# pachterlab/kallisto

Hardware: AMD Instinct MI355X
Metric: M paired-end reads/sec quantified (human txome index) (higher is better)
Workload: dtype u64+f64

## Files before the change

__graft_entry__.py:

```python
from __future__ import annotations

import os
import subprocess
import sys

ROOT = os.path.dirname(os.path.abspath(__file__))
if ROOT not in sys.path:
    sys.path.insert(0, ROOT)


def build() -> None:
    env = dict(os.environ)
    subprocess.check_call(["make", "-C", os.path.join(ROOT, "kallisto_amd", "csrc"), f"-j{min(os.cpu_count() or 1, 8)}", "all"], env=env)
    subprocess.check_call(["make", "-C", os.path.join(ROOT, "oracle"), "oracle"], env=env)
    subprocess.check_call(["make", "-C", os.path.join(ROOT, "tests", "emu")], env=env)
    subprocess.check_call(["make", "-C", os.path.join(ROOT, "tests", "emu_ixbuild")], env=env)
    subprocess.check_call(["make", "-C", os.path.join(ROOT, "tests", "emu_aa")], env=env)
    subprocess.check_call(["make", "-C", os.path.join(ROOT, "tests", "emu_shade")], env=env)
    subprocess.check_call(["make", "-C", os.path.join(ROOT, "tests", "emu_inflate")], env=env)
    subprocess.check_call(["make", "-C", os.path.join(ROOT, "tests", "emu_readec")], env=env)
    subprocess.check_call(["make", "-C", os.path.join(ROOT, "tests", "emu_bustag")], env=env)
    if os.path.exists("/root/reference/src/main.cpp"):
        subprocess.check_call(["make", "-C", os.path.join(ROOT, "oracle"), "-j8", "ref"], env=env)
        subprocess.check_call(["make", "-C", os.path.join(ROOT, "oracle"), "ref_bound"], env=env)
    import kallisto_amd
    kallisto_amd.load_library()
    if os.path.exists(os.path.join(ROOT, "oracle", "_ref", "kallisto")):
        for extra in ([], ["--workload", "stress"], ["--genes", "46000"]):
            subprocess.check_call([sys.executable, os.path.join(ROOT, "bench.py"), "--prepare-only", *extra], env=env)


def smoke() -> None:
    import numpy as np
    import kallisto_amd as ka
    from oracle import oracle as O
    from tests import common

    meta, idx_path, r1, r2 = common.load_case("ref_test_pe")
    reads = common.interleave(r1, r2)
    index = ka.Index(idx_path)
    ctx = ka.Context(0)
    ctx.upload(index)
    words, lens, max_len = ctx.pack_reads_host(reads)
    opts = ka.QuantOpts(1, 0.0, 0.0, 0, 0)
    res = ka.quant(ctx, opts, [(words, lens, len(r1), max_len)])
    oix = O.Index(idx_path)
    buf, off, ln = O.pack_reads(reads)
    ores = O.process_reads(oix, O.Opts(1, 0.0, 0.0, 0, 0), buf, off, ln)
    assert res.ecs.multiset() == ores.multiset(), "EC counts differ from the oracle"
    assert np.array_equal(res.flens, ores.flens), "fragment length sample differs from the oracle"
    eff, _ = O.eff_lens(oix.target_lens, O.mean_frag_lens_trunc(ores.flens))
    assert np.array_equal(eff, res.eff_lens)
    alpha, _, rounds = O.em_run(ores.ec_off, ores.ec_ids, ores.counts, eff, oix.num_targets)
    common.assert_abundance_close(res.est_counts, alpha, "est_counts")
    print(f"smoke ok: {res.n_processed} pairs, {res.n_pseudoaligned} pseudoaligned, {len(res.ecs.counts)} ECs, "
          f"EM rounds {res.em_rounds} (oracle {rounds})")


if __name__ == "__main__":
    build()
    if len(sys.argv) > 1 and sys.argv[1] == "smoke":
        smoke()
```

kallisto_amd/csrc/kamd_ctx.hip:

```cpp
#include "kamd_dev.h"

namespace {
void tuning_defaults(kamd_tuning* t) {
  memset(t, 0, sizeof *t);
  t->text_verify = 1; t->items_per_wave = 1024; t->refill_min = 8; t->lds_pad = -1;
  t->em_form = 3; t->em_local_block = 1024; t->em_group_div = -1; t->em_split_len = 16; t->em_small_nnz = -1; t->em_entries_per_lane = -1; t->em_windowed = 2; t->em_graph = 1; t->em_row_lanes = 4;
  t->em_fin_blocks = 1024; t->dedup_form = 2; t->align_chunks = -1; t->em_reg_slices = 1;
  t->em_hybrid = 1; t->overflow_second_pass = 1; t->em_giant_nnz = -1; t->em_blocked = 1;
}
void tuning_merge(kamd_tuning* t, const kamd_tuning& n) {
  if (n.text_verify == 1 || n.text_verify == 2) t->text_verify = n.text_verify;
  if (n.dedup_form == 1 || n.dedup_form == 2) t->dedup_form = n.dedup_form;
  if (n.items_per_wave >= 64) t->items_per_wave = n.items_per_wave;
  if (n.refill_min >= 1 && n.refill_min <= 64) t->refill_min = n.refill_min;
  if (n.lds_pad != 0) t->lds_pad = n.lds_pad < 0 ? -1 : n.lds_pad;
  if (n.em_form >= 1 && n.em_form <= 3) t->em_form = n.em_form;
  if (n.em_local_block == 128 || n.em_local_block == 256 || n.em_local_block == 512 || n.em_local_block == 1024) t->em_local_block = n.em_local_block;
  if (n.em_split_len >= 1 && n.em_split_len <= 64) t->em_split_len = n.em_split_len;
  if (n.em_group_div >= 1 && n.em_group_div <= 1024) t->em_group_div = n.em_group_div;
  else if (n.em_group_div < 0) t->em_group_div = -1;
  if (n.em_small_nnz != 0) t->em_small_nnz = n.em_small_nnz < 0 ? -1 : std::min(n.em_small_nnz, 4096);
  if (n.em_entries_per_lane != 0) t->em_entries_per_lane = n.em_entries_per_lane < 0 ? -1 : n.em_entries_per_lane;
  if (n.em_windowed == 1 || n.em_windowed == 2) t->em_windowed = n.em_windowed;
  if (n.em_graph == 1 || n.em_graph == 2) t->em_graph = n.em_graph;
  if (n.em_row_lanes == 2 || n.em_row_lanes == 4 || n.em_row_lanes == 8) t->em_row_lanes = n.em_row_lanes;
  if (n.em_fin_blocks >= 64) t->em_fin_blocks = n.em_fin_blocks;
  if (n.align_chunks != 0) t->align_chunks = n.align_chunks < 0 ? -1 : std::min(n.align_chunks, 64);
  if (n.em_reg_slices == 1 || n.em_reg_slices == 2) t->em_reg_slices = n.em_reg_slices;
  if (n.em_hybrid == 1 || n.em_hybrid == 2) t->em_hybrid = n.em_hybrid;
  if (n.overflow_second_pass >= 1 && n.overflow_second_pass <= 3) t->overflow_second_pass = n.overflow_second_pass;
  if (n.em_blocked == 1 || n.em_blocked == 2) t->em_blocked = n.em_blocked;
  if (n.em_giant_nnz != 0) t->em_giant_nnz = n.em_giant_nnz < 0 ? -1 : std::max(n.em_giant_nnz, 8);
}
void tuning_from_env(kamd_tuning* t) {
  const char* e = getenv("KAMD_TUNE");
  if (!e || !*e) return;
  kamd_tuning n; memset(&n, 0, sizeof n);
  struct Field { const char* name; int32_t kamd_tuning::*p; bool onoff; };
  static const Field fields[] = {
    {"text_verify", &kamd_tuning::text_verify, true}, {"items_per_wave", &kamd_tuning::items_per_wave, false}, {"refill_min", &kamd_tuning::refill_min, false},
    {"lds_pad", &kamd_tuning::lds_pad, false}, {"em_form", &kamd_tuning::em_form, false}, {"em_entries_per_lane", &kamd_tuning::em_entries_per_lane, false},
    {"em_windowed", &kamd_tuning::em_windowed, true}, {"em_graph", &kamd_tuning::em_graph, true}, {"em_row_lanes", &kamd_tuning::em_row_lanes, false},
    {"em_fin_blocks", &kamd_tuning::em_fin_blocks, false}, {"em_local_block", &kamd_tuning::em_local_block, false}, {"em_group_div", &kamd_tuning::em_group_div, false},
    {"em_split_len", &kamd_tuning::em_split_len, false}, {"dedup_form", &kamd_tuning::dedup_form, false}, {"align_chunks", &kamd_tuning::align_chunks, false},
    {"em_small_nnz", &kamd_tuning::em_small_nnz, false}, {"em_reg_slices", &kamd_tuning::em_reg_slices, true}, {"em_hybrid", &kamd_tuning::em_hybrid, true},
    {"overflow_second_pass", &kamd_tuning::overflow_second_pass, false}, {"em_giant_nnz", &kamd_tuning::em_giant_nnz, false}, {"em_blocked", &kamd_tuning::em_blocked, true}};
  std::string all(e);
  for (size_t pos = 0; pos < all.size();) {
    size_t end = all.find(',', pos);
    if (end == std::string::npos) end = all.size();
    const std::string kv = all.substr(pos, end - pos);
    pos = end + 1;
    const size_t eq = kv.find('=');
    if (eq == std::string::npos) continue;
    const std::string key = kv.substr(0, eq), val = kv.substr(eq + 1);
    bool known = false;
    for (const Field& f : fields) {
      if (key != f.name) continue;
      known = true;
      int32_t v = atoi(val.c_str());
      if (key == "em_form") v = val == "streamed" ? 1 : val == "csr" ? 2 : val == "local" ? 3 : v;
      if (key == "overflow_second_pass" && v == 0) v = 2;
      n.*(f.p) = f.onoff ? (v != 0 ? 1 : 2) : v;
    }
    if (!known) fprintf(stderr, "[kallisto_amd] KAMD_TUNE: unknown field '%s' ignored\n", key.c_str());
  }
  tuning_merge(t, n);
}
}
namespace kamdi {
void apply_quant_opts(kamd_ctx* c, const kamd_quant_opts* o) {
  c->ix.no_jump = o->no_jump ? 1 : 0;
  c->ix.union_mode = o->do_union ? 1 : 0;
  c->ix.comprehensive = (o->strand != 0 && (o->no_jump || o->do_union || c->ix.n_shades)) ? 1 : 0;
}
void apply_tuning(kamd_ctx* c) {
  c->items_per_wave = c->tune.items_per_wave; c->refill_min = c->tune.refill_min;
}
int sync_state(kamd_ctx* c) {
  if (!c->state_pin) HIPC(hipHostMalloc((void**)&c->state_pin, sizeof(DevState), hipHostMallocDefault));
  HIPC(hipMemcpyAsync(c->state_pin, c->state.p, sizeof(DevState), hipMemcpyDeviceToHost, c->stream));
  HIPC(hipStreamSynchronize(c->stream));
  memcpy(&c->host_state, c->state_pin, sizeof(DevState));
  return 0;
}
int push_state(kamd_ctx* c) {
  HIPC(hipMemcpyAsync(c->state.p, &c->host_state, sizeof(DevState), hipMemcpyHostToDevice, c->stream));
  return 0;
}
}

extern "C" uint32_t kamd_abi_version(void) { return KAMD_ABI_VERSION; }
extern "C" int kamd_ctx_create(int device, void* hip_stream, kamd_ctx** out) {
  if (!out) return kamd::fail(-1, "kamd_ctx_create: null output pointer");
  *out = nullptr;
  int ndev = 0;
  if (hipGetDeviceCount(&ndev) != hipSuccess || ndev == 0)
    return kamd::fail(-102, "kamd_ctx_create: no HIP device available (this library has no CPU path)");
  if (device < 0 || device >= ndev) return kamd::fail(-1, "kamd_ctx_create: bad device ordinal");
  HIPC(hipSetDevice(device));
  kamd_ctx* c = new kamd_ctx;
  c->device = device;
  c->stream = (hipStream_t)hip_stream;
  { int v = 0; if (hipDeviceGetAttribute(&v, hipDeviceAttributeMultiprocessorCount, device) != hipSuccess || v <= 0) v = 256; c->n_cus = v; }
  if (c->state.ensure(sizeof(DevState), 0, c->stream)) { delete c; return -100; }
  memset(&c->host_state, 0, sizeof c->host_state);
  if (push_state(c)) { delete c; return -100; }
  if (hipEventCreate(&c->ev0) != hipSuccess || hipEventCreate(&c->ev1) != hipSuccess || hipEventCreate(&c->ev2) != hipSuccess || hipEventCreate(&c->ev3) != hipSuccess) { delete c; return kamd::fail(-100, "hipEventCreate failed"); }
  if (c->stats_a.ensure(sizeof(DevStatsA), 0, c->stream) || hipMemsetAsync(c->stats_a.p, 0, sizeof(DevStatsA), c->stream) != hipSuccess) { delete c; return -100; }
  tuning_defaults(&c->tune);
  tuning_from_env(&c->tune);
  apply_tuning(c);
  *out = c;
  return 0;
}

extern "C" int kamd_ctx_tune(kamd_ctx* c, const kamd_tuning* t) {
  if (!c || !t) return kamd::fail(-1, "kamd_ctx_tune: null argument");
  tuning_merge(&c->tune, *t);
  apply_tuning(c);
  return 0;
}
extern "C" int kamd_ctx_get_tuning(const kamd_ctx* c, kamd_tuning* out) {
  if (!c || !out) return kamd::fail(-1, "kamd_ctx_get_tuning: null argument");
  *out = c->tune;
  return 0;
}

extern "C" void kamd_ctx_destroy(kamd_ctx* c) {
  if (!c) return;
  (void)hipSetDevice(c->device);
  (void)hipStreamSynchronize(c->stream);
  comm_detach_all(c);
  if (c->ev0) (void)hipEventDestroy(c->ev0);
  if (c->ev1) (void)hipEventDestroy(c->ev1);
  if (c->ev2) (void)hipEventDestroy(c->ev2);
  if (c->ev3) (void)hipEventDestroy(c->ev3);
  if (c->al_stream) { (void)hipStreamSynchronize(c->al_stream); (void)hipStreamDestroy(c->al_stream); }
  if (c->al_ev_in) (void)hipEventDestroy(c->al_ev_in);
  if (c->al_ev_out) (void)hipEventDestroy(c->al_ev_out);
  for (hipEvent_t e : c->al_ev_chunk) if (e) (void)hipEventDestroy(e);
  if (c->ev_fin0) (void)hipEventDestroy(c->ev_fin0);
  if (c->ev_fin1) (void)hipEventDestroy(c->ev_fin1);
  for (hipEvent_t e : c->aa_ev) if (e) (void)hipEventDestroy(e);
  for (hipEvent_t e : c->rec_ev) if (e) (void)hipEventDestroy(e);
  for (hipEvent_t e : c->bus_ev) if (e) (void)hipEventDestroy(e);
  if (c->ev_ab0) (void)hipEventDestroy(c->ev_ab0);
  if (c->ev_ab1) (void)hipEventDestroy(c->ev_ab1);
  if (c->em_stream) (void)hipStreamDestroy(c->em_stream);
  if (c->em_side_stream) { (void)hipStreamSynchronize(c->em_side_stream); (void)hipStreamDestroy(c->em_side_stream); }
  if (c->em_ev_fork) (void)hipEventDestroy(c->em_ev_fork);
  if (c->em_ev_join) (void)hipEventDestroy(c->em_ev_join);
  if (c->em_pin) (void)hipHostFree(c->em_pin);
  if (c->state_pin) (void)hipHostFree(c->state_pin);
  c->em_clk.release();
  if (c->hy_giant_stream) { (void)hipStreamSynchronize(c->hy_giant_stream); (void)hipStreamDestroy(c->hy_giant_stream); }
  if (c->hy_ev_sell) (void)hipEventDestroy(c->hy_ev_sell);
  if (c->hy_ev_giant) (void)hipEventDestroy(c->hy_ev_giant);
  if (c->ev_mg0) (void)hipEventDestroy(c->ev_mg0);
  if (c->ev_mg1) (void)hipEventDestroy(c->ev_mg1);
  if (c->ev_ov0) (void)hipEventDestroy(c->ev_ov0);
  if (c->ev_ov1) (void)hipEventDestroy(c->ev_ov1);
  if (c->ov_stream) { (void)hipStreamSynchronize(c->ov_stream); (void)hipStreamDestroy(c->ov_stream); }
  for (hipEvent_t e : {c->ov_ev_in, c->ov_ev_done, c->ov_ev_t0, c->ov_ev_t1}) if (e) (void)hipEventDestroy(e);
  if (c->ov_pin) (void)hipHostFree(c->ov_pin);
  c->ov_state.release();
  for (DBuf* b : {&c->hy_sub, &c->hy_a, &c->hy_b, &c->hy_x, &c->hy_maps, &c->hy_gb[0], &c->hy_gb[1], &c->hy_gb[2], &c->hy_gb[3], &c->hy_gb[4], &c->hy_gb[5]}) b->release();
  if (c->fld_stream) { (void)hipStreamSynchronize(c->fld_stream); (void)hipStreamDestroy(c->fld_stream); }
  if (c->fld_ev) (void)hipEventDestroy(c->fld_ev);
  if (c->fld_ev_in) (void)hipEventDestroy(c->fld_ev_in);
  if (c->fld_host) (void)hipHostFree(c->fld_host);
  if (c->fq_host) (void)hipHostFree(c->fq_host);
  if (c->sell_cache) sell_cache_free(c->sell_cache);
  for (void* p : c->index_allocs) (void)hipFree(p);
  for (DBuf* b : {&c->dense, &c->stream_buf, &c->rec_off, &c->overflow_items, &c->overflow_scratch, &c->state, &c->rec_slot,
                  &c->retry, &c->ttable, &c->tstore, &c->stats_a, &c->list, &c->cand, &c->cand_off, &c->cand_slot, &c->ctable, &c->tup_bound, &c->tup_off, &c->tup_big, &c->raw2, &c->overflow_left, &c->stats_b, &c->clist, &c->sizes, &c->explicit_items,
                  &c->explicit_items_big, &c->exp_stream, &c->exp_off, &c->exp_scratch, &c->bs_cp, &c->bs_samp, &c->raw, &c->dense_first, &c->exp_key, &c->cand_key, &c->ec_first, &c->pm_a, &c->pm_b, &c->pm_rank, &c->eml_tmp, &c->ems_tmp, &c->ems_plan, &c->ems_maps, &c->fld_tl, &c->fld_card, &c->fld_scratch, &c->fld_items, &c->fld_cand,
                  &c->block_sums, &c->ec_off, &c->ec_ids, &c->ec_counts, &c->em_alpha, &c->em_next, &c->em_eff,
                  &c->em_state, &c->em_cn, &c->em_colcnt, &c->em_coloff, &c->em_colrow,
                  &c->em_segoff, &c->em_segt, &c->em_partial, &c->em_a0, &c->em_a1, &c->em_single, &c->em_actflag, &c->em_actpos, &c->em_active, &c->pt_label, &c->pt_flag, &c->pt_len,
                  &c->pt_rowpos, &c->pt_nnzpos, &c->pt_off, &c->pt_ids, &c->pt_counts, &c->pt_wcounts, &c->pt_hist, &c->pt_ck_alpha,
                  &c->pt_ck_a, &c->fq_tiles, &c->fq_nlpos[0], &c->fq_nlpos[1], &c->fq_recs, &c->fq_res, &c->fq_words, &c->fq_len, &c->aa_frames, &c->aa_flen, &c->aa_scratch, &c->aa_offlist, &c->aa_ctr, &c->inf_members, &c->inf_res, &c->txt_counts, &c->txt_res,
                  &c->rec_table, &c->rec_scratch, &c->rec_big_scratch, &c->rec_big_items, &c->rec_ctr, &c->bus_blk, &c->bus_ctr})
    b->release();
  delete c;
}

namespace {
__global__ void k_bm_fill(const u64* __restrict__ ec_off, const u32* __restrict__ ec_ids, const u32* __restrict__ which, u32 stride, u32* words) {
  const u32 e = which[blockIdx.x];
  u32* w = words + (u64)blockIdx.x * stride;
  for (u64 j = ec_off[e] + threadIdx.x; j < ec_off[e + 1]; j += blockDim.x) { const u32 x = ec_ids[j]; atomicOr(&w[x >> 5], 1u << (x & 31)); }
}
}
extern "C" int kamd_index_upload(kamd_ctx* c, const kamd_index* hix) {
  if (!c || !hix) return kamd::fail(-1, "kamd_index_upload: null argument");
  HIPC(hipSetDevice(c->device));
  kamd_index_view v;
  if (int rc = kamd_index_get_view(hix, &v)) return rc;
  const bool build_table = v.table == nullptr;
  HIPC(hipStreamSynchronize(c->stream));
  c->has_index = false;
  for (void* p : c->index_allocs) (void)hipFree(p);
  c->index_allocs.clear();
  DevIndex d{};
  d.k = v.k; d.n_buckets = v.n_buckets; d.n_ecs = v.n_ecs;
  d.table_layout = (int)v.table_layout; d.tag_q = v.tag_q; d.tag_dsh = v.tag_dsh; d.tag_w = v.tag_w;
  const u64 slots = (v.n_buckets + v.pad_buckets) * v.slots_per_bucket;
  if (!build_table) {
    if (int rc = upload(c, (const u64*)v.table, (size_t)(v.n_buckets + v.pad_buckets) * 8, &d.table)) return rc;
    if (int rc = upload(c, v.slot_block, slots, &d.slot_block)) return rc;
    if (int rc = upload(c, v.slot_dist, slots, &d.slot_dist)) return rc;
  }
  if (int rc = upload(c, v.uec_ec, v.n_uec, &d.uec_ec)) return rc;
  if (int rc = upload(c, (const u64*)v.ec_off, v.n_ecs + 1, &d.ec_off)) return rc;
  if (int rc = upload(c, v.ec_ids, v.ec_nnz, &d.ec_ids)) return rc;
  std::vector<uint8_t> ne(v.n_ecs + 1);
  for (u64 e = 0; e < v.n_ecs; e++) ne[e] = v.ec_off[e + 1] > v.ec_off[e];
  if (int rc = upload(c, ne.data(), v.n_ecs, &d.ec_nonempty)) return rc;
  std::vector<u32> ecn(v.n_uec + 1);
  for (u64 u = 0; u < v.n_uec; u++) ecn[u] = v.uec_ec[u] | (ne[v.uec_ec[u]] ? 0x80000000u : 0u);
  if (int rc = upload(c, ecn.data(), v.n_uec, &d.uec_ecn)) return rc;
  if (int rc = upload(c, v.onlist_bits, v.onlist_words, &d.onlist_bits)) return rc;
  d.n_shades = v.n_shades;
  if (v.n_shades) {
    if (int rc = upload(c, (const u64*)v.core_off, v.n_ecs + 1, &d.core_off)) return rc;
    if (int rc = upload(c, v.core_ids, (size_t)v.core_nnz, &d.core_ids)) return rc;
    if (int rc = upload(c, (const u64*)v.shade_off, v.n_ecs + 1, &d.shade_off)) return rc;
    if (int rc = upload(c, v.shade_ids, (size_t)v.shade_nnz, &d.shade_ids)) return rc;
    if (int rc = upload(c, v.shade_colour, (size_t)v.n_targets, &d.shade_colour)) return rc;
  }
  {
    const uint64_t* boff = v.n_shades ? v.core_off : v.ec_off;
    const u64 n_ids = v.n_targets + v.dlist_size;
    const u32 stride = (u32)((n_ids + 31) / 32);
    std::vector<std::pair<u64, u32>> big;
    for (u64 e = 0; e < v.n_ecs; e++) { const u64 sz = boff[e + 1] - boff[e]; if (sz > BM_MIN_MEMBERS) big.emplace_back(sz, (u32)e); }
    std::sort(big.begin(), big.end(), [](const std::pair<u64, u32>& a, const std::pair<u64, u32>& b) { return a.first > b.first || (a.first == b.first && a.second < b.second); });
    const size_t fit = stride ? BM_MAX_BYTES / ((size_t)stride * 4) : 0;
    if (big.size() > fit) big.resize(fit);
    d.bm_stride = stride; d.bm_min = big.empty() ? 0xFFFFFFFFu : BM_MIN_MEMBERS;
    d.ec_bm_slot = nullptr; d.bm_words = nullptr;
    if (!big.empty()) {
      std::vector<u32> slot(v.n_ecs, BM_NONE), which(big.size());
      for (size_t s = 0; s < big.size(); s++) { slot[big[s].second] = (u32)s; which[s] = big[s].second; }
      const u32* d_which = nullptr; const u32* d_words = nullptr;
      if (int rc = upload(c, slot.data(), slot.size(), &d.ec_bm_slot)) return rc;
      if (int rc = upload(c, which.data(), which.size(), &d_which)) return rc;
      {
        void* p = nullptr;
        HIPC(hipMalloc(&p, big.size() * (size_t)stride * 4));
        c->index_allocs.push_back(p);
        HIPC(hipMemsetAsync(p, 0, big.size() * (size_t)stride * 4, c->stream));
        d_words = (const u32*)p;
      }
      hipLaunchKernelGGL(k_bm_fill, dim3((unsigned)big.size()), dim3(256), 0, c->stream, v.n_shades ? d.core_off : d.ec_off, v.n_shades ? d.core_ids : d.ec_ids, d_which, stride, const_cast<u32*>(d_words));
      HIPC(hipGetLastError());
      d.bm_words = d_words;
      HIPC(hipStreamSynchronize(c->stream));
    }
    c->n_set_bitmaps = (u32)big.size();
  }
  if (int rc = upload(c, (const u64*)v.unitig_blk_off, v.n_unitigs + 1, &d.unitig_blk_off)) return rc;
  if (int rc = upload(c, v.unitig_len, v.n_unitigs, &d.unitig_len)) return rc;
  if (int rc = upload(c, v.blk_unitig, v.n_blocks, &d.blk_unitig)) return rc;
  if (int rc = upload(c, v.blk_lb, v.n_blocks, &d.blk_lb)) return rc;
  if (int rc = upload(c, v.blk_ub, v.n_blocks, &d.blk_ub)) return rc;
  if (int rc = upload(c, v.blk_ec, v.n_blocks, &d.blk_ec)) return rc;
  if (int rc = upload(c, (const u64*)v.blk_pos_off, v.n_blocks + 1, &d.blk_pos_off)) return rc;
  if (int rc = upload(c, v.blk_posw, (size_t)v.blk_pos_off[v.n_blocks], &d.blk_posw)) return rc;
  if (int rc = upload(c, v.blk_sense, (size_t)v.blk_pos_off[v.n_blocks], &d.blk_sense)) return rc;
  if (int rc = upload(c, v.target_lens, v.n_targets + v.dlist_size, &d.target_lens)) return rc;
  d.dtable = nullptr; d.n_dbuckets = v.n_dbuckets; d.dummy_slot = v.dummy_slot; d.dummy_uec = v.dummy_uec; d.dummy_strand = v.dummy_strand;
  if (v.n_dbuckets) if (int rc = upload(c, (const u64*)v.dtable, (size_t)(v.n_dbuckets + v.dpad_buckets) * 8, &d.dtable)) return rc;
  if (int rc = upload(c, v.utext, (size_t)v.utext_words, &d.utext)) return rc;
  HIPC(hipStreamSynchronize(c->stream));
  kamd_table_info ti; memset(&ti, 0, sizeof ti);
  if (build_table) { if (int rc = index_build_device(c, hix, v, &d, &ti)) return rc; }
  else {
    ti.n_buckets = v.n_buckets; ti.pad_buckets = v.pad_buckets; ti.table_layout = v.table_layout; ti.slots_per_bucket = v.slots_per_bucket;
    ti.tag_q = v.tag_q; ti.tag_dsh = v.tag_dsh; ti.tag_w = v.tag_w; ti.n_dbuckets = v.n_dbuckets; ti.dpad_buckets = v.dpad_buckets;
    ti.dummy_slot = v.dummy_slot; ti.dummy_uec = v.dummy_uec; ti.dummy_strand = v.dummy_strand;
  }
  c->tinfo = ti;
  c->aa_ready = false; memset(&c->aa_stats, 0, sizeof c->aa_stats);
  c->ix = d; c->has_index = true; c->n_ecs = v.n_ecs; c->n_targets = v.n_targets;
  if (int rc = c->dense.ensure(std::max<u64>(v.n_ecs, 1) * sizeof(u32), 0, c->stream)) return rc;
  HIPC(hipMemsetAsync(c->dense.p, 0, std::max<u64>(v.n_ecs, 1) * sizeof(u32), c->stream));
  if (int rc = c->dense_first.ensure(std::max<u64>(v.n_ecs, 1) * sizeof(u64), 0, c->stream)) return rc;
  HIPC(hipMemsetAsync(c->dense_first.p, 0xFF, std::max<u64>(v.n_ecs, 1) * sizeof(u64), c->stream));
  memset(&c->host_state, 0, sizeof c->host_state);
  c->finalized = false; c->exp_words_done = 0; c->recs_total = 0; c->multi_before = 0; c->last_absorb_ms = 0.f; c->overflow_total = 0; c->overflow_ms = 0.f;
  if (int rc = tuples_clear(c)) return rc;
  HIPC(hipMemsetAsync(c->stats_a.p, 0, sizeof(DevStatsA), c->stream));
  return push_state(c);
}

extern "C" int kamd_ec_reset(kamd_ctx* c) {
  if (!c || !c->has_index) return kamd::fail(-1, "kamd_ec_reset: no context / index");
  HIPC(hipSetDevice(c->device));
  HIPC(hipMemsetAsync(c->dense.p, 0, std::max<u64>(c->n_ecs, 1) * sizeof(u32), c->stream));
  HIPC(hipMemsetAsync(c->dense_first.p, 0xFF, std::max<u64>(c->n_ecs, 1) * sizeof(u64), c->stream));
  memset(&c->host_state, 0, sizeof c->host_state);
  c->finalized = false; c->exp_words_done = 0; c->recs_total = 0; c->multi_before = 0; c->last_absorb_ms = 0.f; c->overflow_total = 0; c->overflow_ms = 0.f; c->overflow_second_total = 0;
  if (c->ov_side_pending) { (void)hipStreamSynchronize(c->ov_stream); c->ov_side_pending = false; }
  if (int rc = tuples_clear(c)) return rc;
// ... 428 lines not shown
```

kallisto_amd/csrc/kamd_dev.h:

```cpp
#pragma once

#include <hip/hip_runtime.h>

#include <dlfcn.h>

#include <algorithm>
#include <cstring>
#include <string>
#include <chrono>
#include <thread>
#include <vector>

#include "../../include/kallisto_amd.h"
#include "kamd_core.h"
#include "kamd_fq_core.h"
#include "kamd_host.h"
#include "kamd_em_local.h"
#include "kamd_em_sell.h"

#define HIPC(x)                                                                                   \
  do {                                                                                            \
    hipError_t e_ = (x);                                                                          \
    if (e_ != hipSuccess) return kamd::fail(-100, std::string(#x) + ": " + hipGetErrorString(e_)); \
  } while (0)
// ... 93 lines not shown
constexpr u32 BM_NONE = 0xFFFFFFFFu;
constexpr u32 BM_MIN_MEMBERS = 128;
constexpr size_t BM_MAX_BYTES = 256u << 20;
__device__ __forceinline__ bool bitmap_has(const DevIndex& ix, u32 slot, u32 x) { return (ix.bm_words[(u64)slot * ix.bm_stride + (x >> 5)] >> (x & 31)) & 1u; }
__device__ __forceinline__ bool set_has(const DevIndex& ix, u32 e, u64 off, u32 sz, u32 x) {
  if (sz > ix.bm_min) { const u32 s = ix.ec_bm_slot[e]; if (s != BM_NONE) return bitmap_has(ix, s, x); }
  return set_contains(ix.ec_ids + off, sz, x);
}
__host__ __device__ inline kamd::ShadeTables shade_tables(const DevIndex& ix) {
  return kamd::ShadeTables{(const uint64_t*)ix.core_off, ix.core_ids, (const uint64_t*)ix.shade_off, ix.shade_ids, ix.shade_colour};
}
__host__ __device__ inline DevIndex core_view(DevIndex ix) {
  if (ix.n_shades) { ix.ec_off = ix.core_off; ix.ec_ids = ix.core_ids; ix.n_shades = 0; }
  return ix;
}
template <class F>
__device__ __forceinline__ void for_each_member(const DevIndex& ix, const kamd::EcList& ecs, u32* cur, F&& f) {
  if (ix.n_shades) {
    kamd::for_each_in_shaded_set(shade_tables(ix), ecs, ix.union_mode != 0, cur, [&](u32 x) { if (onlisted(ix.onlist_bits, x)) f(x); });
    return;
  }
  const kamd::SetTables st{(const uint64_t*)ix.ec_off, ix.ec_ids};
  kamd::for_each_in_set(st, ecs, ix.union_mode != 0, cur, [&](u32 x) { if (onlisted(ix.onlist_bits, x)) f(x); });
}
__device__ __forceinline__ kamd::PosTables pos_tables(const DevIndex& ix) {
  return kamd::PosTables{(const uint64_t*)ix.unitig_blk_off, ix.unitig_len, ix.blk_unitig, ix.blk_lb, ix.blk_ub, ix.blk_ec,
                         (const uint64_t*)ix.blk_pos_off, ix.blk_posw, ix.blk_sense, (const uint64_t*)ix.ec_off, ix.ec_ids,
                         ix.target_lens, ix.k};
}
__device__ __forceinline__ kamd::FirstHit first_hit(const DevIndex& ix, const kamd::MateInfo& m) {
  kamd::FirstHit h; h.valid = m.n_hits > 0;
  h.block = h.valid ? ix.slot_block[m.first_slot] : 0u; h.dist = h.valid ? ix.slot_dist[m.first_slot] : 0u;
  h.strand = m.first_strand; h.pos = m.first_pos;
  return h;
}
__device__ __forceinline__ kamd::FilterCfg item_filter_cfg(const FilterDev& fd, bool paired, const kamd::MateInfo& m0,
                                                           const kamd::MateInfo& m1) {
  kamd::FilterCfg cfg;
  cfg.fraglen = !fd.single_overhang && fd.has_mean_fl && (!paired || m0.n_hits == 0 || m1.n_hits == 0);
  cfg.fl = fd.fl; cfg.strand = fd.strand;
  cfg.comprehensive = fd.comprehensive != 0 && fd.strand != 0;
  return cfg;
}
__device__ __forceinline__ bool needs_hit_list(const FilterDev& fd, const kamd::MateInfo& m1) {
  return fd.comprehensive != 0 && fd.strand != 0 && m1.n_hits == 0;
}
__device__ __noinline__ u32 class_size_bound(const DevIndex& ix, const kamd::EcList& ecs) {
  if (ix.n_shades) return (u32)kamd::shaded_size_bound(shade_tables(ix), ecs.e, ecs.n, ix.union_mode != 0);
  const kamd::SetTables st{(const uint64_t*)ix.ec_off, ix.ec_ids};
  return (u32)kamd::set_size_bound(st, ecs.e, ecs.n, ix.union_mode != 0);
}
__device__ __forceinline__ int filter_outcome(const DevIndex& ix, const FilterDev& fd, bool paired, const kamd::MateInfo& m0,
                                              const kamd::MateInfo& m1, const kamd::EcList& ecs, u32* kept, u32* cur) {
  const kamd::FilterCfg cfg = item_filter_cfg(fd, paired, m0, m1);
  if (!cfg.fraglen && !cfg.strand) return 0;
  if (needs_hit_list(fd, m1)) {
    *kept = class_size_bound(ix, ecs);
    return 2;
  }
  const kamd::PosTables pt = pos_tables(ix);
  const kamd::FirstHit h0 = first_hit(ix, m0), h1 = first_hit(ix, m1);
  u32 total = 0, keep = 0;
  for_each_member(ix, ecs, cur, [&](u32 tr) { ++total; keep += kamd::keep_transcript(pt, cfg, h0, h1, tr) ? 1u : 0u; });
  *kept = keep;
  return keep == total ? 0 : (keep == 0 ? 1 : 2);
}
struct DBuf {
  void* p = nullptr; size_t cap = 0;
  int ensure(size_t bytes, size_t keep, hipStream_t s) {
    if (bytes <= cap) return 0;
    size_t ncap = std::max(bytes, 2 * cap);
    void* np = nullptr;
    HIPC(hipMalloc(&np, ncap));
    if (keep && p) HIPC(hipMemcpyAsync(np, p, keep, hipMemcpyDeviceToDevice, s));
    if (p) { HIPC(hipStreamSynchronize(s)); HIPC(hipFree(p)); }
    p = np; cap = ncap;
    return 0;
  }
  void release() { if (p) (void)hipFree(p); p = nullptr; cap = 0; }
  template <class T> T* as() { return reinterpret_cast<T*>(p); }
};

inline unsigned grid_for(u64 n, int block) { return (unsigned)((n + block - 1) / block); }

struct SellCache;
void sell_cache_free(SellCache*);
}
using namespace kamdi;
namespace {
__global__ void k_copy_words(const u32* __restrict__ src, u64 n, u32* dst) {
  u64 i = (u64)blockIdx.x * blockDim.x + threadIdx.x;
  if (i < n) dst[i] = src[i];
}
__global__ void k_copy_offsets(const u64* __restrict__ src, u64 n, u64 base, u64* dst) {
  u64 i = (u64)blockIdx.x * blockDim.x + threadIdx.x;
  if (i < n) dst[i] = src[i] + base;
}
}

struct kamd_ctx {
  int device = 0;
  hipStream_t stream = nullptr;
  bool has_index = false;
  DevIndex ix{};
  std::vector<void*> index_allocs;
  u64 n_ecs = 0, n_targets = 0;
  u32 n_set_bitmaps = 0;
  kamd_table_info tinfo{};
  DBuf dense, stream_buf, rec_off, overflow_items, overflow_scratch, state, rec_slot, retry, ttable, list;
  DBuf cand, cand_off, cand_slot, ctable, clist, sizes, block_sums, tup_bound, tup_off, tup_big;
  DBuf raw2, overflow_left, stats_b;
  u64 overflow_second_total = 0;
  DBuf ov_state; DevState* ov_pin = nullptr; hipStream_t ov_stream = nullptr; hipEvent_t ov_ev_in = nullptr, ov_ev_done = nullptr, ov_ev_t0 = nullptr, ov_ev_t1 = nullptr;
  bool ov_side_pending = false;
  u64 last_fin_big = 0;
  DBuf explicit_items, explicit_items_big, exp_stream, exp_off, exp_scratch, bs_cp, bs_samp, raw, dense_first, exp_key, cand_key, ec_first;
  DBuf ec_off, ec_ids, ec_counts;
  DBuf em_alpha, em_next, em_eff, em_state, em_cn, em_colcnt, em_coloff, em_colrow, em_segoff, em_segt, em_partial, em_a0, em_a1, em_single, em_actflag, em_actpos, em_active;
  DBuf pm_a, pm_b, pm_rank;
  DBuf eml_tmp, ems_tmp, ems_plan, ems_maps;
  SellCache* sell_cache = nullptr;
  u64 ec_generation = 0;
  int last_em_plan_cached = 0;
  DBuf fq_tiles, fq_nlpos[2], fq_recs, fq_res, fq_words, fq_len;
  void* fq_host = nullptr;
  u64 fq_batch_reads = 0; int32_t fq_batch_max_len = 0, fq_batch_files = 0;
  DBuf fld_tl, fld_card, fld_scratch, fld_items, fld_cand;
  void* fld_host = nullptr; u64 fld_host_cap = 0;
  hipStream_t fld_stream = nullptr; hipEvent_t fld_ev = nullptr, fld_ev_in = nullptr;
  struct { const uint32_t* w = nullptr; const uint16_t* l = nullptr; u64 n = 0; int32_t max_len = 0, strand = 0, so = 0; bool valid = false; } fld_pending;
  struct { const uint32_t* w = nullptr; const uint16_t* l = nullptr; u64 n = 0; int32_t max_len = 0, strand = 0, so = 0, comp = 0; bool valid = false; } fld_deferred;
  DBuf pt_label, pt_flag, pt_len, pt_rowpos, pt_nnzpos, pt_off, pt_ids, pt_counts, pt_wcounts, pt_hist, pt_ck_alpha, pt_ck_a;
  DevState host_state{};
  DevState* state_pin = nullptr;
  u64 tcap = 0, ccap = 0;
  DBuf tstore;
  bool ttable_clean = false;
  u64 recs_total = 0;
  u64 multi_before = 0;
  u64 n_distinct_tuples = 0;
  float last_absorb_ms = 0.f; hipEvent_t ev_ab0 = nullptr, ev_ab1 = nullptr;
  kamd_ec_result result{};
  bool finalized = false;
  u64 exp_words_done = 0;
  hipEvent_t ev0 = nullptr, ev1 = nullptr;
  float last_align_ms = 0.f, last_em_ms = 0.f, last_classify_ms = 0.f;
  hipEvent_t ev2 = nullptr, ev3 = nullptr, ev_fin0 = nullptr, ev_fin1 = nullptr;
  DBuf stats_a;
  hipStream_t al_stream = nullptr; hipEvent_t al_ev_in = nullptr, al_ev_out = nullptr; std::vector<hipEvent_t> al_ev_chunk;
  float last_finalize_ms = 0.f; u64 last_fin_records = 0, last_fin_stream_words = 0, last_fin_cand_words = 0;
  hipStream_t em_stream = nullptr;
  hipStream_t em_side_stream = nullptr; hipEvent_t em_ev_fork = nullptr, em_ev_join = nullptr;
  void* em_pin = nullptr; size_t em_pin_bytes = 0;
  DBuf em_clk;
  DBuf hy_sub, hy_a, hy_b, hy_x, hy_maps;
  DBuf hy_gb[6];
  hipStream_t hy_giant_stream = nullptr;
  hipEvent_t hy_ev_sell = nullptr, hy_ev_giant = nullptr;
  uint64_t last_em_max_comp_nnz = 0, last_em_giant_nnz = 0, last_em_giant_rows = 0, last_em_giant_tr = 0;
  uint32_t last_em_giant_chunks = 0; uint64_t last_em_giant_pieces = 0; int last_em_graph_fallback = 0; float last_em_plan_ms = 0.f;
  float last_merge_ms = 0.f, em_coll_ms = 0.f; uint32_t em_coll_n = 0; hipEvent_t ev_mg0 = nullptr, ev_mg1 = nullptr;
  const uint32_t* labels_override = nullptr;
  bool em_prefer_hybrid = false;
  uint64_t overflow_total = 0; float overflow_ms = 0.f; hipEvent_t ev_ov0 = nullptr, ev_ov1 = nullptr;
  int items_per_wave = 1024, refill_min = 8;
  kamd_tuning tune{};
  bool track_order = false;
  bool had_overflow_items = false;
  int n_cus = 0, last_em_k = 0; unsigned last_em_grid = 0, last_em_lds = 0;
  uint64_t last_em_iters = 0, last_em_nnz = 0, last_em_nnz_multi = 0, last_em_nseg = 0, last_em_necs = 0;
  DBuf aa_frames, aa_flen, aa_scratch, aa_offlist, aa_ctr;
  bool aa_ready = false;
  kamd_aa_stats aa_stats{};
  hipEvent_t aa_ev[3] = {nullptr, nullptr, nullptr};
  DBuf inf_members, inf_res, txt_counts, txt_res;
  DBuf rec_table, rec_scratch, rec_big_scratch, rec_big_items, rec_ctr;
  u64 rec_table_gen = 0, rec_table_cap = 0, rec_chunk = 0, rec_second = 0;
  int rec_small_cap = 0;
  hipEvent_t rec_ev[3] = {nullptr, nullptr, nullptr};
  float rec_table_ms = 0.f, rec_items_ms = 0.f;
  DBuf bus_blk, bus_ctr;
  hipEvent_t bus_ev[2] = {nullptr, nullptr};
  std::vector<struct kamd_comm*> comms;
};

namespace kamdi {
int sync_state(kamd_ctx* c);
int push_state(kamd_ctx* c);
void apply_quant_opts(kamd_ctx* c, const kamd_quant_opts* o);
void apply_tuning(kamd_ctx* c);
void comm_detach_all(kamd_ctx* c);
int index_build_device(kamd_ctx* c, const kamd_index* hix, const kamd_index_view& v, DevIndex* d, kamd_table_info* info);
int exclusive_scan(kamd_ctx* c, const u32* sizes, u64 n, u64* out, u64* d_total);
int tuples_clear(kamd_ctx* c);
int absorb_tuples(kamd_ctx* c, const u32* batch, const u64* rec_off, u64 n, u64 batch_words, u64 key_base, u64 n_tuple_bound,
                  const u64* first_idx = nullptr, u32 fixed_stride = 0, u64 item0 = 0);
template <class T>
int upload(kamd_ctx* c, const T* host, size_t n, const T** dev) {
  void* p = nullptr;
  size_t bytes = std::max<size_t>(n, 1) * sizeof(T);
  HIPC(hipMalloc(&p, bytes));
  c->index_allocs.push_back(p);
  if (n) HIPC(hipMemcpyAsync(p, host, n * sizeof(T), hipMemcpyHostToDevice, c->stream));
  *dev = reinterpret_cast<const T*>(p);
  return 0;
}
}
```

kallisto_amd/csrc/kamd_em.hip:

```cpp
#include "kamd_dev.h"

namespace {

struct EmState {
  int iter;
  int chcount;
  int final_round;
  int done;
  int rounds;
  int force_final;
  int pad[2];
};
struct EmNow { int it, fin, done, rounds; };
__host__ __device__ inline EmNow em_next_round(const EmState& prev, int n_iter, int min_rounds, bool spec) {
  EmNow n; n.it = prev.iter; n.fin = prev.final_round; n.done = prev.done; n.rounds = prev.rounds;
  if (n.done) return n;
  if (prev.final_round) { n.done = 1; n.rounds = prev.iter; return n; }
  const bool stopEM = !spec && prev.chcount == 0 && prev.iter > min_rounds;
  n.it = prev.iter + 1;
  n.fin = (stopEM || prev.force_final) ? 1 : 0;
  if (n.it >= n_iter) { n.done = 1; n.rounds = n_iter; }
  return n;
}
__device__ __forceinline__ double em_clamped(const double* alpha, const double* a, u32 t, int clamp) {
// ... 763 lines not shown
    case 8: pm_launch_round<8>(P, s, parity); break;
    case 12: pm_launch_round<12>(P, s, parity); break;
    case 16: pm_launch_round<16>(P, s, parity); break;
    case 20: pm_launch_round<20>(P, s, parity); break;
    case 24: pm_launch_round<24>(P, s, parity); break;
    case 28: pm_launch_round<28>(P, s, parity); break;
    default: pm_launch_round<32>(P, s, parity); break;
  }
}

int em_streamed_setup(kamd_ctx* c, const u64* ec_off, const u32* ec_ids, const u32* counts, const u32* wcounts, u64 n_ecs, u64 T,
                      const u32* col_cnt, u32* col_fill, PmPlan* P, DBuf* arena_a = nullptr, DBuf* arena_b = nullptr) {
  if (n_ecs == 0) return 1;
  DBuf& ar_a = arena_a ? *arena_a : c->pm_a;
  DBuf& ar_b = arena_b ? *arena_b : c->pm_b;
  if (c->n_cus == 0) {
    int v = 0;
    HIPC(hipDeviceGetAttribute(&v, hipDeviceAttributeMultiprocessorCount, c->device));
    c->n_cus = v > 0 ? v : 256;
  }
  Carver s1;
  const size_t o_hist = s1.take((T + 1) * 4), o_fill = s1.take((T + 1) * 4), o_mflag = s1.take(T * 4);
  const size_t o_start = s1.take((T + 2) * 8), o_rpos = s1.take((n_ecs + 1) * 8), o_mpos = s1.take((T + 1) * 8);
  const size_t o_len = s1.take((n_ecs + 1) * 4), o_roff = s1.take((n_ecs + 2) * 8);
  if (int rc = ar_a.ensure(s1.off, 0, c->stream)) return rc;
  char* b1 = (char*)ar_a.p;
  u32* hist = (u32*)(b1 + o_hist); u32* mflag = (u32*)(b1 + o_mflag);
  u64* start = (u64*)(b1 + o_start); u64* rpos = (u64*)(b1 + o_rpos); u64* mpos = (u64*)(b1 + o_mpos);
  u32* len_sorted = (u32*)(b1 + o_len); u64* roff = (u64*)(b1 + o_roff);
  (void)o_fill;
  HIPC(hipMemsetAsync(hist, 0, (o_mflag - o_hist), c->stream));
  hipLaunchKernelGGL(k_pm_flags, dim3(grid_for(std::max(n_ecs, T), BLOCK)), dim3(BLOCK), 0, c->stream, ec_off, ec_ids, n_ecs, col_cnt, T, hist,
                     mflag);
  if (int rc = exclusive_scan(c, hist, T, start, start + T)) return rc;
  if (int rc = exclusive_scan(c, mflag, T, mpos, mpos + T)) return rc;
  u64 R = 0, NZ = 0, M = 0;
  HIPC(hipMemcpyAsync(&R, start + T, 8, hipMemcpyDeviceToHost, c->stream));
  HIPC(hipMemcpyAsync(&M, mpos + T, 8, hipMemcpyDeviceToHost, c->stream));
  HIPC(hipMemcpyAsync(&NZ, c->em_coloff.as<u64>() + T, 8, hipMemcpyDeviceToHost, c->stream));
  HIPC(hipStreamSynchronize(c->stream));
  if (NZ == 0 || R == 0 || M == 0 || R >= 0x7FFFFFF0ULL || M >= 0x7FFFFFF0ULL || NZ >= (1ULL << 40)) return 1;
  {
    if (n_ecs >= 0xFFFFFFF0ULL) return 1;
    const u32 n_tiles = (u32)((n_ecs + PM_RANK_TILE - 1) / PM_RANK_TILE);
    const u64 n_cells = (u64)PM_RANK_BUCKETS * n_tiles;
    Carver rv;
    const size_t o_key = rv.take(n_ecs * 8), o_oa = rv.take(n_ecs * 4), o_ob = rv.take(n_ecs * 4), o_h = rv.take(n_cells * 4), o_f = rv.take((n_cells + 2) * 8);
    if (int rc = c->pm_rank.ensure(rv.off, 0, c->stream)) return rc;
    char* rb = (char*)c->pm_rank.p;
    u64* key = (u64*)(rb + o_key); u32* ord[2] = {(u32*)(rb + o_oa), (u32*)(rb + o_ob)}; u32* rhist = (u32*)(rb + o_h); u64* rfirst = (u64*)(rb + o_f);
    hipLaunchKernelGGL(k_pm_rowkey, dim3(grid_for(n_ecs * 8, BLOCK)), dim3(BLOCK), 0, c->stream, ec_off, ec_ids, n_ecs, T, key);
    const u32* in = nullptr;
    for (int pass = 0; pass < PM_RANK_PASSES; pass++) {
      u32* out = ord[pass & 1];
      hipLaunchKernelGGL(k_pm_radix_hist, dim3(n_tiles), dim3(64), 0, c->stream, (const u64*)key, in, n_ecs, pass, n_tiles, rhist);
      if (int rc = exclusive_scan(c, rhist, n_cells, rfirst, rfirst + n_cells)) return rc;
      hipLaunchKernelGGL(k_pm_radix_place, dim3(n_tiles), dim3(64), 0, c->stream, (const u64*)key, in, n_ecs, pass, n_tiles, (const u64*)rfirst, out);
      in = out;
    }
    hipLaunchKernelGGL(k_pm_rank_emit, dim3(grid_for(R, BLOCK)), dim3(BLOCK), 0, c->stream, ec_off, in, R, rpos, len_sorted);
    HIPC(hipGetLastError());
  }
  if (int rc = exclusive_scan(c, len_sorted, R, roff, roff + R)) return rc;
  int K = PM_KS[sizeof(PM_KS) / sizeof(PM_KS[0]) - 1];
  bool k_forced = false;
  if (c->tune.em_entries_per_lane > 0) { for (int k : PM_KS) if (k == c->tune.em_entries_per_lane) { K = k; k_forced = true; } }
  if (!k_forced) for (int k : PM_KS) if ((NZ + 64ULL * k - 1) / (64ULL * k) <= (u64)c->n_cus * 12) { K = k; break; }
  const u32 chunk = 64u * (u32)K;
  const u64 n_chunks64 = (NZ + chunk - 1) / chunk;
  if (n_chunks64 >= 0x7FFFFFF0ULL) return 1;
  const u32 n_chunks = (u32)n_chunks64;
  const u64 nzpad = (u64)n_chunks * chunk;
  Carver s2;
  const size_t front = 64 * PM_HEAD * 4;
  const size_t o_rs = s2.take(front + nzpad * 4), o_cs = s2.take(front + nzpad * 4);
  size_t o_meta[2][5];
  size_t o_lane[2];
  for (int s = 0; s < 2; s++) {
    for (int j = 0; j < 3; j++) o_meta[s][j] = s2.take((size_t)n_chunks * 4);
    for (int j = 3; j < 5; j++) o_meta[s][j] = s2.take((size_t)n_chunks * 8);
    o_lane[s] = s2.take((size_t)n_chunks * 64 * 4);
  }
  const size_t o_cw = s2.take(R * 8), o_coff = s2.take((M + 1) * 8), o_g = s2.take((R + 1) * 8);
  size_t o_vec[6];
  for (int j = 0; j < 6; j++) o_vec[j] = s2.take((M + 1) * 8);
  const size_t o_single = s2.take(M * 8), o_eff = s2.take(M * 8), o_nfix = s2.take(64);
  if (int rc = ar_b.ensure(s2.off, 0, c->stream)) return rc;
  char* b2 = (char*)ar_b.p;
  u32* rs = (u32*)(b2 + o_rs + front); u32* cs = (u32*)(b2 + o_cs + front);
  HIPC(hipMemsetAsync(b2 + o_rs, 0, front, c->stream));
  HIPC(hipMemsetAsync(b2 + o_cs, 0, front, c->stream));
  u64* cw = (u64*)(b2 + o_cw); u64* coff = (u64*)(b2 + o_coff);
  double* g = (double*)(b2 + o_g);
  double* vec[6]; for (int j = 0; j < 6; j++) vec[j] = (double*)(b2 + o_vec[j]);
  double* single_m = (double*)(b2 + o_single); double* eff_m = (double*)(b2 + o_eff);
  HIPC(hipMemsetAsync(b2 + o_nfix, 0, 64, c->stream));
  HIPC(hipMemsetAsync(g + R, 0, 8, c->stream));
  const u64* col_off = c->em_coloff.as<u64>();
  hipLaunchKernelGGL(k_pm_rows, dim3(grid_for(n_ecs * 8, BLOCK)), dim3(BLOCK), 0, c->stream, ec_off, ec_ids, counts, wcounts, n_ecs, rpos, roff,
                     mpos, rs, cw);
  hipLaunchKernelGGL(k_pm_cols, dim3(grid_for(n_ecs * 8, BLOCK)), dim3(BLOCK), 0, c->stream, ec_off, ec_ids, n_ecs, rpos, col_off, col_fill, cs);
  if (nzpad > NZ) {
    hipLaunchKernelGGL(k_pm_fill, dim3(grid_for(nzpad - NZ, BLOCK)), dim3(BLOCK), 0, c->stream, rs, NZ, nzpad, (u32)M);
    hipLaunchKernelGGL(k_pm_fill, dim3(grid_for(nzpad - NZ, BLOCK)), dim3(BLOCK), 0, c->stream, cs, NZ, nzpad, (u32)R);
  }
  hipLaunchKernelGGL(k_pm_minit, dim3(grid_for(T, BLOCK)), dim3(BLOCK), 0, c->stream, T, mflag, mpos, col_off, c->em_single.as<double>(),
                     c->em_eff.as<double>(), M, coff, single_m, eff_m, vec[0], vec[1], vec[2], vec[3], vec[4], vec[5]);
  PmSide sides[2];
  for (int s = 0; s < 2; s++) {
    PmSide& d = sides[s];
    d.stream = s == 0 ? rs : cs;
    u32* sb = (u32*)(b2 + o_meta[s][0]); u32* hd = (u32*)(b2 + o_meta[s][1]); u32* ff = (u32*)(b2 + o_meta[s][2]);
    d.seg_base = sb; d.head = hd; d.fix_first = ff;
    d.lp = (double*)(b2 + o_meta[s][3]); d.rp = (double*)(b2 + o_meta[s][4]);
    d.n_chunks = n_chunks;
    u32* lw = (u32*)(b2 + o_lane[s]);
    d.lane_word = lw;
    hipLaunchKernelGGL(k_pm_lanes, dim3(grid_for(n_chunks, PM_BLOCK / 64)), dim3(PM_BLOCK), 0, c->stream, d.stream, chunk / 64, n_chunks, lw);
    hipLaunchKernelGGL(k_pm_chunks, dim3(grid_for(n_chunks, BLOCK)), dim3(BLOCK), 0, c->stream, s == 0 ? roff : coff, s == 0 ? R : M, NZ, chunk,
                       n_chunks, sb, hd, ff, (u32*)(b2 + o_nfix) + s, (u32*)(b2 + o_nfix) + 2, getenv("KAMD_EM_NO_LONG_HEADS") ? 1 : 0);
  }
  HIPC(hipGetLastError());
  PmArgs& A = P->args;
  A.rows = sides[0]; A.cols = sides[1];
  A.cw = cw; A.g = g;
  A.alpha0 = vec[0]; A.alpha1 = vec[1]; A.a0 = vec[2]; A.a1 = vec[3]; A.ac0 = vec[4]; A.ac1 = vec[5];
  A.single = single_m; A.eff = eff_m;
  A.R = (u32)R; A.M = (u32)M;
  A.st = (EmState*)c->em_state.p;
  u32 plan_words[3] = {0, 0, 0};
  HIPC(hipMemcpyAsync(plan_words, b2 + o_nfix, sizeof plan_words, hipMemcpyDeviceToHost, c->stream));
  HIPC(hipStreamSynchronize(c->stream));
  P->n_fix[0] = plan_words[0]; P->n_fix[1] = plan_words[1];
  P->windowed = plan_words[2] > (u32)PM_LDS_SLOTS;
  if (c->tune.em_windowed == 1) P->windowed = true;
  P->k = K; P->n_chunks = n_chunks; P->mflag = mflag; P->mpos = mpos; P->rpos = rpos;
  P->roff = roff; P->coff = coff; P->rs = rs; P->cs = cs; P->nzpad = nzpad;
  c->last_em_nnz_multi = NZ; c->last_em_nseg = n_chunks; c->last_em_necs = n_ecs; c->last_em_k = K;
  c->last_em_grid = grid_for(n_chunks, PM_BLOCK / 64);
  return 0;
}

struct EmLocalDev {
  const u32* row_base; const u32* tr_base; const u64* nz_base;
  const u32* row_ptr; const u32* col_ptr; const uint16_t* row_tr; const uint16_t* col_row;
  const u64* cw; const double* single; const double* eff;
  const u32* tr_id = nullptr;
};
constexpr int EML_MAX_ROUNDS = 64;
struct EmSellDev {
  const u32* row_base; const u32* tr_base; const u32* rslice_base; const u32* cslice_base; const u64* rell_base; const u64* cell_base;
  const u32* rdesc; const u32* cdesc; const uint16_t* rell; const uint16_t* cell;
  const u64* cw; const double* single; const double* eff;
};
constexpr int EMS_MAX_BLOCK = 1024;
template <int EXP>
__device__ __forceinline__ double ems_slice_sum(const u64* e, u32 width, const double* src, u32 n_src) {
  const u32 cf = (u32)lane_id() % n_src;
  u32 sink = 0;
  auto val_at = [&](u32 ix) -> double {
    if constexpr (EXP == 1) { sink += ix; return src[cf]; }
    else if constexpr (EXP == 3) return __hiloint2double(0x3ff00000, (int)ix);
    else return src[ix];
  };
  double S = 0.0;
  u32 j = 0;
  for (; j + 8 <= width; j += 8) {
    const u64 w0 = e[(size_t)(j >> 2) * 64], w1 = e[(size_t)((j >> 2) + 1) * 64];
    const u32 a0 = (u32)w0, a1 = (u32)(w0 >> 32), b0 = (u32)w1, b1 = (u32)(w1 >> 32);
    const double v0 = val_at(a0 & 0xFFFFu), v1 = val_at(a0 >> 16), v2 = val_at(a1 & 0xFFFFu), v3 = val_at(a1 >> 16);
    const double v4 = val_at(b0 & 0xFFFFu), v5 = val_at(b0 >> 16), v6 = val_at(b1 & 0xFFFFu), v7 = val_at(b1 >> 16);
    S += v0; S += v1; S += v2; S += v3; S += v4; S += v5; S += v6; S += v7;
  }
  if (j < width) {
    const u32 rem = width - j;
    const u64 w0 = e[(size_t)(j >> 2) * 64];
    const u64 w1 = rem > 4 ? e[(size_t)((j >> 2) + 1) * 64] : 0ULL;
    const u32 a0 = (u32)w0, a1 = (u32)(w0 >> 32), b0 = (u32)w1, b1 = (u32)(w1 >> 32);
    const double v0 = val_at(a0 & 0xFFFFu);
    const double v1 = rem > 1 ? val_at(a0 >> 16) : 0.0;
    const double v2 = rem > 2 ? val_at(a1 & 0xFFFFu) : 0.0;
    const double v3 = rem > 3 ? val_at(a1 >> 16) : 0.0;
    S += v0;
    if (rem > 1) S += v1;
    if (rem > 2) S += v2;
    if (rem > 3) S += v3;
    if (rem > 4) {
      const double v4 = val_at(b0 & 0xFFFFu);
      const double v5 = rem > 5 ? val_at(b0 >> 16) : 0.0;
      const double v6 = rem > 6 ? val_at(b1 & 0xFFFFu) : 0.0;
      S += v4;
      if (rem > 5) S += v5;
      if (rem > 6) S += v6;
    }
  }
  if constexpr (EXP != 0) { if (sink == 0xFFFFFFFFu) S += 1.0; }
  return S;
}
constexpr int EMS_CLK_ROUND = 8, EMS_CLK_WORDS = 16;
template <bool WAVE_TEAM, int EXP = 0>
__device__ __forceinline__ void ems_group_rounds(const EmSellDev& P, u32 g, unsigned char* smem, u32 tid, u32 nthr, const double* alpha, const double* a,
                                                 double* alpha_out, double* a_out, int n_rounds, int clamp, int* s_hist, long long* clk = nullptr) {
  namespace L = kamd_em_sell;
  const int lane = lane_id();
  const u32 wv = WAVE_TEAM ? 0u : (u32)__builtin_amdgcn_readfirstlane((int)(tid >> 6)), NW = WAVE_TEAM ? 1u : nthr >> 6;
  const u32 r0 = P.row_base[g], nR = P.row_base[g + 1] - r0, t0 = P.tr_base[g], nT = P.tr_base[g + 1] - t0;
  const u32 rs0 = P.rslice_base[g], nrs = P.rslice_base[g + 1] - rs0, cs0 = P.cslice_base[g], ncs = P.cslice_base[g + 1] - cs0;
  const u64 re0 = P.rell_base[g], ce0 = P.cell_base[g];
  const u32 nru = (u32)(P.rell_base[g + 1] - re0), ncu = (u32)(P.cell_base[g + 1] - ce0);
  auto team_sync = [] {
    if (WAVE_TEAM || EXP == 5) __builtin_amdgcn_fence(__ATOMIC_SEQ_CST, "wavefront");
    else __syncthreads();
  };
  double* s_al0 = reinterpret_cast<double*>(smem);
  double* s_a0 = s_al0 + (nT + 1); double* s_al1 = s_a0 + (nT + 1); double* s_a1 = s_al1 + (nT + 1);
  double* s_single = s_a1 + (nT + 1); double* s_eff = s_single + nT; double* s_g = s_eff + nT;
  u64* s_cw = reinterpret_cast<u64*>(s_g + (nR + 1));
  u32* s_rdesc = reinterpret_cast<u32*>(s_cw + nR); u32* s_cdesc = s_rdesc + 2 * nrs;
  uint16_t* s_rell = reinterpret_cast<uint16_t*>(s_cdesc + 2 * ncs); uint16_t* s_cell = s_rell + ((nru + 1) & ~1u);
  for (u32 i = tid; i < nT; i += nthr) {
    double al = alpha[t0 + i], av = a[t0 + i];
    if (clamp && al < 1e-7 / 10.0) { al = 0.0; av = 0.0; }
    s_al0[i] = al; s_a0[i] = av; s_single[i] = P.single[t0 + i]; s_eff[i] = P.eff[t0 + i];
  }
  for (u32 i = tid; i < nR; i += nthr) s_cw[i] = P.cw[r0 + i];
  for (u32 i = tid; i < 2 * nrs; i += nthr) s_rdesc[i] = P.rdesc[2 * (u64)rs0 + i];
  for (u32 i = tid; i < 2 * ncs; i += nthr) s_cdesc[i] = P.cdesc[2 * (u64)cs0 + i];
  for (u32 i = tid; i < nru; i += nthr) { const uint16_t v = P.rell[re0 + i]; s_rell[i] = v == (uint16_t)L::SELL_PAD ? (uint16_t)nT : v; }
  for (u32 i = tid; i < ncu; i += nthr) { const uint16_t v = P.cell[ce0 + i]; s_cell[i] = v == (uint16_t)L::SELL_PAD ? (uint16_t)nR : v; }
  if (tid == 0) { s_al0[nT] = s_a0[nT] = s_al1[nT] = s_a1[nT] = 0.0; s_g[nR] = 0.0; }
  team_sync();
  double* al = s_al0; double* av = s_a0; double* aln = s_al1; double* avn = s_a1;
  for (int r = 0; r < n_rounds; r++) {
    const bool tick = clk && r == EMS_CLK_ROUND && lane == 0;
    long long w0 = 0;
    if (tick) { clk[0] = clock64(); w0 = wall_clock64(); }
    for (u32 s = wv; s < nrs; s += NW) {
      const u32 d0 = s_rdesc[2 * s], d1 = s_rdesc[2 * s + 1];
      const bool meta = (d0 & L::DESC_META) != 0;
      const u32 off = d0 & ~L::DESC_META, width = d1 & 0xFFFFu;
      const bool tk = tick && s == wv;
      if (tk) clk[12] = clock64();
      double S = ems_slice_sum<EXP>(reinterpret_cast<const u64*>(s_rell + off + (meta ? 2 * L::SELL_META_WORDS : 0u)) + lane, width, av, nT);
      if (tk) { clk[13] = clock64(); clk[14] = (long long)(width | (meta ? 0x10000u : 0u)); }
      u32 seg = (d1 >> 16) + (u32)lane; bool fin = seg < nR;
      if (meta) {
        const u32 w = reinterpret_cast<const u32*>(s_rell + off)[lane];
        S = pm_scan_seg(S, (int)((w >> 16) & 0x7Fu), lane);
        seg = w & 0xFFFFu; fin = (w & L::META_ACTIVE) && (w & L::META_LAST);
      }
      if (fin) {
        const u64 cwv = s_cw[seg];
        const u32 cnt = (u32)cwv, wc = (u32)(cwv >> 32);
        if constexpr (EXP == 4) s_g[seg] = (double)cnt * S;
        else s_g[seg] = (cnt == 0 || (double)wc * S < 4.9406564584124654e-324) ? 0.0 : (double)cnt / S;
      }
      if (tk) clk[15] = clock64();
    }
    if (tick) clk[1] = clock64();
    team_sync();
    if (tick) clk[2] = clock64();
    int ch = 0;
    for (u32 s = wv; s < ncs; s += NW) {
      const u32 d0 = s_cdesc[2 * s], d1 = s_cdesc[2 * s + 1];
      const bool meta = (d0 & L::DESC_META) != 0;
      const u32 off = d0 & ~L::DESC_META, width = d1 & 0xFFFFu;
      const bool tk = tick && s == wv;
      if (tk) clk[8] = clock64();
      double acc = ems_slice_sum<EXP>(reinterpret_cast<const u64*>(s_cell + off + (meta ? 2 * L::SELL_META_WORDS : 0u)) + lane, width, s_g, nR);
      if (tk) { clk[9] = clock64(); clk[10] = (long long)(width | (meta ? 0x10000u : 0u)); }
      u32 seg = (d1 >> 16) + (u32)lane; bool fin = seg < nT;
      if (meta) {
        const u32 w = reinterpret_cast<const u32*>(s_cell + off)[lane];
        acc = pm_scan_seg(acc, (int)((w >> 16) & 0x7Fu), lane);
        seg = w & 0xFFFFu; fin = (w & L::META_ACTIVE) && (w & L::META_LAST);
      }
      bool chg = false;
      if (fin) {
        const double at = av[seg], cur = al[seg];
        const double nx = s_single[seg] + at * acc;
        const double dd = fabs(nx - cur);
        bool moved = dd > 1.0000001e-2 * nx;
        if (dd > 0.9999999e-2 * nx && !moved) moved = dd / nx > 1e-2;
        chg = nx > 1e-2 && moved;
        aln[seg] = nx;
        if constexpr (EXP == 4) avn[seg] = nx * s_eff[seg];
        else avn[seg] = nx / s_eff[seg];
      }
      ch += __popcll(__ballot(chg));
      if (tk) clk[11] = clock64();
    }
    if (ch && lane == 0) atomicAdd(&s_hist[r], ch);
    if (tick) clk[3] = clock64();
    team_sync();
    if (tick) { clk[4] = clock64(); clk[5] = (long long)(nrs | (ncs << 16)); clk[6] = (long long)(nru | ((u64)ncu << 32)); clk[7] = wall_clock64() - w0; }
    double* t1 = al; al = aln; aln = t1;
    double* t2 = av; av = avn; avn = t2;
  }
  for (u32 i = tid; i < nT; i += nthr) { alpha_out[t0 + i] = al[i]; a_out[t0 + i] = av[i]; }
}
template <int NB>
__device__ __forceinline__ void ems_reg_gather(const u64* w, const unsigned char* lds0, double* v) {
#pragma unroll
  for (int q = 0; q < NB; q++) {
    u32 lo = (u32)w[q], hi = (u32)(w[q] >> 32);
    asm volatile("" : "+v"(lo), "+v"(hi));
    v[4 * q] = *reinterpret_cast<const double*>(lds0 + (lo & 0xFFFFu)); v[4 * q + 1] = *reinterpret_cast<const double*>(lds0 + (lo >> 16));
    v[4 * q + 2] = *reinterpret_cast<const double*>(lds0 + (hi & 0xFFFFu)); v[4 * q + 3] = *reinterpret_cast<const double*>(lds0 + (hi >> 16));
  }
}
template <int NQ, bool TREE>
__device__ __forceinline__ double ems_reg_sum(const u64* w, const unsigned char* lds0, double S = 0.0) {
  if constexpr (!TREE) {
    constexpr int NB = NQ < 2 ? NQ : 2;
    double v[4 * NB];
    ems_reg_gather<NB>(w, lds0, v);
#pragma unroll
    for (int i = 0; i < 4 * NB; i++) S += v[i];
    if constexpr (NQ > 2) return ems_reg_sum<NQ - 2, false>(w + 2, lds0, S);
    else return S;
  } else {
    constexpr int NB = NQ < 4 ? NQ : 4;
    double v[4 * NB];
    ems_reg_gather<NB>(w, lds0, v);
#pragma unroll
    for (int st = 1; st < 4 * NB; st *= 2)
#pragma unroll
      for (int i = 0; i + st < 4 * NB; i += 2 * st) v[i] += v[i + st];
    if constexpr (NQ > 4) return ems_reg_sum<NQ - 4, true>(w + 4, lds0, S + v[0]);
    else return S + v[0];
  }
}
template <int W, bool TREE, int NQ = 1>
__device__ __forceinline__ double ems_reg_slice_sum(const u64* w, u32 nq, const unsigned char* lds0) {
  if constexpr (NQ >= W) return ems_reg_sum<W, TREE>(w, lds0);
  else { if (nq <= (u32)NQ) return ems_reg_sum<NQ, TREE>(w, lds0); return ems_reg_slice_sum<W, TREE, NQ + 1>(w, nq, lds0); }
}
__device__ __forceinline__ u32 pm_scan_seg_steps(int reach, int lane) {
  const int r = lane & 15;
  u32 m = 0;
  if (__ballot(reach >= 1 && r >= 1)) m |= 1u;
  if (__ballot(reach >= 2 && r >= 2)) m |= 2u;
  if (__ballot(reach >= 4 && r >= 4)) m |= 4u;
  if (__ballot(reach >= 8 && r >= 8)) m |= 8u;
  if (__ballot((lane & 16) && reach > r)) m |= 16u;
  if (__ballot(lane >= 32 && reach > lane - 32)) m |= 32u;
  return m;
}
__device__ __forceinline__ double pm_scan_seg_masked(double y, int reach, int lane, u32 steps) {
  const int r = lane & 15;
  if (steps & 1u) { const double t = pm_dpp<0x111, 0xF>(y); if (reach >= 1 && r >= 1) y += t; }
  if (steps & 2u) { const double t = pm_dpp<0x112, 0xF>(y); if (reach >= 2 && r >= 2) y += t; }
  if (steps & 4u) { const double t = pm_dpp<0x114, 0xF>(y); if (reach >= 4 && r >= 4) y += t; }
  if (steps & 8u) { const double t = pm_dpp<0x118, 0xF>(y); if (reach >= 8 && r >= 8) y += t; }
  if (steps & 16u) { const double t = pm_dpp<0x142, 0xA>(y); if ((lane & 16) && reach > r) y += t; }
  if (steps & 32u) { const double t = pm_dpp<0x143, 0xC>(y); if (lane >= 32 && reach > lane - 32) y += t; }
  return y;
}
__device__ __forceinline__ double ems_slice_sum_narrow(const u64* e, u32 width, const double* src) {
  double S = 0.0;
  for (u32 j = 0; j < width; j += 4) {
    const u64 w = e[(size_t)(j >> 2) * 64];
    const u32 lo = (u32)w, hi = (u32)(w >> 32);
    const double v0 = src[lo & 0xFFFFu], v1 = src[lo >> 16], v2 = src[hi & 0xFFFFu], v3 = src[hi >> 16];
    S += v0; S += v1; S += v2; S += v3;
  }
  return S;
}
template <int W, int NS>
__device__ __forceinline__ void ems_group_rounds_reg(const EmSellDev& P, u32 g, unsigned char* smem, u32 tid, u32 nthr, const double* alpha, const double* a,
                                                     double* alpha_out, double* a_out, int n_rounds, int clamp, int* s_hist, long long* clk = nullptr) {
  namespace L = kamd_em_sell;
  constexpr bool TREE = W >= 8 || (W == 4 && NS == 2);
  const int lane = lane_id();
  const u32 wv = (u32)__builtin_amdgcn_readfirstlane((int)(tid >> 6)), NW = nthr >> 6;
  const u32 r0 = P.row_base[g], nR = P.row_base[g + 1] - r0, t0 = P.tr_base[g], nT = P.tr_base[g + 1] - t0;
  const u32 rs0 = P.rslice_base[g], nrs = P.rslice_base[g + 1] - rs0, cs0 = P.cslice_base[g], ncs = P.cslice_base[g + 1] - cs0;
  const u64 re0 = P.rell_base[g], ce0 = P.cell_base[g];
  const u32 nru = (u32)(P.rell_base[g + 1] - re0), ncu = (u32)(P.cell_base[g + 1] - ce0);
  double* s_a0 = reinterpret_cast<double*>(smem);
  double* s_g = s_a0 + (nT + 1);
  double* s_al0 = s_g + (nR + 1);
  double* s_single = s_al0 + (nT + 1); double* s_eff = s_single + nT;
  u64* s_cw = reinterpret_cast<u64*>(s_eff + nT);
  u32* s_rdesc = reinterpret_cast<u32*>(s_cw + nR); u32* s_cdesc = s_rdesc + 2 * nrs;
  uint16_t* s_rell = reinterpret_cast<uint16_t*>(s_cdesc + 2 * ncs); uint16_t* s_cell = s_rell + ((nru + 1) & ~1u);
  const u32 a_off = 0u, g_off = (nT + 1) * 8u;
  const bool near = g_off + (nR + 1) * 8u <= 0x10000u;
  for (u32 i = tid; i < nT; i += nthr) {
    double al = alpha[t0 + i], av = a[t0 + i];
    if (clamp && al < 1e-7 / 10.0) { al = 0.0; av = 0.0; }
    s_al0[i] = al; s_a0[i] = av; s_single[i] = P.single[t0 + i]; s_eff[i] = P.eff[t0 + i];
  }
  for (u32 i = tid; i < nR; i += nthr) s_cw[i] = P.cw[r0 + i];
  for (u32 i = tid; i < 2 * nrs; i += nthr) s_rdesc[i] = P.rdesc[2 * (u64)rs0 + i];
  for (u32 i = tid; i < 2 * ncs; i += nthr) s_cdesc[i] = P.cdesc[2 * (u64)cs0 + i];
  for (u32 i = tid; i < nru; i += nthr) { const uint16_t v = P.rell[re0 + i]; s_rell[i] = v == (uint16_t)L::SELL_PAD ? (uint16_t)nT : v; }
  for (u32 i = tid; i < ncu; i += nthr) { const uint16_t v = P.cell[ce0 + i]; s_cell[i] = v == (uint16_t)L::SELL_PAD ? (uint16_t)nR : v; }
  if (tid == 0) { s_al0[nT] = s_a0[nT] = 0.0; s_g[nR] = 0.0; }
  __syncthreads();
  struct Own { u64 w[W]; u32 nq, seg, steps; int reach; bool has, meta, fin; };
  auto take = [&](const u32* desc, const uint16_t* ell, u32 s, u32 n_slices, u32 n_segs, u32 zero, u32 base_off) {
    Own o;
    o.has = near && s < n_slices; o.nq = 1; o.seg = 0; o.reach = 0; o.meta = false; o.fin = false; o.steps = 0;
    if (o.has && (((desc[2 * s + 1] & 0xFFFFu) + 3u) >> 2) > (u32)W) o.has = false;
    const u64 padw = (u64)(base_off + zero * 8u) * 0x0001000100010001ULL;
#pragma unroll
    for (int q = 0; q < W; q++) o.w[q] = padw;
    if (o.has) {
      const u32 d0 = desc[2 * s], d1 = desc[2 * s + 1];
      o.meta = (d0 & L::DESC_META) != 0;
      const u32 off = d0 & ~L::DESC_META, width = d1 & 0xFFFFu;
      o.nq = (u32)__builtin_amdgcn_readfirstlane((int)((width + 3u) >> 2));
      const u64* e = reinterpret_cast<const u64*>(ell + off + (o.meta ? 2 * L::SELL_META_WORDS : 0u)) + lane;
#pragma unroll
      for (int q = 0; q < W; q++) if ((u32)q < o.nq) {
        const u64 ix4 = e[(size_t)q * 64];
        o.w[q] = ((ix4 & 0x1FFF1FFF1FFF1FFFULL) << 3) + (u64)base_off * 0x0001000100010001ULL;
      }
      o.seg = (d1 >> 16) + (u32)lane; o.fin = o.seg < n_segs;
      if (o.meta) {
        const u32 w = reinterpret_cast<const u32*>(ell + off)[lane];
        o.reach = (int)((w >> 16) & 0x7Fu); o.seg = w & 0xFFFFu; o.fin = (w & L::META_ACTIVE) && (w & L::META_LAST);
        o.steps = pm_scan_seg_steps(o.reach, lane);
      }
      if (!o.fin) o.seg = 0;
    }
    return o;
  };
  Own ro[NS], co[NS];
  u32 r_cnt[NS], r_wc[NS];
  double c_single[NS], c_eff[NS], c_at[NS], c_cur[NS];
  u32 r_next = wv, c_next = wv;
#pragma unroll
  for (int k = 0; k < NS; k++) {
    ro[k] = take(s_rdesc, s_rell, wv + (u32)k * NW, nrs, nR, nT, a_off);
    co[k] = take(s_cdesc, s_cell, wv + (u32)k * NW, ncs, nT, nR, g_off);
    if (ro[k].has && r_next == wv + (u32)k * NW) r_next += NW; else ro[k].has = false;
    if (co[k].has && c_next == wv + (u32)k * NW) c_next += NW; else co[k].has = false;
    r_cnt[k] = 0; r_wc[k] = 0; c_single[k] = 0.0; c_eff[k] = 1.0; c_at[k] = 0.0; c_cur[k] = 0.0;
    if (ro[k].has && ro[k].fin) { const u64 cwv = s_cw[ro[k].seg]; r_cnt[k] = (u32)cwv; r_wc[k] = (u32)(cwv >> 32); }
    if (co[k].has && co[k].fin) { c_single[k] = s_single[co[k].seg]; c_eff[k] = s_eff[co[k].seg]; c_at[k] = s_a0[co[k].seg]; c_cur[k] = s_al0[co[k].seg]; }
  }
  double* const al = s_al0; double* const av = s_a0;
  const unsigned char* const lds0 = smem;
  for (int r = 0; r < n_rounds; r++) {
    const bool tick = clk && r == EMS_CLK_ROUND && lane == 0;
    long long w0 = 0;
    if (tick) { clk[0] = clock64(); w0 = wall_clock64(); }
#pragma unroll
    for (int k = 0; k < NS; k++) {
      if (ro[k].has) {
        const bool tk = tick && k == 0;
        if (tk) clk[12] = clock64();
        double S = ems_reg_slice_sum<W, TREE>(ro[k].w, ro[k].nq, lds0);
        if (tk) { clk[13] = clock64(); clk[14] = (long long)((ro[k].nq * 4u) | (ro[k].meta ? 0x10000u : 0u)); }
        if (ro[k].meta) S = pm_scan_seg_masked(S, ro[k].reach, lane, ro[k].steps);
        if (ro[k].fin) s_g[ro[k].seg] = (r_cnt[k] == 0 || (double)r_wc[k] * S < 4.9406564584124654e-324) ? 0.0 : (double)r_cnt[k] / S;
        if (tk) clk[15] = clock64();
      }
    }
    for (u32 s = r_next; s < nrs; s += NW) {
      const u32 d0 = s_rdesc[2 * s], d1 = s_rdesc[2 * s + 1];
      const bool meta = (d0 & L::DESC_META) != 0;
      const u32 off = d0 & ~L::DESC_META, width = d1 & 0xFFFFu;
      double S = ems_slice_sum_narrow(reinterpret_cast<const u64*>(s_rell + off + (meta ? 2 * L::SELL_META_WORDS : 0u)) + lane, width, av);
      u32 seg = (d1 >> 16) + (u32)lane; bool fin = seg < nR;
      if (meta) {
        const u32 w = reinterpret_cast<const u32*>(s_rell + off)[lane];
        S = pm_scan_seg(S, (int)((w >> 16) & 0x7Fu), lane);
        seg = w & 0xFFFFu; fin = (w & L::META_ACTIVE) && (w & L::META_LAST);
      }
      if (fin) {
        const u64 cwv = s_cw[seg];
        const u32 cnt = (u32)cwv, wc = (u32)(cwv >> 32);
        s_g[seg] = (cnt == 0 || (double)wc * S < 4.9406564584124654e-324) ? 0.0 : (double)cnt / S;
      }
    }
    if (tick) clk[1] = clock64();
    __syncthreads();
    if (tick) clk[2] = clock64();
    int ch = 0;
    auto finish_col = [&](u32 seg, double at, double cur, double single, double eff, double acc, double& nx_out, double& a_out_v) {
      const double nx = single + at * acc;
      const double dd = fabs(nx - cur);
      bool moved = dd > 1.0000001e-2 * nx;
      if (dd > 0.9999999e-2 * nx && !moved) moved = dd / nx > 1e-2;
      nx_out = nx; a_out_v = nx / eff;
      al[seg] = nx; av[seg] = a_out_v;
      return nx > 1e-2 && moved;
    };
#pragma unroll
    for (int k = 0; k < NS; k++) {
      if (co[k].has) {
        const bool tk = tick && k == 0;
        if (tk) clk[8] = clock64();
        double acc = ems_reg_slice_sum<W, TREE>(co[k].w, co[k].nq, lds0);
        if (tk) { clk[9] = clock64(); clk[10] = (long long)((co[k].nq * 4u) | (co[k].meta ? 0x10000u : 0u)); }
        if (co[k].meta) acc = pm_scan_seg_masked(acc, co[k].reach, lane, co[k].steps);
        bool chg = false;
        if (co[k].fin) chg = finish_col(co[k].seg, c_at[k], c_cur[k], c_single[k], c_eff[k], acc, c_cur[k], c_at[k]);
        ch += __popcll(__ballot(chg));
        if (tk) clk[11] = clock64();
      }
    }
    for (u32 s = c_next; s < ncs; s += NW) {
      const u32 d0 = s_cdesc[2 * s], d1 = s_cdesc[2 * s + 1];
      const bool meta = (d0 & L::DESC_META) != 0;
      const u32 off = d0 & ~L::DESC_META, width = d1 & 0xFFFFu;
      double acc = ems_slice_sum_narrow(reinterpret_cast<const u64*>(s_cell + off + (meta ? 2 * L::SELL_META_WORDS : 0u)) + lane, width, s_g);
      u32 seg = (d1 >> 16) + (u32)lane; bool fin = seg < nT;
      if (meta) {
        const u32 w = reinterpret_cast<const u32*>(s_cell + off)[lane];
        acc = pm_scan_seg(acc, (int)((w >> 16) & 0x7Fu), lane);
        seg = w & 0xFFFFu; fin = (w & L::META_ACTIVE) && (w & L::META_LAST);
      }
      bool chg = false;
      if (fin) { double nx, an; chg = finish_col(seg, av[seg], al[seg], s_single[seg], s_eff[seg], acc, nx, an); }
      ch += __popcll(__ballot(chg));
    }
    if (ch && lane == 0) atomicAdd(&s_hist[r], ch);
    if (tick) clk[3] = clock64();
    __syncthreads();
    if (tick) { clk[4] = clock64(); clk[5] = (long long)(nrs | (ncs << 16)); clk[6] = (long long)(nru | ((u64)ncu << 32)); clk[7] = wall_clock64() - w0; }
  }
  for (u32 i = tid; i < nT; i += nthr) { alpha_out[t0 + i] = al[i]; a_out[t0 + i] = av[i]; }
}
struct EmsPrev { const int* hist; int n; int base; int min_rounds; int* host_hist; int* host_seq; int seq; };
__device__ __forceinline__ bool ems_prev_stopped(const EmsPrev& v, int* s_flag) {
  if (!v.hist) return false;
  if (threadIdx.x < 64) {
    const int i = (int)threadIdx.x;
    const int h = i < v.n ? v.hist[i] : 1;
    const bool stop = i < v.n && h == 0 && v.base + i > v.min_rounds;
    const u64 m = __ballot(stop);
    if (blockIdx.x == 0 && v.host_hist) {
      if (i < v.n) v.host_hist[i] = h;
      __threadfence_system();
      if (i == 0) __hip_atomic_store(v.host_seq, v.seq, __ATOMIC_RELEASE, __HIP_MEMORY_SCOPE_SYSTEM);
    }
    if (i == 0) *s_flag = m != 0;
  }
  __syncthreads();
  return *s_flag != 0;
}
template <bool CLK, int EXP = 0, int W = 0, int NS = 1>
__global__ __launch_bounds__(EMS_MAX_BLOCK) __attribute__((amdgpu_waves_per_eu((W >= 8 || (W == 4 && NS == 2)) ? 4 : 8))) void k_em_sell(EmSellDev P, u32 g_first, const double* alpha, const double* a, double* alpha_out, double* a_out,
                                                           int n_rounds, int clamp, int* hist, EmsPrev prev, long long* clk) {
  extern __shared__ __attribute__((aligned(16))) unsigned char ems_smem[];
  __shared__ int s_hist[EML_MAX_ROUNDS];
  __shared__ int s_stop;
  if (ems_prev_stopped(prev, &s_stop)) return;
  if (threadIdx.x < EML_MAX_ROUNDS) s_hist[threadIdx.x] = 0;
  __syncthreads();
  long long* my_clk = CLK ? clk + ((size_t)blockIdx.x * (EMS_MAX_BLOCK / 64) + (threadIdx.x >> 6)) * EMS_CLK_WORDS : nullptr;
  if constexpr (W > 0) ems_group_rounds_reg<W, NS>(P, g_first + blockIdx.x, ems_smem, threadIdx.x, blockDim.x, alpha, a, alpha_out, a_out, n_rounds, clamp, s_hist, my_clk);
  else ems_group_rounds<false, EXP>(P, g_first + blockIdx.x, ems_smem, threadIdx.x, blockDim.x, alpha, a, alpha_out, a_out, n_rounds, clamp, s_hist, my_clk);
  __syncthreads();
  if (hist && (int)threadIdx.x < n_rounds && s_hist[threadIdx.x]) atomicAdd(&hist[threadIdx.x], s_hist[threadIdx.x]);
}
constexpr int EMS_WAVE_TEAMS = 4;
__global__ __launch_bounds__(64 * EMS_WAVE_TEAMS) void k_em_sell_wave(EmSellDev P, u32 n_small, u32 team_bytes, const double* alpha, const double* a,
                                                                        double* alpha_out, double* a_out, int n_rounds, int clamp, int* hist, EmsPrev prev) {
  extern __shared__ __attribute__((aligned(16))) unsigned char ems_smem[];
  __shared__ int s_hist[EML_MAX_ROUNDS];
  __shared__ int s_stop;
  if (ems_prev_stopped(prev, &s_stop)) return;
  if (threadIdx.x < EML_MAX_ROUNDS) s_hist[threadIdx.x] = 0;
  __syncthreads();
  const u32 team = (u32)__builtin_amdgcn_readfirstlane((int)(threadIdx.x >> 6));
  const u32 g = blockIdx.x * EMS_WAVE_TEAMS + team;
  if (g < n_small) ems_group_rounds<true>(P, g, ems_smem + (size_t)team * team_bytes, (u32)lane_id(), 64u, alpha, a, alpha_out, a_out, n_rounds, clamp, s_hist);
  __syncthreads();
  if (hist && (int)threadIdx.x < n_rounds && s_hist[threadIdx.x]) atomicAdd(&hist[threadIdx.x], s_hist[threadIdx.x]);
}
struct SellBuild {
  const u32* row_base; const u32* tr_base; const u32* row_ptr; const u32* col_ptr; const uint16_t* row_tr; const uint16_t* col_row; const u64* nz_base;
  const u64* cw; const double* single; const double* eff; const u32* tr_id; u32 n_groups; u32 R; u32 M; u32 cap;
  u32* rlen; u32* clen; u32* rnew; u32* cnew; u32* rlane; u32* clane; u32* rvl; u32* cvl; u32* gsz;
  const u32* rslice_base; const u32* cslice_base; const u64* rell_base; const u64* cell_base;
  u32* rdesc; u32* cdesc; uint16_t* rell; uint16_t* cell; u64* cw_new; double* single_new; double* eff_new; u32* tr_id_new;
};
__device__ __forceinline__ u32 sell_group_of(const u32* base, u32 n_groups, u32 i) {
  u32 lo = 0, hi = n_groups;
  while (hi - lo > 1) { const u32 mid = (lo + hi) / 2; if (base[mid] <= i) lo = mid; else hi = mid; }
  return lo;
}
__global__ void k_sell_lens(SellBuild B) {
  const u32 i = blockIdx.x * blockDim.x + threadIdx.x;
  if (i < B.R) { const u32 g = sell_group_of(B.row_base, B.n_groups, i); B.rlen[i] = B.row_ptr[(u64)i + g + 1] - B.row_ptr[(u64)i + g]; }
  if (i < B.M) { const u32 g = sell_group_of(B.tr_base, B.n_groups, i); B.clen[i] = B.col_ptr[(u64)i + g + 1] - B.col_ptr[(u64)i + g]; }
}
constexpr int SELL_BUILD_WAVES = 4;
struct SellWaveScratch { u32 hist[kamd_em_sell::SELL_LANES + 1], start[kamd_em_sell::SELL_LANES + 1], cur[kamd_em_sell::SELL_LANES + 1]; };
template <class Sink>
__device__ kamd_em_sell::LayoutSize sell_layout_wave(const u32* __restrict__ len, u32 n, u32 cap, Sink& sink, SellWaveScratch& S) {
  namespace L = kamd_em_sell;
  const int lane = lane_id();
  for (u32 b = lane; b <= L::SELL_LANES; b += 64) { S.hist[b] = 0; S.cur[b] = 0; }
  __builtin_amdgcn_wave_barrier();
  u32 n_split = 0, pos = 0;
  u32 off = 0;
  u32 width = 0;
  u32 mw = 0;
  u32 closed = 0;
  for (u32 c0 = 0; c0 < n; c0 += 64) {
    const u32 i = c0 + lane;
    const u32 l = i < n ? len[i] : 0;
    if (i < n && l <= cap) atomicAdd(&S.hist[l], 1u);
    u64 m = __ballot(i < n && l > cap);
    while (m) {
      const int b = __ffsll((unsigned long long)m) - 1;
      m &= m - 1;
      const u32 lb = (u32)__shfl((int)l, b, 64);
      const u32 nv = L::seg_lanes(lb, cap), vl = L::seg_vlen(lb, cap);
      if ((pos % L::SELL_LANES) + nv > L::SELL_LANES) {
        sink.meta(off, lane, mw);
        if (lane == 0) sink.slice(closed, off | L::DESC_META, width);
        off += 2 * L::SELL_META_WORDS + L::quad_width(width) * L::SELL_LANES; ++closed; width = 0; mw = 0;
        pos = (pos / L::SELL_LANES + 1) * L::SELL_LANES;
      }
      if (Sink::wants_segments && lane == b) sink.seg(c0 + b, n_split, pos, nv, vl);
      const u32 rel = pos % L::SELL_LANES;
      if ((u32)lane >= rel && (u32)lane < rel + nv) {
        const u32 v = (u32)lane - rel;
        mw = n_split | (v << 16) | (v + 1 == nv ? L::META_LAST : 0u) | L::META_ACTIVE;
      }
      width = vl > width ? vl : width;
      pos += nv; ++n_split;
      if (pos % L::SELL_LANES == 0) {
        sink.meta(off, lane, mw);
        if (lane == 0) sink.slice(closed, off | L::DESC_META, width);
        off += 2 * L::SELL_META_WORDS + L::quad_width(width) * L::SELL_LANES; ++closed; width = 0; mw = 0;
      }
    }
  }
  __builtin_amdgcn_wave_barrier();
  const u32 split_lanes = pos;
  if (lane == 0) { u32 c = split_lanes; for (u32 b = L::SELL_LANES; b >= 1; b--) { S.start[b] = c; c += S.hist[b]; } S.start[0] = c; }
  __builtin_amdgcn_wave_barrier();
  const u32 total_lanes = S.start[0];
  if (Sink::wants_segments) {
    for (u32 c0 = 0; c0 < n; c0 += 64) {
      const u32 i = c0 + lane;
      const u32 l = i < n ? len[i] : 0u;
      const bool act = i < n && l <= cap;
      u64 same = __ballot(act);
#pragma unroll
      for (int b = 0; b < 7; b++) { const u64 bal = __ballot((l >> b) & 1u); same &= ((l >> b) & 1u) ? bal : ~bal; }
      const u32 below = (u32)__popcll(same & ((1ULL << lane) - 1ULL)), cls = (u32)__popcll(same);
      u32 base = 0;
      if (act) base = S.cur[l];
      __builtin_amdgcn_wave_barrier();
      if (act) {
        const u32 p = S.start[l] + base + below;
        sink.seg(i, n_split + (p - split_lanes), p, 1u, l);
        if (below + 1 == cls) S.cur[l] = base + cls;
      }
      __builtin_amdgcn_wave_barrier();
    }
  }
  auto len_at = [&](u32 p) -> u32 {
    u32 b = L::SELL_LANES;
    while (b > 1 && !(p >= S.start[b] && p < S.start[b] + S.hist[b])) --b;
    return b;
  };
  const u32 n_slices = (total_lanes + L::SELL_LANES - 1) / L::SELL_LANES;
  if (split_lanes % L::SELL_LANES) {
    const u32 lo = closed * L::SELL_LANES, p = lo + (u32)lane;
    if (split_lanes < total_lanes) { const u32 b = len_at(split_lanes); width = b > width ? b : width; }
    if (p >= split_lanes && p < total_lanes) mw = (n_split + (p - split_lanes)) | L::META_LAST | L::META_ACTIVE;
    sink.meta(off, lane, mw);
    if (lane == 0) sink.slice(closed, off | L::DESC_META, width);
    off += 2 * L::SELL_META_WORDS + L::quad_width(width) * L::SELL_LANES; ++closed;
  }
  for (u32 s0 = closed; s0 < n_slices; s0 += 64) {
    const u32 si = s0 + (u32)lane;
    u32 w = 0;
    if (si < n_slices) w = len_at(si * L::SELL_LANES);
    const u32 mine = L::quad_width(w) * L::SELL_LANES;
    const u32 incl = wave_incl_scan(mine);
    if (si < n_slices) sink.slice(si, off + (incl - mine), w | ((n_split + (si * L::SELL_LANES - split_lanes)) << 16));
    off += (u32)__shfl((int)incl, 63, 64);
  }
  return L::LayoutSize{n_slices, off};
}
__global__ __launch_bounds__(64 * SELL_BUILD_WAVES) void k_sell_sizes(SellBuild B) {
  __shared__ SellWaveScratch scr[SELL_BUILD_WAVES];
  const u32 w = (blockIdx.x * blockDim.x + threadIdx.x) / 64, g = w >> 1;
  if (g >= B.n_groups) return;
  kamd_em_sell::NullSink ns;
  const kamd_em_sell::LayoutSize z = (w & 1) ? sell_layout_wave(B.clen + B.tr_base[g], B.tr_base[g + 1] - B.tr_base[g], B.cap, ns, scr[threadIdx.x / 64])
                                             : sell_layout_wave(B.rlen + B.row_base[g], B.row_base[g + 1] - B.row_base[g], B.cap, ns, scr[threadIdx.x / 64]);
  if (lane_id() == 0) { B.gsz[4 * g + 2 * (w & 1)] = z.n_slices; B.gsz[4 * g + 2 * (w & 1) + 1] = z.n_u16; }
}
struct SellDevSink {
  static const bool wants_segments = true;
  u32* new_id; u32* lane; u32* vlen; u32* desc; uint16_t* ell; u32 seg0; u32 desc0; u64 ell0;
  __device__ void seg(u32 old, u32 id, u32 ln, u32, u32 vl) const { new_id[seg0 + old] = id; lane[seg0 + old] = ln; vlen[seg0 + old] = vl; }
  __device__ void slice(u32 i, u32 d0, u32 d1) const { desc[2 * (u64)(desc0 + i)] = d0; desc[2 * (u64)(desc0 + i) + 1] = d1; }
  __device__ void meta(u32 off, u32 l, u32 w) const { ell[ell0 + off + 2 * l] = (uint16_t)w; ell[ell0 + off + 2 * l + 1] = (uint16_t)(w >> 16); }
};
__global__ __launch_bounds__(64 * SELL_BUILD_WAVES) void k_sell_layout(SellBuild B) {
  __shared__ SellWaveScratch scr[SELL_BUILD_WAVES];
  const u32 w = (blockIdx.x * blockDim.x + threadIdx.x) / 64, g = w >> 1;
  if (g >= B.n_groups) return;
  if (w & 1) {
    SellDevSink sc{B.cnew, B.clane, B.cvl, B.cdesc, B.cell, B.tr_base[g], B.cslice_base[g], B.cell_base[g]};
    sell_layout_wave(B.clen + B.tr_base[g], B.tr_base[g + 1] - B.tr_base[g], B.cap, sc, scr[threadIdx.x / 64]);
  } else {
    SellDevSink sr{B.rnew, B.rlane, B.rvl, B.rdesc, B.rell, B.row_base[g], B.rslice_base[g], B.rell_base[g]};
    sell_layout_wave(B.rlen + B.row_base[g], B.row_base[g + 1] - B.row_base[g], B.cap, sr, scr[threadIdx.x / 64]);
  }
}
__global__ void k_sell_entries(SellBuild B) {
  const u32 i = blockIdx.x * blockDim.x + threadIdx.x;
  if (i < B.R) {
    const u32 g = sell_group_of(B.row_base, B.n_groups, i), r0 = B.row_base[g], t0 = B.tr_base[g];
    B.cw_new[r0 + B.rnew[i]] = B.cw[i];
    const u32* rd = B.rdesc + 2 * (u64)B.rslice_base[g];
    const uint16_t* src = B.row_tr + B.nz_base[g];
    const u32 b = B.row_ptr[(u64)i + g], e = B.row_ptr[(u64)i + g + 1];
    const u32 ln = B.rlane[i], vl = B.rvl[i];
    for (u32 j = b, q = 0; j < e; j++, q++)
      B.rell[B.rell_base[g] + kamd_em_sell::entry_pos(rd, ln, vl, q)] = (uint16_t)B.cnew[t0 + src[j]];
// ... 106 lines not shown
  for (int d = 1; d < 64; d <<= 1) { const u32 t = __shfl_up(incl, d, 64); if (lane_id() >= d) incl += t; }
  const u32 w = tid >> 6;
  if (lane_id() == 63) s_w[w] = incl;
  __syncthreads();
  u32 woff = 0;
  for (u32 j = 0; j < w; j++) woff += s_w[j];
  u32 acc = woff + incl - run;
  for (u32 i = b0; i < b1; i++) { const u32 x = a[i]; a[i] = acc; acc += x; }
  if (tid == nthr - 1) a[n] = woff + incl;
  __syncthreads();
}
__global__ __launch_bounds__(BLOCK) void k_eml_rank_tr(kamd_em_local::BuildArgs A) {
  extern __shared__ __attribute__((aligned(16))) unsigned char gb_smem[];
  u32* s_t = reinterpret_cast<u32*>(gb_smem);
  const u32 g = blockIdx.x, lo = A.tr_base[g], n = A.tr_base[g + 1] - lo;
  for (u32 i = threadIdx.x; i < n; i += blockDim.x) s_t[i] = A.tmp_tr_id[lo + i];
  __syncthreads();
  for (u32 i = threadIdx.x; i < n; i += blockDim.x) {
    const u32 t = s_t[i];
    u32 rank = 0;
    u32 j = 0;
    for (; j + 8 <= n; j += 8) {
      u32 k[8];
#pragma unroll
      for (int q = 0; q < 8; q++) k[q] = s_t[j + q];
#pragma unroll
      for (int q = 0; q < 8; q++) rank += k[q] < t ? 1u : 0u;
    }
    for (; j < n; j++) rank += s_t[j] < t ? 1u : 0u;
    A.local_of[t] = rank;
    const u64 m = (u64)lo + rank;
    A.tr_id[m] = t; A.single[m] = A.single_all[t]; A.eff_m[m] = A.eff[t];
  }
}
constexpr int EML_RANK_BLOCK = 1024;
__global__ __launch_bounds__(EML_RANK_BLOCK) void k_eml_rank_rows(kamd_em_local::BuildArgs A) {
  extern __shared__ __attribute__((aligned(16))) unsigned char gb_smem[];
  const u32 g = blockIdx.x, lo = A.row_base[g], n = A.row_base[g + 1] - lo;
  u64* s_k = reinterpret_cast<u64*>(gb_smem);
  u32* s_e = reinterpret_cast<u32*>(s_k + n);
  for (u32 i = threadIdx.x; i < n; i += blockDim.x) { s_k[i] = A.row_key[lo + i]; s_e[i] = A.row_e[lo + i]; }
  __syncthreads();
  for (u32 i = threadIdx.x; i < n; i += blockDim.x) {
    const u64 key = s_k[i];
    const u32 e = s_e[i];
    u32 rank = 0;
    u32 j = 0;
    for (; j + 8 <= n; j += 8) {
      u64 k[8];
#pragma unroll
      for (int q = 0; q < 8; q++) k[q] = s_k[j + q];
      bool tie = false;
#pragma unroll
      for (int q = 0; q < 8; q++) { rank += k[q] < key ? 1u : 0u; tie = tie || k[q] == key; }
      if (tie) {
#pragma unroll
        for (int q = 0; q < 8; q++) rank += (k[q] == key && s_e[j + q] < e) ? 1u : 0u;
      }
    }
    for (; j < n; j++) { const u64 kj = s_k[j]; rank += (kj < key || (kj == key && s_e[j] < e)) ? 1u : 0u; }
    const u32 rn = lo + rank;
    A.row_new[e] = rn;
    A.row_e_final[rn] = e;
    A.len_new[rn] = (u32)(A.ec_off[(u64)e + 1] - A.ec_off[e]);
    A.cw[rn] = (u64)A.counts[e] | ((u64)(A.wcounts ? A.wcounts[e] : A.counts[e]) << 32);
  }
}
__global__ __launch_bounds__(BLOCK) void k_eml_group_build(kamd_em_local::BuildArgs A) {
  extern __shared__ __attribute__((aligned(16))) unsigned char gb_smem[];
  __shared__ u32 s_w[BLOCK / 64];
  const u32 g = blockIdx.x, tid = threadIdx.x, nthr = blockDim.x;
  const u32 r0 = A.row_base[g], nR = A.row_base[g + 1] - r0, t0 = A.tr_base[g], nT = A.tr_base[g + 1] - t0;
  const u64 z0 = A.nz_base[g];
  const u32 nnz = (u32)(A.nz_base[g + 1] - z0);
  u32* s_roff = reinterpret_cast<u32*>(gb_smem);
  u32* s_coff = s_roff + (nR + 1);
  u32* s_cur = s_coff + (nT + 1);
  uint16_t* s_erow = reinterpret_cast<uint16_t*>(s_cur + nT);
  uint16_t* s_ecol = s_erow + ((nnz + 1) & ~1u);
  for (u32 r = tid; r < nR; r += nthr) s_roff[r] = A.len_new[r0 + r];
  for (u32 l = tid; l <= nT; l += nthr) s_coff[l] = 0;
  for (u32 l = tid; l < nT; l += nthr) s_cur[l] = 0;
  __syncthreads();
  eml_block_excl_scan(s_roff, nR, s_w);
  for (u32 r = tid; r <= nR; r += nthr) A.row_ptr[(u64)r0 + r + g] = s_roff[r];
  for (u32 r = tid; r < nR; r += nthr) {
    const u32 e = A.row_e_final[r0 + r];
    const u64 a = A.ec_off[e];
    const u32 len = s_roff[r + 1] - s_roff[r], at = s_roff[r];
    for (u32 j = 0; j < len; j++) {
      const u32 l = A.local_of[A.ec_ids[a + j]];
      A.row_tr[z0 + at + j] = (uint16_t)l;
      atomicAdd(&s_coff[l], 1u);
    }
  }
  __syncthreads();
  eml_block_excl_scan(s_coff, nT, s_w);
  for (u32 l = tid; l <= nT; l += nthr) A.col_ptr[(u64)t0 + l + g] = s_coff[l];
  for (u32 r = tid; r < nR; r += nthr) {
    const u32 len = s_roff[r + 1] - s_roff[r], at = s_roff[r];
    for (u32 j = 0; j < len; j++) {
      const u32 l = A.row_tr[z0 + at + j];
      const u32 p = s_coff[l] + atomicAdd(&s_cur[l], 1u);
      s_erow[p] = (uint16_t)r; s_ecol[p] = (uint16_t)l;
    }
  }
  __syncthreads();
  for (u32 p = tid; p < nnz; p += nthr) {
    const u32 l = s_ecol[p], v = s_erow[p];
    const u32 lo = s_coff[l], hi = s_coff[l + 1];
    u32 rank = 0;
    u32 q = lo;
    for (; q + 8 <= hi; q += 8) {
      u32 k[8];
#pragma unroll
      for (int i = 0; i < 8; i++) k[i] = s_erow[q + i];
#pragma unroll
      for (int i = 0; i < 8; i++) rank += k[i] < v ? 1u : 0u;
    }
    for (; q < hi; q++) rank += s_erow[q] < v ? 1u : 0u;
    A.col_row[z0 + lo + rank] = (uint16_t)v;
  }
}
struct CompStats { u32 max_nnz, max_rows, max_tr, pad; };
__global__ void k_comp_stats(const u32* __restrict__ c_nnz, const u32* __restrict__ c_rows, const u32* __restrict__ c_tr, u64 T, u32* stats) {
  u32 v0 = 0, v1 = 0, v2 = 0;
  for (u64 r = (u64)blockIdx.x * blockDim.x + threadIdx.x; r < T; r += (u64)gridDim.x * blockDim.x) {
    v0 = max(v0, c_nnz[r]);
    if (c_rows) v1 = max(v1, c_rows[r]);
    if (c_tr) v2 = max(v2, c_tr[r]);
  }
  __shared__ u32 red[3][BLOCK / 64];
#pragma unroll
  for (int d = 32; d > 0; d >>= 1) { v0 = max(v0, (u32)__shfl_down(v0, d, 64)); v1 = max(v1, (u32)__shfl_down(v1, d, 64)); v2 = max(v2, (u32)__shfl_down(v2, d, 64)); }
  const int w = threadIdx.x >> 6;
  if (lane_id() == 0) { red[0][w] = v0; red[1][w] = v1; red[2][w] = v2; }
  __syncthreads();
  if (threadIdx.x == 0) {
    for (int i = 1; i < (int)(blockDim.x >> 6); i++) { v0 = max(v0, red[0][i]); v1 = max(v1, red[1][i]); v2 = max(v2, red[2][i]); }
    if (v0 > __atomic_load_n(&stats[0], __ATOMIC_RELAXED)) atomicMax(&stats[0], v0);
    if (v1 > __atomic_load_n(&stats[1], __ATOMIC_RELAXED)) atomicMax(&stats[1], v1);
    if (v2 > __atomic_load_n(&stats[2], __ATOMIC_RELAXED)) atomicMax(&stats[2], v2);
  }
}
constexpr unsigned COMP_STATS_BLOCKS = 256;
int cc_labels(kamd_ctx* c, const u64* d_ec_off, const u32* d_ec_ids, u64 n_ecs, u64 T) {
  if (int rc = c->pt_label.ensure((T + 1) * sizeof(u32), 0, c->stream)) return rc;
  hipLaunchKernelGGL(k_cc_init, dim3(grid_for(T, BLOCK)), dim3(BLOCK), 0, c->stream, c->pt_label.as<u32>(), T);
  if (n_ecs) hipLaunchKernelGGL(k_cc_union, dim3(grid_for(n_ecs, BLOCK)), dim3(BLOCK), 0, c->stream, d_ec_off, d_ec_ids, n_ecs, c->pt_label.as<u32>());
  hipLaunchKernelGGL(k_cc_flatten, dim3(grid_for(T, BLOCK)), dim3(BLOCK), 0, c->stream, c->pt_label.as<u32>(), T);
  HIPC(hipGetLastError());
  return 0;
}
int em_local_setup_device(kamd_ctx* c, const u64* d_ec_off, const u32* d_ec_ids, const u32* d_counts, const u32* d_wcounts, u64 n_ecs, u64 nnz,
                          const double* eff_lens, u64 T, u64 budget, u64 target, kamd_em_local::Plan* P, EmLocalDev* dev,
                          kamd_em_local::BuildArgs* args_out = nullptr, u32 small_limit = 0, u64 target_small = 0, bool host_maps = true,
                          CompStats* comp_out = nullptr) {
  namespace L = kamd_em_local;
  if (nnz >= (1ULL << 32) || T >= 0xFFFFFFF0ULL || n_ecs >= 0xFFFFFFF0ULL) return 1;
  if (int rc = c->pt_label.ensure((T + 1) * sizeof(u32), 0, c->stream)) return rc;
  if (int rc = c->pt_hist.ensure(64, 0, c->stream)) return rc;
  if (!c->labels_override) if (int rc = cc_labels(c, d_ec_off, d_ec_ids, n_ecs, T)) return rc;
  Carver t1;
  const size_t o_inm = t1.take(T + 8), o_sall = t1.take(T * 8 + 8), o_cn = t1.take(T * 4 + 8), o_cr = t1.take(T * 4 + 8), o_ct = t1.take(T * 4 + 8);
  const size_t o_cum = t1.take((T + 2) * 8), o_loc = t1.take(T * 4 + 8), o_eff = t1.take(T * 8 + 8), o_rnew = t1.take(n_ecs * 4 + 8);
  const size_t o_cs = t1.take(small_limit ? T * 4 + 8 : 8), o_cb = t1.take(small_limit ? T * 4 + 8 : 8), o_cumb = t1.take(small_limit ? (T + 2) * 8 : 8);
  const u64 ng_max = nnz / std::max<u64>(1, target) + 2 + (small_limit ? nnz / std::max<u64>(1, target_small) + 2 : 0);
  const size_t o_gr = t1.take(ng_max * 4 + 8), o_gt = t1.take(ng_max * 4 + 8), o_gn = t1.take(ng_max * 4 + 8), o_rf = t1.take(ng_max * 4 + 8),
               o_tf = t1.take(ng_max * 4 + 8);
  if (int rc = c->eml_tmp.ensure(t1.off, 0, c->stream)) return rc;
  char* tb = (char*)c->eml_tmp.p;
  HIPC(hipMemsetAsync(tb, 0, o_cum, c->stream));
  HIPC(hipMemcpyAsync(tb + o_eff, eff_lens, T * 8, hipMemcpyHostToDevice, c->stream));
  L::BuildArgs A{};
  A.ec_off = (const uint64_t*)d_ec_off; A.ec_ids = d_ec_ids; A.counts = d_counts; A.wcounts = d_wcounts; A.n_ecs = n_ecs;
  A.eff = (const double*)(tb + o_eff); A.T = T; A.label = c->labels_override ? c->labels_override : c->pt_label.as<u32>(); A.target_nnz = std::max<u64>(1, target);
  A.in_multi = (uint8_t*)(tb + o_inm); A.single_all = (double*)(tb + o_sall); A.c_nnz = (u32*)(tb + o_cn); A.c_rows = (u32*)(tb + o_cr);
  A.c_tr = (u32*)(tb + o_ct); A.cum_nnz = (const uint64_t*)(tb + o_cum); A.local_of = (u32*)(tb + o_loc); A.row_new = (u32*)(tb + o_rnew);
  hipLaunchKernelGGL(k_eml_step<0>, dim3(grid_for(n_ecs, BLOCK)), dim3(BLOCK), 0, c->stream, A, n_ecs);
  hipLaunchKernelGGL(k_eml_step<1>, dim3(grid_for(T, BLOCK)), dim3(BLOCK), 0, c->stream, A, T);
  CompStats cst{};
  HIPC(hipMemsetAsync(c->pt_hist.p, 0, sizeof(CompStats), c->stream));
  hipLaunchKernelGGL(k_comp_stats, dim3(std::min<unsigned>(grid_for(T, BLOCK), COMP_STATS_BLOCKS)), dim3(BLOCK), 0, c->stream, A.c_nnz, A.c_rows, A.c_tr, T, (u32*)c->pt_hist.p);
  HIPC(hipMemcpyAsync(&cst, c->pt_hist.p, sizeof(CompStats), hipMemcpyDeviceToHost, c->stream));
  u64 NZ = 0;
  u32 ng = 0;
  P->n_small = 0;
  if (small_limit) {
    A.small_limit = small_limit; A.c_small = (u32*)(tb + o_cs); A.c_big = (u32*)(tb + o_cb);
    hipLaunchKernelGGL(k_eml_step<9>, dim3(grid_for(T, BLOCK)), dim3(BLOCK), 0, c->stream, A, T);
    if (int rc = exclusive_scan(c, A.c_small, T, (u64*)(tb + o_cum), (u64*)(tb + o_cum) + T)) return rc;
    if (int rc = exclusive_scan(c, A.c_big, T, (u64*)(tb + o_cumb), (u64*)(tb + o_cumb) + T)) return rc;
    u64 nz2[2] = {0, 0};
    HIPC(hipMemcpyAsync(&nz2[0], (u64*)(tb + o_cum) + T, 8, hipMemcpyDeviceToHost, c->stream));
    HIPC(hipMemcpyAsync(&nz2[1], (u64*)(tb + o_cumb) + T, 8, hipMemcpyDeviceToHost, c->stream));
    HIPC(hipStreamSynchronize(c->stream));
    NZ = nz2[0] + nz2[1];
    if (comp_out) *comp_out = cst;
    if (NZ == 0) return 1;
    A.target_big = A.target_nnz; A.target_nnz = std::max<u64>(1, target_small); A.cum_big = (const uint64_t*)(tb + o_cumb);
    A.ng_small = nz2[0] ? (u32)((nz2[0] - 1) / A.target_nnz + 1) : 0u;
    ng = A.ng_small + (nz2[1] ? (u32)((nz2[1] - 1) / A.target_big + 1) : 0u);
    P->n_small = A.ng_small;
  } else {
    if (int rc = exclusive_scan(c, A.c_nnz, T, (u64*)(tb + o_cum), (u64*)(tb + o_cum) + T)) return rc;
    HIPC(hipMemcpyAsync(&NZ, (u64*)(tb + o_cum) + T, 8, hipMemcpyDeviceToHost, c->stream));
    HIPC(hipStreamSynchronize(c->stream));
    if (comp_out) *comp_out = cst;
    if (NZ == 0) return 1;
    ng = (u32)((NZ - 1) / A.target_nnz + 1);
  }
  if (comp_out) *comp_out = cst;
  if ((u64)ng > ng_max) return kamd::fail(-105, "kamd_em_run: component-local EM: more groups than entries allow");
  A.n_groups = ng;
  HIPC(hipMemsetAsync(tb + o_gr, 0, t1.off - o_gr, c->stream));
  A.g_rows = (u32*)(tb + o_gr); A.g_tr = (u32*)(tb + o_gt); A.g_nnz = (u32*)(tb + o_gn); A.row_fill = (u32*)(tb + o_rf); A.tr_fill = (u32*)(tb + o_tf);
  hipLaunchKernelGGL(k_eml_step<2>, dim3(grid_for(T, BLOCK)), dim3(BLOCK), 0, c->stream, A, T);
  std::vector<u32> g_rows(ng), g_tr(ng), g_nnz(ng);
  HIPC(hipMemcpyAsync(g_rows.data(), A.g_rows, ng * 4, hipMemcpyDeviceToHost, c->stream));
  HIPC(hipMemcpyAsync(g_tr.data(), A.g_tr, ng * 4, hipMemcpyDeviceToHost, c->stream));
  HIPC(hipMemcpyAsync(g_nnz.data(), A.g_nnz, ng * 4, hipMemcpyDeviceToHost, c->stream));
  HIPC(hipStreamSynchronize(c->stream));
  P->n_groups = ng; P->T = T; P->max_group_bytes = 0;
  P->row_base.assign(ng + 1, 0); P->tr_base.assign(ng + 1, 0); P->nz_base.assign(ng + 1, 0);
  for (u32 g = 0; g < ng; g++) {
    const u64 gb = L::group_bytes(g_nnz[g], g_rows[g], g_tr[g]);
    if (g_rows[g] > 65535 || g_tr[g] > 65535 || gb > budget) return 1;
    P->max_group_bytes = std::max<uint64_t>(P->max_group_bytes, gb);
    P->row_base[g + 1] = P->row_base[g] + g_rows[g]; P->tr_base[g + 1] = P->tr_base[g] + g_tr[g]; P->nz_base[g + 1] = P->nz_base[g] + g_nnz[g];
  }
  const u64 R = P->row_base[ng], M = P->tr_base[ng];
  if (P->nz_base[ng] != NZ) return kamd::fail(-105, "kamd_em_run: component-local EM: group sizes do not add up");
  Carver pv;
  const size_t p_rb = pv.take((ng + 1) * 4), p_tb = pv.take((ng + 1) * 4), p_zb = pv.take((ng + 1) * 8);
  const size_t p_rp = pv.take((R + ng) * 4 + 8), p_cp = pv.take((M + ng) * 4 + 8), p_rt = pv.take(NZ * 2 + 8), p_cr = pv.take(NZ * 2 + 8);
  const size_t p_cw = pv.take(R * 8 + 8), p_sg = pv.take(M * 8 + 8), p_ef = pv.take(M * 8 + 8), p_id = pv.take(M * 4 + 8);
  const size_t p_len = pv.take(R * 4 + 8), p_rabs = pv.take((R + 2) * 8), p_cc = pv.take(M * 4 + 8), p_cf = pv.take(M * 4 + 8), p_cabs = pv.take((M + 2) * 8);
  const size_t p_tt = pv.take(M * 4 + 8), p_rk = pv.take(R * 8 + 8), p_crt = pv.take(NZ * 2 + 8), p_ec = pv.take(NZ * 4 + 8), p_re = pv.take(R * 4 + 8), p_ref = pv.take(R * 4 + 8);
  if (int rc = c->pm_a.ensure(pv.off, 0, c->stream)) return rc;
  char* pb = (char*)c->pm_a.p;
  HIPC(hipMemcpyAsync(pb + p_rb, P->row_base.data(), (ng + 1) * 4, hipMemcpyHostToDevice, c->stream));
  HIPC(hipMemcpyAsync(pb + p_tb, P->tr_base.data(), (ng + 1) * 4, hipMemcpyHostToDevice, c->stream));
  HIPC(hipMemcpyAsync(pb + p_zb, P->nz_base.data(), (ng + 1) * 8, hipMemcpyHostToDevice, c->stream));
  HIPC(hipMemsetAsync(pb + p_cc, 0, p_cabs - p_cc, c->stream));
  A.row_base = (const u32*)(pb + p_rb); A.tr_base = (const u32*)(pb + p_tb); A.nz_base = (const uint64_t*)(pb + p_zb);
  A.row_ptr = (u32*)(pb + p_rp); A.col_ptr = (u32*)(pb + p_cp); A.row_tr = (uint16_t*)(pb + p_rt); A.col_row = (uint16_t*)(pb + p_cr);
  A.cw = (uint64_t*)(pb + p_cw); A.single = (double*)(pb + p_sg); A.eff_m = (double*)(pb + p_ef); A.tr_id = (u32*)(pb + p_id);
  A.len_new = (u32*)(pb + p_len); A.row_abs = (const uint64_t*)(pb + p_rabs); A.col_cnt = (u32*)(pb + p_cc); A.col_fill = (u32*)(pb + p_cf);
  A.col_abs = (const uint64_t*)(pb + p_cabs);
  A.tmp_tr_id = (u32*)(pb + p_tt); A.row_key = (uint64_t*)(pb + p_rk); A.col_row_tmp = (uint16_t*)(pb + p_crt); A.ent_col = (u32*)(pb + p_ec); A.row_e = (u32*)(pb + p_re); A.row_e_final = (u32*)(pb + p_ref);
  size_t rk_lds = 0;
  for (u32 g = 0; g < ng; g++) rk_lds = std::max(rk_lds, std::max((size_t)g_tr[g] * 4, (size_t)g_rows[g] * 12) + 16);
  const bool lds_rank = rk_lds <= 150 * 1024;
  hipLaunchKernelGGL(k_eml_step<3>, dim3(grid_for(T, BLOCK)), dim3(BLOCK), 0, c->stream, A, T);
  if (lds_rank) {
    HIPC(hipFuncSetAttribute((const void*)k_eml_rank_tr, hipFuncAttributeMaxDynamicSharedMemorySize, (int)rk_lds));
    HIPC(hipFuncSetAttribute((const void*)k_eml_rank_rows, hipFuncAttributeMaxDynamicSharedMemorySize, (int)rk_lds));
    hipLaunchKernelGGL(k_eml_rank_tr, dim3(ng), dim3(BLOCK), rk_lds, c->stream, A);
  } else hipLaunchKernelGGL(k_eml_step<10>, dim3(grid_for(M, BLOCK)), dim3(BLOCK), 0, c->stream, A, M);
  if (A.n_groups <= (u32)RG_BINS) hipLaunchKernelGGL(k_eml_rows_g, dim3(grid_for(n_ecs, RG_BLOCK * RG_PER)), dim3(RG_BLOCK), 0, c->stream, A);
  else hipLaunchKernelGGL(k_eml_step<4>, dim3(grid_for(n_ecs, BLOCK)), dim3(BLOCK), 0, c->stream, A, n_ecs);
  if (lds_rank) hipLaunchKernelGGL(k_eml_rank_rows, dim3(ng), dim3(EML_RANK_BLOCK), rk_lds, c->stream, A);
  else hipLaunchKernelGGL(k_eml_step<11>, dim3(grid_for(R, BLOCK)), dim3(BLOCK), 0, c->stream, A, R);
  size_t gb_lds = 0;
  for (u32 g = 0; g < ng; g++)
    gb_lds = std::max(gb_lds, ((size_t)g_rows[g] + 1 + 2 * (size_t)g_tr[g] + 1) * 4 + (((size_t)g_nnz[g] + 1) & ~(size_t)1) * 4 + 16);
  if (gb_lds <= 150 * 1024) {
    HIPC(hipFuncSetAttribute((const void*)k_eml_group_build, hipFuncAttributeMaxDynamicSharedMemorySize, (int)gb_lds));
    hipLaunchKernelGGL(k_eml_group_build, dim3(ng), dim3(BLOCK), gb_lds, c->stream, A);
  } else {
    if (int rc = exclusive_scan(c, A.len_new, R, (u64*)(pb + p_rabs), (u64*)(pb + p_rabs) + R)) return rc;
    hipLaunchKernelGGL(k_eml_step<5>, dim3(grid_for(n_ecs, BLOCK)), dim3(BLOCK), 0, c->stream, A, n_ecs);
    if (int rc = exclusive_scan(c, A.col_cnt, M, (u64*)(pb + p_cabs), (u64*)(pb + p_cabs) + M)) return rc;
    hipLaunchKernelGGL(k_eml_step<6>, dim3(grid_for(M, BLOCK)), dim3(BLOCK), 0, c->stream, A, M);
    hipLaunchKernelGGL(k_eml_step<7>, dim3(grid_for(ng, BLOCK)), dim3(BLOCK), 0, c->stream, A, (u64)ng);
    hipLaunchKernelGGL(k_eml_step<8>, dim3(grid_for(n_ecs, BLOCK)), dim3(BLOCK), 0, c->stream, A, n_ecs);
    hipLaunchKernelGGL(k_eml_step<12>, dim3(grid_for(NZ, BLOCK)), dim3(BLOCK), 0, c->stream, A, NZ);
  }
  HIPC(hipGetLastError());
  if (host_maps) {
    P->tr_id.resize(M); P->single_all.resize(T);
    if (M) HIPC(hipMemcpyAsync(P->tr_id.data(), A.tr_id, M * 4, hipMemcpyDeviceToHost, c->stream));
    HIPC(hipMemcpyAsync(P->single_all.data(), A.single_all, T * 8, hipMemcpyDeviceToHost, c->stream));
    HIPC(hipStreamSynchronize(c->stream));
  }
  *dev = EmLocalDev{(const u32*)(pb + p_rb), (const u32*)(pb + p_tb), (const u64*)(pb + p_zb), (const u32*)(pb + p_rp), (const u32*)(pb + p_cp),
                    (const uint16_t*)(pb + p_rt), (const uint16_t*)(pb + p_cr), (const u64*)(pb + p_cw), (const double*)(pb + p_sg),
                    (const double*)(pb + p_ef), (const u32*)(pb + p_id)};
  if (args_out) *args_out = A;
  return 0;
}
constexpr u32 SELL_NONE = 0xFFFFFFFFu;
__global__ void k_sell_maps(kamd_em_local::BuildArgs A, SellBuild B, u32* row_final, u32* mslot) {
  const u64 i = (u64)blockIdx.x * blockDim.x + threadIdx.x;
  if (i < A.n_ecs) {
    const u64 a = A.ec_off[i], b = A.ec_off[i + 1];
    u32 rf = SELL_NONE;
    if (b - a >= 2) {
      const u32 rn = A.row_new[i];
      const u32 g = sell_group_of(B.row_base, B.n_groups, rn);
      rf = B.row_base[g] + B.rnew[rn];
    }
    row_final[i] = rf;
  }
  if (i < A.T) {
    u32 ms = SELL_NONE;
    if (A.in_multi[i]) {
      const u32 g = kamd_em_local::eml_group_of(A, A.label[i]);
      const u32 old_m = B.tr_base[g] + A.local_of[i];
      ms = B.tr_base[g] + B.cnew[old_m];
    }
    mslot[i] = ms;
  }
}
__global__ void k_sell_refresh(const u64* __restrict__ ec_off, const u32* __restrict__ ec_ids, const u32* __restrict__ counts,
                               const u32* __restrict__ wcounts, u64 n_ecs, const double* __restrict__ eff, u64 T,
                               const u32* __restrict__ row_final, const u32* __restrict__ mslot, u64* cw, double* single_m,
                               double* eff_m, double* single_all) {
  const u64 i = (u64)blockIdx.x * blockDim.x + threadIdx.x;
  if (i < n_ecs) {
    const u64 a = ec_off[i], b = ec_off[i + 1];
    if (b - a == 1) {
      const u32 t = ec_ids[a];
      single_all[t] = (double)counts[i];
      if (mslot[t] != SELL_NONE) single_m[mslot[t]] = (double)counts[i];
    } else if (b - a >= 2) cw[row_final[i]] = (u64)counts[i] | ((u64)wcounts[i] << 32);
  }
  if (i < T && mslot[i] != SELL_NONE) eff_m[mslot[i]] = eff[i];
}

struct GiDesc { int* hist; int stopped; int pad; };
__global__ void k_gi_set_desc(GiDesc* d, EmsPrev prev, int* hist) {
  const int i = (int)threadIdx.x;
  bool stop = false;
  if (prev.hist && i < 64) { const int h = i < prev.n ? prev.hist[i] : 1; stop = i < prev.n && h == 0 && prev.base + i > prev.min_rounds; }
  const u64 m = __ballot(stop);
  if (i == 0) { d->hist = hist; d->stopped = m != 0 ? 1 : 0; d->pad = 0; }
}
__device__ __forceinline__ bool gi_stopped(const GiDesc* d, int*) { return d->stopped != 0; }
struct GiColEmit {
  const double* alpha_cur; const double* a_cur; const double* single; const double* eff; double* alpha_nx; double* a_nx; int* ch; int clamp;
  struct Ctx { double al, at, sg, ef; };
  __device__ __forceinline__ Ctx load(u32 m) const { return Ctx{alpha_cur[m], a_cur[m], single[m], eff[m]}; }
  __device__ __forceinline__ void finish(u32 m, const Ctx& x, double acc) const {
    const double al = (clamp && x.al < 1e-7 / 10.0) ? 0.0 : x.al;
    const double nx = x.sg + x.at * acc;
    if (nx > 1e-2 && (fabs(nx - al) / nx) > 1e-2) ++*ch;
    alpha_nx[m] = nx;
    a_nx[m] = nx / x.ef;
  }
};
__device__ __forceinline__ void gi_count_changes(int ch, int* lds_ch, int* slot) {
  if (threadIdx.x == 0) *lds_ch = 0;
  __syncthreads();
  if (__ballot(ch != 0)) {
    int wsum = ch;
#pragma unroll
    for (int d = 32; d > 0; d >>= 1) wsum += __shfl_down(wsum, d, 64);
    if (lane_id() == 0) atomicAdd(lds_ch, wsum);
  }
  __syncthreads();
  if (threadIdx.x == 0 && *lds_ch && slot) atomicAdd(slot, *lds_ch);
}
template <int K, int PRE, bool WIN>
__global__ __launch_bounds__(PM_BLOCK) void k_gi_rows(PmArgs A, const double* a_src, const GiDesc* desc) {
  __shared__ double lds_sums[(PM_BLOCK / 64) * PM_LDS_SLOTS];
  __shared__ int s_stop;
  const u32 c = __builtin_amdgcn_readfirstlane(blockIdx.x * (PM_BLOCK / 64) + (threadIdx.x >> 6));
  PmWave<K> w;
  if (c < A.rows.n_chunks) pm_wave_load<K>(A.rows, c, w);
  if (gi_stopped(desc, &s_stop)) return;
  if (c >= A.rows.n_chunks) return;
  const PmRowEmit em{A.cw, A.g};
  pm_wave_pass<K, PRE, WIN>(A.rows, c, w, PmSrcGlobal{a_src}, lds_sums + (threadIdx.x >> 6) * PM_LDS_SLOTS, em);
}
// ... 753 lines not shown
                             const double* __restrict__ before, u64 T, int have_final, double* out_alpha, double* out_abz) {
  const u64 t = (u64)blockIdx.x * blockDim.x + threadIdx.x;
  if (t >= T) return;
  const u32 ms = mslot[t];
  const double sa = single_all[t];
  out_alpha[t] = ms != 0xFFFFFFFFu ? fin[ms] : sa;
  out_abz[t] = have_final ? (ms != 0xFFFFFFFFu ? before[ms] : sa) : 0.0;
}
__global__ void k_em_publish(EmsPrev prev) {
  __shared__ int s_stop;
  (void)ems_prev_stopped(prev, &s_stop);
}
int em_sell_drive_async(kamd_ctx* c, EmSellGpu& B, const SellCache& K, u64 T, int n_iter, int min_rounds, double* alpha_out, double* abz_out, int* rounds_out) {
  const int CH = EML_MAX_ROUNDS;
  if (n_iter <= 0) {
    hipLaunchKernelGGL(k_em_scatter, dim3(grid_for(T, BLOCK)), dim3(BLOCK), 0, c->stream, K.mslot, K.single_all, B.d_alpha, B.d_alpha, T, 0, B.d_out, B.d_out + T);
    if (B.gi) hipLaunchKernelGGL(k_gi_scatter, dim3(grid_for(T, BLOCK)), dim3(BLOCK), 0, c->stream, T, B.gi->plan.mflag, B.gi->plan.mpos, B.gi->G_al[0], B.gi->G_al[0], 0,
                                 B.d_out, B.d_out + T);
    HIPC(hipGetLastError());
    std::vector<double> tmp(2 * T);
    HIPC(hipMemcpyAsync(tmp.data(), B.d_out, 2 * T * 8, hipMemcpyDeviceToHost, c->stream));
    HIPC(hipStreamSynchronize(c->stream));
    memcpy(alpha_out, tmp.data(), T * 8);
    if (abz_out) memcpy(abz_out, tmp.data() + T, T * 8);
    *rounds_out = 0;
    return 0;
  }
  const int n_chunks = std::max(1, (n_iter + CH - 1) / CH);
  const size_t hist_ints = (size_t)(n_chunks + 1) * CH;
  const size_t need = hist_ints * 4 + 256 + 2 * T * 8 + 256;
  if (c->em_pin_bytes < need) {
    if (c->em_pin) { HIPC(hipStreamSynchronize(c->stream)); HIPC(hipHostFree(c->em_pin)); c->em_pin = nullptr; c->em_pin_bytes = 0; }
    HIPC(hipHostMalloc(&c->em_pin, need, hipHostMallocMapped));
    c->em_pin_bytes = need;
  }
  int* h_hist = (int*)c->em_pin;
  int* h_seq = h_hist + hist_ints;
  double* h_out = (double*)((char*)c->em_pin + hist_ints * 4 + 256);
  void* dp = nullptr;
  HIPC(hipHostGetDevicePointer(&dp, c->em_pin, 0));
  int* d_hh = (int*)dp; int* d_seq = d_hh + hist_ints;
  __atomic_store_n(h_seq, 0, __ATOMIC_RELEASE);
  HIPC(hipMemsetAsync(B.d_hist, 0, (size_t)n_chunks * CH * sizeof(int), c->stream));
  double* al[2] = {B.d_alpha, B.d_ck_alpha};
  double* av[2] = {B.d_a, B.d_ck_a};
  auto prev_of = [&](int k) {
    if (k == 0) return EmsPrev{};
    const int pb = (k - 1) * CH;
    return EmsPrev{B.d_hist + (size_t)(k - 1) * CH, std::min(CH, n_iter - pb), pb, min_rounds, d_hh + (size_t)(k - 1) * CH, d_seq, k};
  };
  const char* clk_path = getenv("KAMD_EM_CLK");
  long long* d_clk = nullptr; size_t clk_words = 0;
  if (clk_path && *clk_path && B.P.n_groups > B.P.n_small) {
    clk_words = (size_t)(B.P.n_groups - B.P.n_small) * (EMS_MAX_BLOCK / 64) * EMS_CLK_WORDS;
    if (int rc = c->em_clk.ensure(clk_words * 8, 0, c->stream)) return rc;
    d_clk = c->em_clk.as<long long>();
    HIPC(hipMemsetAsync(d_clk, 0, clk_words * 8, c->stream));
  }
  int launched = 0, decided = 0, stop = -1;
  bool published_last = false;
  for (;;) {
    while (launched < n_chunks && launched < decided + 2) {
      const int k = launched, base = k * CH, n = std::min(CH, n_iter - base);
      if (int rc = B.launch(n, 0, al[k & 1], av[k & 1], al[(k + 1) & 1], av[(k + 1) & 1], B.d_hist + (size_t)k * CH, prev_of(k), k == 0 ? d_clk : nullptr))
        return kamd::fail(rc, "kamd_em_run: the component-local EM failed to launch");
      ++launched;
    }
    if (launched == n_chunks && decided == n_chunks - 1 && !published_last) {
      hipLaunchKernelGGL(k_em_publish, dim3(1), dim3(64), 0, c->stream, prev_of(n_chunks));
      HIPC(hipGetLastError());
      published_last = true;
    }
    {
      const auto t0 = std::chrono::steady_clock::now();
      for (u64 spin = 1;; spin++) {
        if (__atomic_load_n(h_seq, __ATOMIC_ACQUIRE) >= decided + 1) break;
        if ((spin & 4095) == 0) {
          const hipError_t q = hipStreamQuery(c->stream);
          if (q == hipSuccess) {
            if (__atomic_load_n(h_seq, __ATOMIC_ACQUIRE) >= decided + 1) break;
            return kamd::fail(-104, "kamd_em_run: the change counts of a chunk never arrived");
          }
          if (q != hipErrorNotReady) return kamd::fail(-104, std::string("kamd_em_run: ") + hipGetErrorString(q));
          if (std::chrono::steady_clock::now() - t0 > std::chrono::seconds(120)) return kamd::fail(-104, "kamd_em_run: timed out waiting for a chunk of rounds");
        }
        __builtin_ia32_pause();
      }
    }
    const int base = decided * CH, n = std::min(CH, n_iter - base);
    const int* hh = h_hist + (size_t)decided * CH;
    for (int i = 0; i < n; i++) if (hh[i] == 0 && base + i > min_rounds) { stop = base + i; break; }
    if (stop >= 0) break;
    if (++decided == n_chunks) break;
  }
  const double* fin; const double* before;
  int rounds;
  const bool have_final = stop >= 0;
  if (have_final) {
    const int s = decided, base = s * CH;
    if (int rc = B.launch(stop - base + 1, 0, al[s & 1], av[s & 1], al[(s + 1) & 1], av[(s + 1) & 1], nullptr, EmsPrev{})) return kamd::fail(rc, "kamd_em_run: replay failed to launch");
    if (int rc = B.launch(1, 1, al[(s + 1) & 1], av[(s + 1) & 1], al[s & 1], av[s & 1], nullptr, EmsPrev{})) return kamd::fail(rc, "kamd_em_run: final round failed to launch");
    before = al[(s + 1) & 1]; fin = al[s & 1];
    rounds = stop + 1;
  } else {
    fin = al[n_chunks & 1]; before = fin;
    rounds = n_iter;
  }
  hipLaunchKernelGGL(k_em_scatter, dim3(grid_for(T, BLOCK)), dim3(BLOCK), 0, c->stream, K.mslot, K.single_all, fin, before, T, have_final ? 1 : 0, B.d_out, B.d_out + T);
  if (B.gi) hipLaunchKernelGGL(k_gi_scatter, dim3(grid_for(T, BLOCK)), dim3(BLOCK), 0, c->stream, T, B.gi->plan.mflag, B.gi->plan.mpos, B.gi->G_al[B.gi_par(fin)],
                               B.gi->G_al[B.gi_par(before)], have_final ? 1 : 0, B.d_out, B.d_out + T);
  HIPC(hipGetLastError());
  HIPC(hipMemcpyAsync(h_out, B.d_out, 2 * T * 8, hipMemcpyDeviceToHost, c->stream));
  HIPC(hipStreamSynchronize(c->stream));
  memcpy(alpha_out, h_out, T * 8);
  if (abz_out) memcpy(abz_out, h_out + T, T * 8);
  if (d_clk) {
    std::vector<long long> hc(clk_words);
    HIPC(hipMemcpy(hc.data(), d_clk, clk_words * 8, hipMemcpyDeviceToHost));
    if (FILE* f = fopen(clk_path, "wb")) {
      const long long hdr[4] = {(long long)(B.P.n_groups - B.P.n_small), EMS_MAX_BLOCK / 64, EMS_CLK_WORDS, B.block};
      fwrite(hdr, 8, 4, f); fwrite(hc.data(), 8, clk_words, f); fclose(f);
    }
  }
  *rounds_out = rounds;
  return 0;
}
int em_sell_setup_device(kamd_ctx* c, const u64* d_ec_off, const u32* d_ec_ids, const u32* d_counts, const u32* d_wcounts, u64 n_ecs, u64 nnz,
                         const double* eff_lens, u64 T, u64 lds_budget, u64 target, kamd_em_sell::Plan* P, EmSellDev* dev, SellCache* cache,
                         u32 small_limit = 0, u64 target_small = 0, u64 small_budget = 0, bool host_maps = true, CompStats* comp_out = nullptr) {
  namespace S = kamd_em_sell;
  kamd_em_local::Plan C;
  EmLocalDev cd{};
  kamd_em_local::BuildArgs A{};
  if (int rc = em_local_setup_device(c, d_ec_off, d_ec_ids, d_counts, d_wcounts, n_ecs, nnz, eff_lens, T, ~0ULL, target, &C, &cd, &A, small_limit, target_small, host_maps, comp_out)) return rc;
  const u32 ng = C.n_groups;
  const u64 R = C.row_base[ng], M = C.tr_base[ng];
  if (R >= 0xFFFFFFF0ULL || M >= 0xFFFFFFF0ULL) return 1;
  for (u32 g = 0; g < ng; g++)
    if (C.row_base[g + 1] - C.row_base[g] >= S::SELL_PAD || C.tr_base[g + 1] - C.tr_base[g] >= S::SELL_PAD) return 1;
  Carver tv;
  const size_t o_rlen = tv.take(R * 4 + 8), o_clen = tv.take(M * 4 + 8), o_rnew = tv.take(R * 4 + 8), o_cnew = tv.take(M * 4 + 8);
  const size_t o_rlane = tv.take(R * 4 + 8), o_clane = tv.take(M * 4 + 8), o_rvl = tv.take(R * 4 + 8), o_cvl = tv.take(M * 4 + 8), o_gsz = tv.take((size_t)ng * 16 + 16);
  if (int rc = c->ems_tmp.ensure(tv.off, 0, c->stream)) return rc;
  char* tb = (char*)c->ems_tmp.p;
  SellBuild B{};
  B.row_base = cd.row_base; B.tr_base = cd.tr_base; B.row_ptr = cd.row_ptr; B.col_ptr = cd.col_ptr; B.row_tr = cd.row_tr; B.col_row = cd.col_row;
  B.nz_base = cd.nz_base; B.cw = cd.cw; B.single = cd.single; B.eff = cd.eff; B.tr_id = cd.tr_id; B.n_groups = ng; B.R = (u32)R; B.M = (u32)M;
  B.cap = (u32)std::min(64, std::max(1, c->tune.em_split_len));
  B.rlen = (u32*)(tb + o_rlen); B.clen = (u32*)(tb + o_clen); B.rnew = (u32*)(tb + o_rnew); B.cnew = (u32*)(tb + o_cnew);
  B.rlane = (u32*)(tb + o_rlane); B.clane = (u32*)(tb + o_clane); B.rvl = (u32*)(tb + o_rvl); B.cvl = (u32*)(tb + o_cvl); B.gsz = (u32*)(tb + o_gsz);
  const u64 nseg = std::max(R, M);
  hipLaunchKernelGGL(k_sell_lens, dim3(grid_for(nseg, BLOCK)), dim3(BLOCK), 0, c->stream, B);
  hipLaunchKernelGGL(k_sell_sizes, dim3(grid_for(2 * (u64)ng, SELL_BUILD_WAVES)), dim3(64 * SELL_BUILD_WAVES), 0, c->stream, B);
  std::vector<u32> gsz((size_t)ng * 4);
  HIPC(hipMemcpyAsync(gsz.data(), B.gsz, (size_t)ng * 16, hipMemcpyDeviceToHost, c->stream));
  HIPC(hipStreamSynchronize(c->stream));
  P->n_groups = ng; P->n_small = C.n_small; P->T = T; P->row_base = C.row_base; P->tr_base = C.tr_base; P->single_all = C.single_all;
  P->rslice_base.assign(ng + 1, 0); P->cslice_base.assign(ng + 1, 0); P->rell_base.assign(ng + 1, 0); P->cell_base.assign(ng + 1, 0);
  P->max_group_bytes = 0; P->max_small_bytes = 0;
  for (u32 g = 0; g < ng; g++) {
    const u64 gb = S::group_bytes(C.row_base[g + 1] - C.row_base[g], C.tr_base[g + 1] - C.tr_base[g], gsz[4 * g], gsz[4 * g + 2], gsz[4 * g + 1], gsz[4 * g + 3]);
    if (g < P->n_small) {
      if (gb > small_budget) return 2;
      P->max_small_bytes = std::max<uint64_t>(P->max_small_bytes, gb);
    } else {
      if (gb > lds_budget) return 1;
      P->max_group_bytes = std::max<uint64_t>(P->max_group_bytes, gb);
    }
    P->rslice_base[g + 1] = P->rslice_base[g] + gsz[4 * g]; P->rell_base[g + 1] = P->rell_base[g] + gsz[4 * g + 1];
    P->cslice_base[g + 1] = P->cslice_base[g] + gsz[4 * g + 2]; P->cell_base[g + 1] = P->cell_base[g] + gsz[4 * g + 3];
  }
  const u64 nrs = P->rslice_base[ng], ncs = P->cslice_base[ng], nru = P->rell_base[ng], ncu = P->cell_base[ng];
  Carver pv;
  const size_t p_rsb = pv.take((ng + 1) * 4), p_csb = pv.take((ng + 1) * 4), p_reb = pv.take((ng + 1) * 8), p_ceb = pv.take((ng + 1) * 8);
  const size_t p_rd = pv.take(nrs * 8 + 8), p_cdesc = pv.take(ncs * 8 + 8), p_re = pv.take(nru * 2 + 8), p_ce = pv.take(ncu * 2 + 8);
  const size_t p_cw = pv.take(R * 8 + 8), p_sg = pv.take(M * 8 + 8), p_ef = pv.take(M * 8 + 8), p_id = pv.take(M * 4 + 8);
  if (int rc = c->ems_plan.ensure(pv.off, 0, c->stream)) return rc;
  char* pb = (char*)c->ems_plan.p;
  HIPC(hipMemcpyAsync(pb + p_rsb, P->rslice_base.data(), (ng + 1) * 4, hipMemcpyHostToDevice, c->stream));
  HIPC(hipMemcpyAsync(pb + p_csb, P->cslice_base.data(), (ng + 1) * 4, hipMemcpyHostToDevice, c->stream));
  HIPC(hipMemcpyAsync(pb + p_reb, P->rell_base.data(), (ng + 1) * 8, hipMemcpyHostToDevice, c->stream));
  HIPC(hipMemcpyAsync(pb + p_ceb, P->cell_base.data(), (ng + 1) * 8, hipMemcpyHostToDevice, c->stream));
  HIPC(hipMemsetAsync(pb + p_re, 0xFF, nru * 2, c->stream));
  HIPC(hipMemsetAsync(pb + p_ce, 0xFF, ncu * 2, c->stream));
  B.rslice_base = (const u32*)(pb + p_rsb); B.cslice_base = (const u32*)(pb + p_csb); B.rell_base = (const u64*)(pb + p_reb); B.cell_base = (const u64*)(pb + p_ceb);
  B.rdesc = (u32*)(pb + p_rd); B.cdesc = (u32*)(pb + p_cdesc); B.rell = (uint16_t*)(pb + p_re); B.cell = (uint16_t*)(pb + p_ce);
  B.cw_new = (u64*)(pb + p_cw); B.single_new = (double*)(pb + p_sg); B.eff_new = (double*)(pb + p_ef); B.tr_id_new = (u32*)(pb + p_id);
  hipLaunchKernelGGL(k_sell_layout, dim3(grid_for(2 * (u64)ng, SELL_BUILD_WAVES)), dim3(64 * SELL_BUILD_WAVES), 0, c->stream, B);
  hipLaunchKernelGGL(k_sell_entries, dim3(grid_for(nseg, BLOCK)), dim3(BLOCK), 0, c->stream, B);
  HIPC(hipGetLastError());
  if (host_maps) {
    P->tr_id.resize(M);
    if (M) HIPC(hipMemcpyAsync(P->tr_id.data(), B.tr_id_new, M * 4, hipMemcpyDeviceToHost, c->stream));
  }
  Carver bv;
  const size_t b_rb = bv.take((ng + 1) * 4), b_tb = bv.take((ng + 1) * 4), b_rf = bv.take(n_ecs * 4 + 8), b_ms = bv.take(T * 4 + 8), b_sa = bv.take(T * 8 + 8),
               b_ef = bv.take(T * 8 + 8);
  if (int rc = c->ems_maps.ensure(bv.off, 0, c->stream)) return rc;
  char* mb = (char*)c->ems_maps.p;
  HIPC(hipMemcpyAsync(mb + b_rb, cd.row_base, (ng + 1) * 4, hipMemcpyDeviceToDevice, c->stream));
  HIPC(hipMemcpyAsync(mb + b_tb, cd.tr_base, (ng + 1) * 4, hipMemcpyDeviceToDevice, c->stream));
  hipLaunchKernelGGL(k_sell_maps, dim3(grid_for(std::max<u64>(n_ecs, T), BLOCK)), dim3(BLOCK), 0, c->stream, A, B, (u32*)(mb + b_rf), (u32*)(mb + b_ms));
  HIPC(hipMemcpyAsync(mb + b_sa, A.single_all, T * 8, hipMemcpyDeviceToDevice, c->stream));
  HIPC(hipGetLastError());
  HIPC(hipStreamSynchronize(c->stream));
  *dev = EmSellDev{(const u32*)(mb + b_rb), (const u32*)(mb + b_tb), B.rslice_base, B.cslice_base, B.rell_base, B.cell_base, B.rdesc, B.cdesc, B.rell, B.cell,
                   B.cw_new, B.single_new, B.eff_new};
  if (cache) { cache->row_final = (u32*)(mb + b_rf); cache->mslot = (u32*)(mb + b_ms); cache->single_all = (double*)(mb + b_sa); cache->d_eff = (double*)(mb + b_ef); }
  return 0;
}
}
namespace kamdi { void sell_cache_free(SellCache* k) { delete k; } }
namespace {
__global__ void k_hy_comp_nnz(const u64* __restrict__ ec_off, const u32* __restrict__ ec_ids, u64 n_ecs, const u32* __restrict__ label, u32* c_nnz) {
  const u64 e = (u64)blockIdx.x * blockDim.x + threadIdx.x;
  u32 root = 0xFFFFFFFFu, len = 0;
  if (e < n_ecs) {
    const u64 a = ec_off[e], b = ec_off[e + 1];
    if (b - a >= 2) { root = label[ec_ids[a]]; len = (u32)(b - a); }
  }
  const bool act = len != 0;
  const u64 am = __ballot(act);
  if (!am) return;
  const int leader = __ffsll((long long)am) - 1;
  const u32 lroot = (u32)__shfl((int)root, leader, 64);
  const bool with_leader = act && root == lroot;
  u32 v = with_leader ? len : 0u;
#pragma unroll
  for (int d = 32; d > 0; d >>= 1) v += (u32)__shfl_down((int)v, d, 64);
  if (lane_id() == 0 && v) atomicAdd(&c_nnz[lroot], v);
  if (act && !with_leader) atomicAdd(&c_nnz[root], len);
}
__global__ void k_hy_sizes(const u64* __restrict__ ec_off, const u32* __restrict__ ec_ids, u64 n_ecs, const u32* __restrict__ label,
                           const u32* __restrict__ c_nnz, u32 lim, u32* flag_s, u32* len_s, u32* flag_g, u32* len_g) {
  const u64 e = (u64)blockIdx.x * blockDim.x + threadIdx.x;
  if (e >= n_ecs) return;
  const u64 a = ec_off[e], b = ec_off[e + 1];
  const bool any = b > a;
  const bool giant = any && c_nnz[label[ec_ids[a]]] > lim;
  flag_s[e] = any && !giant ? 1u : 0u; len_s[e] = any && !giant ? (u32)(b - a) : 0u;
  flag_g[e] = giant ? 1u : 0u; len_g[e] = giant ? (u32)(b - a) : 0u;
}
__global__ void k_hy_single(const u64* __restrict__ ec_off, const u32* __restrict__ ec_ids, const u32* __restrict__ counts, u64 n_ecs, double* single_all) {
  const u64 e = (u64)blockIdx.x * blockDim.x + threadIdx.x;
  if (e >= n_ecs) return;
  const u64 a = ec_off[e];
  if (ec_off[e + 1] - a == 1) single_all[ec_ids[a]] = (double)counts[e];
}
int hy_streams(kamd_ctx* c) {
  if (!c->hy_giant_stream) {
    HIPC(hipStreamCreateWithFlags(&c->hy_giant_stream, hipStreamNonBlocking));
    HIPC(hipEventCreateWithFlags(&c->hy_ev_giant, hipEventDisableTiming));
    HIPC(hipEventCreateWithFlags(&c->hy_ev_sell, hipEventDisableTiming));
  }
  return 0;
}
int em_sell_plan_search(kamd_ctx* c, const u64* d_ec_off, const u32* d_ec_ids, const u32* d_counts, const u32* d_wcounts, u64 n_ecs, u64 nnz,
                        const double* eff_lens, u64 T, u64 lds_budget, int n_cus, bool multi, SellCache& K, CompStats* cst) {
  u32 small = c->tune.em_small_nnz > 0 ? (u32)c->tune.em_small_nnz : 0u;
  const bool auto_div = c->tune.em_group_div < 0;
  const u64 ncu = (u64)std::max(1, n_cus);
  const u64 div0 = auto_div ? std::max<u64>(1, (nnz + ncu * 10000 - 1) / (ncu * 10000)) : (u64)c->tune.em_group_div;
  int prc = 1, tries = 0;
  for (u64 div = div0; div <= 1024 && prc >= 1; ) {
    const u64 target = std::max<u64>(1024, (nnz + ncu * div - 1) / (ncu * div));
    prc = em_sell_setup_device(c, d_ec_off, d_ec_ids, d_counts, d_wcounts, n_ecs, nnz, eff_lens, T, lds_budget, target, &K.P, &K.dev, &K, small, small,
                               24 * 1024, multi, cst);
    if (prc == 2) { small = 0; continue; }
    if (prc <= 0 || target == 1024) break;
    if (cst && ((u64)cst->max_nnz * 4 + (u64)cst->max_rows * 16 > lds_budget || cst->max_rows > 65000 || cst->max_tr > 65000)) break;
    if (++tries >= 5) break;
    div = auto_div && tries == 1 ? div + 1 : div * 2;
  }
  return prc == 2 ? 1 : prc;
}
int em_hybrid_setup(kamd_ctx* c, const u64* d_ec_off, const u32* d_ec_ids, const u32* d_counts, const u32* d_wcounts, u64 n_ecs, u64 nnz,
                    const double* eff_lens, u64 T, u64 lds_budget, SellCache& K, bool first_try = false, bool host_maps = false) {
  if (n_ecs == 0 || nnz >= (1ULL << 32) || T >= 0xFFFFFFF0ULL || n_ecs >= 0xFFFFFFF0ULL) return 1;
  GiantPart& G = K.G;
  G.drop_graphs();
  if (int rc = cc_labels(c, d_ec_off, d_ec_ids, n_ecs, T)) return rc;
  Carver cv;
  const size_t o_lab = cv.take(T * 4 + 8);
  const size_t o_cn = cv.take(T * 4 + 8), o_fs = cv.take(n_ecs * 4 + 8), o_ls = cv.take(n_ecs * 4 + 8), o_fg = cv.take(n_ecs * 4 + 8), o_lg = cv.take(n_ecs * 4 + 8);
  const size_t o_rs = cv.take((n_ecs + 2) * 8), o_zs = cv.take((n_ecs + 2) * 8), o_rg = cv.take((n_ecs + 2) * 8), o_zg = cv.take((n_ecs + 2) * 8);
  const size_t o_off_s = cv.take((n_ecs + 2) * 8), o_off_g = cv.take((n_ecs + 2) * 8), o_ids_s = cv.take(nnz * 4 + 8), o_ids_g = cv.take(nnz * 4 + 8);
  const size_t o_cnt_s = cv.take(n_ecs * 4 + 8), o_cnt_g = cv.take(n_ecs * 4 + 8), o_wc_s = cv.take(n_ecs * 4 + 8), o_wc_g = cv.take(n_ecs * 4 + 8);
  if (int rc = c->hy_sub.ensure(cv.off, 0, c->stream)) return rc;
  char* hb = (char*)c->hy_sub.p;
  u32* c_nnz = (u32*)(hb + o_cn);
  u32* flag_s = (u32*)(hb + o_fs); u32* len_s = (u32*)(hb + o_ls); u32* flag_g = (u32*)(hb + o_fg); u32* len_g = (u32*)(hb + o_lg);
  u64* rpos_s = (u64*)(hb + o_rs); u64* zpos_s = (u64*)(hb + o_zs); u64* rpos_g = (u64*)(hb + o_rg); u64* zpos_g = (u64*)(hb + o_zg);
  u64* off_s = (u64*)(hb + o_off_s); u64* off_g = (u64*)(hb + o_off_g); u32* ids_s = (u32*)(hb + o_ids_s); u32* ids_g = (u32*)(hb + o_ids_g);
  u32* cnt_s = (u32*)(hb + o_cnt_s); u32* cnt_g = (u32*)(hb + o_cnt_g); u32* wc_s = (u32*)(hb + o_wc_s); u32* wc_g = (u32*)(hb + o_wc_g);
  u32* label = (u32*)(hb + o_lab);
  HIPC(hipMemcpyAsync(label, c->pt_label.p, T * 4, hipMemcpyDeviceToDevice, c->stream));
  HIPC(hipMemsetAsync(c_nnz, 0, T * 4, c->stream));
  hipLaunchKernelGGL(k_hy_comp_nnz, dim3(grid_for(n_ecs, BLOCK)), dim3(BLOCK), 0, c->stream, d_ec_off, d_ec_ids, n_ecs, label, c_nnz);
  HIPC(hipGetLastError());
  {
    CompStats cs{};
    if (int rc = c->pt_hist.ensure(64, 0, c->stream)) return rc;
    HIPC(hipMemsetAsync(c->pt_hist.p, 0, sizeof(CompStats), c->stream));
    hipLaunchKernelGGL(k_comp_stats, dim3(std::min<unsigned>(grid_for(T, BLOCK), COMP_STATS_BLOCKS)), dim3(BLOCK), 0, c->stream, c_nnz, (const u32*)nullptr, (const u32*)nullptr, T, (u32*)c->pt_hist.p);
    HIPC(hipMemcpyAsync(&cs, c->pt_hist.p, sizeof(CompStats), hipMemcpyDeviceToHost, c->stream));
    HIPC(hipStreamSynchronize(c->stream));
    c->last_em_max_comp_nnz = cs.max_nnz;
    if (cs.max_nnz == 0) return 1;
  }
  u32 lim = c->tune.em_giant_nnz > 0 ? (u32)c->tune.em_giant_nnz : 6000u;
  if (c->last_em_max_comp_nnz <= lim && first_try) return 1;
  for (int attempt = 0; attempt < 4; attempt++, lim = std::max(lim / 2, 8u)) {
    hipLaunchKernelGGL(k_hy_sizes, dim3(grid_for(n_ecs, BLOCK)), dim3(BLOCK), 0, c->stream, d_ec_off, d_ec_ids, n_ecs, label, c_nnz, lim,
                       flag_s, len_s, flag_g, len_g);
    if (int rc = exclusive_scan(c, flag_s, n_ecs, rpos_s, rpos_s + n_ecs)) return rc;
    if (int rc = exclusive_scan(c, len_s, n_ecs, zpos_s, zpos_s + n_ecs)) return rc;
    if (int rc = exclusive_scan(c, flag_g, n_ecs, rpos_g, rpos_g + n_ecs)) return rc;
    if (int rc = exclusive_scan(c, len_g, n_ecs, zpos_g, zpos_g + n_ecs)) return rc;
    u64 tot[4] = {0, 0, 0, 0};
    HIPC(hipMemcpyAsync(&tot[0], rpos_s + n_ecs, 8, hipMemcpyDeviceToHost, c->stream));
    HIPC(hipMemcpyAsync(&tot[1], zpos_s + n_ecs, 8, hipMemcpyDeviceToHost, c->stream));
    HIPC(hipMemcpyAsync(&tot[2], rpos_g + n_ecs, 8, hipMemcpyDeviceToHost, c->stream));
    HIPC(hipMemcpyAsync(&tot[3], zpos_g + n_ecs, 8, hipMemcpyDeviceToHost, c->stream));
    HIPC(hipStreamSynchronize(c->stream));
    const u64 n_s = tot[0], nnz_s = tot[1], n_g = tot[2], nnz_g = tot[3];
    if (n_g == 0) continue;
    hipLaunchKernelGGL(k_part_copy, dim3(grid_for(n_ecs, BLOCK)), dim3(BLOCK), 0, c->stream, d_ec_off, d_ec_ids, d_counts, d_wcounts, n_ecs, flag_s, rpos_s, zpos_s,
                       off_s, ids_s, cnt_s, wc_s);
    hipLaunchKernelGGL(k_part_copy, dim3(grid_for(n_ecs, BLOCK)), dim3(BLOCK), 0, c->stream, d_ec_off, d_ec_ids, d_counts, d_wcounts, n_ecs, flag_g, rpos_g, zpos_g,
                       off_g, ids_g, cnt_g, wc_g);
    HIPC(hipMemcpyAsync(off_s + n_s, zpos_s + n_ecs, 8, hipMemcpyDeviceToDevice, c->stream));
    HIPC(hipMemcpyAsync(off_g + n_g, zpos_g + n_ecs, 8, hipMemcpyDeviceToDevice, c->stream));
    HIPC(hipGetLastError());
    if (int rc = hy_streams(c)) return rc;
    const int sell_cus = c->n_cus;
    CompStats cst{};
    c->labels_override = label;
    int prc = n_s ? em_sell_plan_search(c, off_s, ids_s, cnt_s, wc_s, n_s, nnz_s, eff_lens, T, lds_budget, sell_cus, host_maps, K, &cst) : 1;
    c->labels_override = nullptr;
    if (prc < 0) return prc;
    if (prc == 1 && cst.max_nnz == 0) {
      K.P = kamd_em_sell::Plan{};
      K.P.T = T; K.P.row_base.assign(1, 0); K.P.tr_base.assign(1, 0);
      K.dev = EmSellDev{};
      Carver mv;
      const size_t m_ms = mv.take(T * 4 + 8), m_sa = mv.take(T * 8 + 8);
      if (int rc = c->hy_maps.ensure(mv.off, 0, c->stream)) return rc;
      char* mb = (char*)c->hy_maps.p;
      HIPC(hipMemsetAsync(mb + m_ms, 0xFF, T * 4, c->stream));
      HIPC(hipMemsetAsync(mb + m_sa, 0, T * 8, c->stream));
      if (n_s) hipLaunchKernelGGL(k_hy_single, dim3(grid_for(n_s, BLOCK)), dim3(BLOCK), 0, c->stream, off_s, ids_s, cnt_s, n_s, (double*)(mb + m_sa));
      HIPC(hipGetLastError());
      K.mslot = (u32*)(mb + m_ms); K.single_all = (double*)(mb + m_sa); K.row_final = nullptr; K.d_eff = nullptr;
      if (host_maps) {
        K.P.single_all.resize(T);
        HIPC(hipMemcpyAsync(K.P.single_all.data(), K.single_all, T * 8, hipMemcpyDeviceToHost, c->stream));
        HIPC(hipStreamSynchronize(c->stream));
      }
      prc = 0;
    }
// ... 560 lines not shown
```

scratch/em_clk_report.py:

```python
import sys
import numpy as np

raw = np.fromfile(sys.argv[1], dtype=np.int64)
ng, nw, words, block = (int(x) for x in raw[:4])
c = raw[4:].reshape(ng, nw, words)
waves = block // 64
c = c[:, :waves]
ok = c[:, 0, 0] != 0
c = c[ok]
print(f"groups {ng} (with clocks {ok.sum()}), wavefronts per group {waves}")
rows = c[:, :, 1] - c[:, :, 0]; b1 = c[:, :, 2] - c[:, :, 1]; cols = c[:, :, 3] - c[:, :, 2]; b2 = c[:, :, 4] - c[:, :, 3]
tot = c[:, :, 4].max(1) - c[:, :, 0].min(1)
nrs = c[:, 0, 5] & 0xFFFF; ncs = (c[:, 0, 5] >> 16) & 0xFFFF
nru = c[:, 0, 6] & 0xFFFFFFFF; ncu = (c[:, 0, 6] >> 32) & 0xFFFFFFFF
wall = c[:, 0, 7]
def q(x): return f"mean {x.mean():9.1f}  p10 {np.percentile(x,10):8.0f}  p50 {np.percentile(x,50):8.0f}  p90 {np.percentile(x,90):8.0f}  max {x.max():8.0f}"
print("round, shader clocks      ", q(tot))
print("round, wall ticks (10 ns) ", q(wall))
print("rows pass, slowest wave   ", q(rows.max(1)))
print("rows pass, mean wave      ", q(rows.mean(1)))
print("barrier 1, shortest wait  ", q(b1.min(1)))
print("cols pass, slowest wave   ", q(cols.max(1)))
print("cols pass, mean wave      ", q(cols.mean(1)))
print("barrier 2, shortest wait  ", q(b2.min(1)))
print("row slices / group        ", q(nrs)); print("col slices / group        ", q(ncs))
print("row stream u16 / group    ", q(nru)); print("col stream u16 / group    ", q(ncu))
print("waves with a row slice    ", q(np.minimum(nrs, waves))); print("waves with a col slice    ", q(np.minimum(ncs, waves)))
if words >= 16:
    for name, a in (("cols", 8), ("rows", 12)):
        if name == "rows":
            st, sm, wd, fn = c[:, :, 12], c[:, :, 13], c[:, :, 14], c[:, :, 15]
        else:
            st, sm, wd, fn = c[:, :, 8], c[:, :, 9], c[:, :, 10], c[:, :, 11]
        has = st != 0
        width = (wd & 0xFFFF)[has]; meta = ((wd >> 16) & 1)[has]
        t_sum = (sm - st)[has]; t_fin = (fn - sm)[has]
        print(f"{name}: first slices {has.sum()}, with split lanes {meta.mean():.2f}")
        for lo, hi in ((1, 4), (5, 8), (9, 16), (17, 24), (25, 32), (33, 64)):
            sel = (width >= lo) & (width <= hi)
            if sel.any():
                print(f"  width {lo:2d}-{hi:2d}: n {sel.sum():6d}  sums {t_sum[sel].mean():8.1f} clk ({(t_sum[sel] / np.maximum(width[sel], 1)).mean():6.1f} / trip)  scan+finish {t_fin[sel].mean():8.1f}"
                      f"  (split {t_fin[sel & (meta == 1)].mean() if (sel & (meta == 1)).any() else 0:8.1f}, plain {t_fin[sel & (meta == 0)].mean() if (sel & (meta == 0)).any() else 0:8.1f})")
```

Baseline: 1137.

## Prefetch SELL group tables before stop check and pin plan readbacks

Precomputes a packed per-group record of bases and sizes so each EM group block loads its metadata in four vector loads instead of many dependent scalar loads. It issues the first batch of global loads for alpha, weights, descriptors and index streams into registers before the early-stop check and barrier, then copies them to LDS with 8-wide vectorized unpadding, which overlaps load latency with setup. Plan-building readbacks now go through a reusable pinned host buffer, with the group arrays fetched in one contiguous copy. The change adds register pressure from the staging struct, pads the index buffers for over-reads, and extends clock instrumentation.

```diff
diff --git a/__graft_entry__.py b/__graft_entry__.py
--- a/__graft_entry__.py
+++ b/__graft_entry__.py
@@ -20,6 +20,7 @@
     subprocess.check_call(["make", "-C", os.path.join(ROOT, "tests", "emu_inflate")], env=env)
     subprocess.check_call(["make", "-C", os.path.join(ROOT, "tests", "emu_readec")], env=env)
     subprocess.check_call(["make", "-C", os.path.join(ROOT, "tests", "emu_bustag")], env=env)
+    subprocess.check_call(["make", "-C", os.path.join(ROOT, "tests", "emu_sell")], env=env)
     if os.path.exists("/root/reference/src/main.cpp"):
         subprocess.check_call(["make", "-C", os.path.join(ROOT, "oracle"), "-j8", "ref"], env=env)
         subprocess.check_call(["make", "-C", os.path.join(ROOT, "oracle"), "ref_bound"], env=env)
diff --git a/kallisto_amd/csrc/kamd_ctx.hip b/kallisto_amd/csrc/kamd_ctx.hip
--- a/kallisto_amd/csrc/kamd_ctx.hip
+++ b/kallisto_amd/csrc/kamd_ctx.hip
@@ -152,6 +152,7 @@
   if (c->em_ev_fork) (void)hipEventDestroy(c->em_ev_fork);
   if (c->em_ev_join) (void)hipEventDestroy(c->em_ev_join);
   if (c->em_pin) (void)hipHostFree(c->em_pin);
+  if (c->plan_pin) (void)hipHostFree(c->plan_pin);
   if (c->state_pin) (void)hipHostFree(c->state_pin);
   c->em_clk.release();
   if (c->hy_giant_stream) { (void)hipStreamSynchronize(c->hy_giant_stream); (void)hipStreamDestroy(c->hy_giant_stream); }
diff --git a/kallisto_amd/csrc/kamd_dev.h b/kallisto_amd/csrc/kamd_dev.h
--- a/kallisto_amd/csrc/kamd_dev.h
+++ b/kallisto_amd/csrc/kamd_dev.h
@@ -269,6 +269,7 @@
   hipStream_t em_stream = nullptr;
   hipStream_t em_side_stream = nullptr; hipEvent_t em_ev_fork = nullptr, em_ev_join = nullptr;
   void* em_pin = nullptr; size_t em_pin_bytes = 0;
+  void* plan_pin = nullptr; size_t plan_pin_bytes = 0;
   DBuf em_clk;
   DBuf hy_sub, hy_a, hy_b, hy_x, hy_maps;
   DBuf hy_gb[6];
diff --git a/kallisto_amd/csrc/kamd_em.hip b/kallisto_amd/csrc/kamd_em.hip
--- a/kallisto_amd/csrc/kamd_em.hip
+++ b/kallisto_amd/csrc/kamd_em.hip
@@ -939,6 +939,7 @@
   const u32* row_base; const u32* tr_base; const u32* rslice_base; const u32* cslice_base; const u64* rell_base; const u64* cell_base;
   const u32* rdesc; const u32* cdesc; const uint16_t* rell; const uint16_t* cell;
   const u64* cw; const double* single; const double* eff;
+  const u32* grec;
 };
 constexpr int EMS_MAX_BLOCK = 1024;
 template <int EXP>
@@ -984,17 +985,106 @@
   if constexpr (EXP != 0) { if (sink == 0xFFFFFFFFu) S += 1.0; }
   return S;
 }
-constexpr int EMS_CLK_ROUND = 8, EMS_CLK_WORDS = 16;
-template <bool WAVE_TEAM, int EXP = 0>
-__device__ __forceinline__ void ems_group_rounds(const EmSellDev& P, u32 g, unsigned char* smem, u32 tid, u32 nthr, const double* alpha, const double* a,
+struct EmsBases { u32 r0, nR, t0, nT, rs0, nrs, cs0, ncs; u64 re0, ce0; u32 nru, ncu; };
+constexpr int EMS_GREC_WORDS = 16;
+__device__ __forceinline__ EmsBases ems_bases(const EmSellDev& P, u32 g) {
+  const uint4* r = reinterpret_cast<const uint4*>(P.grec + (size_t)g * EMS_GREC_WORDS);
+  const uint4 q0 = r[0], q1 = r[1], q2 = r[2], q3 = r[3];
+  EmsBases B;
+  B.r0 = q0.x; B.nR = q0.y; B.t0 = q0.z; B.nT = q0.w;
+  B.rs0 = q1.x; B.nrs = q1.y; B.cs0 = q1.z; B.ncs = q1.w;
+  B.re0 = (u64)q2.x | ((u64)q2.y << 32); B.ce0 = (u64)q2.z | ((u64)q2.w << 32);
+  B.nru = q3.x; B.ncu = q3.y;
+  return B;
+}
+__global__ void k_sell_group_rec(EmSellDev P, u32 n_groups, u32* grec) {
+  const u32 g = blockIdx.x * blockDim.x + threadIdx.x;
+  if (g >= n_groups) return;
+  const u32 r0 = P.row_base[g], t0 = P.tr_base[g], rs0 = P.rslice_base[g], cs0 = P.cslice_base[g];
+  const u64 re0 = P.rell_base[g], ce0 = P.cell_base[g];
+  uint4* r = reinterpret_cast<uint4*>(grec + (size_t)g * EMS_GREC_WORDS);
+  r[0] = make_uint4(r0, P.row_base[g + 1] - r0, t0, P.tr_base[g + 1] - t0);
+  r[1] = make_uint4(rs0, P.rslice_base[g + 1] - rs0, cs0, P.cslice_base[g + 1] - cs0);
+  r[2] = make_uint4((u32)re0, (u32)(re0 >> 32), (u32)ce0, (u32)(ce0 >> 32));
+  r[3] = make_uint4((u32)(P.rell_base[g + 1] - re0), (u32)(P.cell_base[g + 1] - ce0), 0u, 0u);
+}
+static_assert((2 * kamd_em_sell::SELL_META_WORDS) % 8 == 0 && (4 * kamd_em_sell::SELL_LANES) % 8 == 0, "index streams are fetched eight entries at a time");
+struct EmsLds { double* al; double* a; double* single; double* eff; u64* cw; u32* rdesc; u32* cdesc; uint16_t* rell; uint16_t* cell; };
+template <int TR> struct EmsStage {
+  double al[TR], a[TR], single[TR], eff[TR];
+  u64 cw[TR], rd, cd;
+  uint4 re[TR], ce[TR];
+};
+template <class T> __device__ __forceinline__ T ems_ld(const T* p, u32 i, u32 n) { return p[i < n ? i : 0u]; }
+__device__ __forceinline__ u32 ems_unpad2(u32 w, u32 zz) {
+  typedef unsigned short us2 __attribute__((ext_vector_type(2)));
+  const us2 one = {1, 1};
+  const us2 m = __builtin_elementwise_min((us2)(__builtin_bit_cast(us2, w) + one), one) - one;
+  const u32 mm = __builtin_bit_cast(u32, m);
+  return (w & ~mm) | (zz & mm);
+}
+__device__ __forceinline__ void ems_put8(uint16_t* dst, u32 i, uint4 v, u32 zero) {
+  const u32 zz = zero * 0x00010001u;
+  u64* d = reinterpret_cast<u64*>(dst) + 2 * (size_t)i;
+  d[0] = (u64)ems_unpad2(v.x, zz) | ((u64)ems_unpad2(v.y, zz) << 32);
+  d[1] = (u64)ems_unpad2(v.z, zz) | ((u64)ems_unpad2(v.w, zz) << 32);
+}
+template <int TR> __device__ __forceinline__ void ems_stage_issue(const EmSellDev& P, const EmsBases& B, const double* alpha, const double* a, u32 tid, u32 nthr, u32 trip0, EmsStage<TR>& S) {
+  const uint4* re = reinterpret_cast<const uint4*>(P.rell + B.re0);
+  const uint4* ce = reinterpret_cast<const uint4*>(P.cell + B.ce0);
+#pragma unroll
+  for (int u = 0; u < TR; u++) {
+    const u32 i = (trip0 + (u32)u) * nthr + tid;
+    S.re[u] = ems_ld(re, i, B.nru >> 3); S.ce[u] = ems_ld(ce, i, B.ncu >> 3);
+  }
+#pragma unroll
+  for (int u = 0; u < TR; u++) {
+    const u32 i = (trip0 + (u32)u) * nthr + tid;
+    S.al[u] = ems_ld(alpha + B.t0, i, B.nT); S.a[u] = ems_ld(a + B.t0, i, B.nT);
+    S.single[u] = ems_ld(P.single + B.t0, i, B.nT); S.eff[u] = ems_ld(P.eff + B.t0, i, B.nT);
+    S.cw[u] = ems_ld(P.cw + B.r0, i, B.nR);
+  }
+  const u32 i = (trip0 / TR) * nthr + tid;
+  S.rd = ems_ld(reinterpret_cast<const u64*>(P.rdesc) + B.rs0, i, B.nrs); S.cd = ems_ld(reinterpret_cast<const u64*>(P.cdesc) + B.cs0, i, B.ncs);
+}
+template <int TR> __device__ __forceinline__ void ems_stage_store(const EmsBases& B, const EmsLds& L, int clamp, u32 tid, u32 nthr, u32 trip0, const EmsStage<TR>& S) {
+#pragma unroll
+  for (int u = 0; u < TR; u++) {
+    const u32 i = (trip0 + (u32)u) * nthr + tid;
+    if (i < B.nT) {
+      double al = S.al[u], av = S.a[u];
+      if (clamp && al < 1e-7 / 10.0) { al = 0.0; av = 0.0; }
+      L.al[i] = al; L.a[i] = av; L.single[i] = S.single[u]; L.eff[i] = S.eff[u];
+    }
+    if (i < B.nR) L.cw[i] = S.cw[u];
+    if (i < (B.nru >> 3)) ems_put8(L.rell, i, S.re[u], B.nT);
+    if (i < (B.ncu >> 3)) ems_put8(L.cell, i, S.ce[u], B.nR);
+  }
+  const u32 i = (trip0 / TR) * nthr + tid;
+  if (i < B.nrs) reinterpret_cast<u64*>(L.rdesc)[i] = S.rd;
+  if (i < B.ncs) reinterpret_cast<u64*>(L.cdesc)[i] = S.cd;
+}
+template <int TR> __device__ __forceinline__ u32 ems_stage_trips(const EmsBases& B, u32 nthr) {
+  const u32 n8 = max(max(B.nT, B.nR), max(B.nru >> 3, B.ncu >> 3));
+  const u32 nd = max(B.nrs, B.ncs);
+  return max((n8 + nthr - 1) / nthr, TR * ((nd + nthr - 1) / nthr));
+}
+template <int TR> __device__ __forceinline__ void ems_stage_rest(const EmSellDev& P, const EmsBases& B, const EmsLds& L, const double* alpha, const double* a, int clamp, u32 tid, u32 nthr) {
+  const u32 trips = ems_stage_trips<TR>(B, nthr);
+  for (u32 t = TR; t < trips; t += TR) {
+    EmsStage<TR> S;
+    ems_stage_issue(P, B, alpha, a, tid, nthr, t, S);
+    ems_stage_store(B, L, clamp, tid, nthr, t, S);
+  }
+}
+constexpr int EMS_CLK_ROUND = 8, EMS_CLK_WORDS = 20;
+template <bool WAVE_TEAM, int EXP = 0, int TR = 1>
+__device__ __forceinline__ void ems_group_rounds(const EmSellDev& P, const EmsBases& B, const EmsStage<TR>& S0, unsigned char* smem, u32 tid, u32 nthr, const double* alpha, const double* a,
                                                  double* alpha_out, double* a_out, int n_rounds, int clamp, int* s_hist, long long* clk = nullptr) {
   namespace L = kamd_em_sell;
   const int lane = lane_id();
   const u32 wv = WAVE_TEAM ? 0u : (u32)__builtin_amdgcn_readfirstlane((int)(tid >> 6)), NW = WAVE_TEAM ? 1u : nthr >> 6;
-  const u32 r0 = P.row_base[g], nR = P.row_base[g + 1] - r0, t0 = P.tr_base[g], nT = P.tr_base[g + 1] - t0;
-  const u32 rs0 = P.rslice_base[g], nrs = P.rslice_base[g + 1] - rs0, cs0 = P.cslice_base[g], ncs = P.cslice_base[g + 1] - cs0;
-  const u64 re0 = P.rell_base[g], ce0 = P.cell_base[g];
-  const u32 nru = (u32)(P.rell_base[g + 1] - re0), ncu = (u32)(P.cell_base[g + 1] - ce0);
+  const u32 nR = B.nR, t0 = B.t0, nT = B.nT, nrs = B.nrs, ncs = B.ncs, nru = B.nru, ncu = B.ncu;
   auto team_sync = [] {
     if (WAVE_TEAM || EXP == 5) __builtin_amdgcn_fence(__ATOMIC_SEQ_CST, "wavefront");
     else __syncthreads();
@@ -1005,19 +1095,13 @@
   u64* s_cw = reinterpret_cast<u64*>(s_g + (nR + 1));
   u32* s_rdesc = reinterpret_cast<u32*>(s_cw + nR); u32* s_cdesc = s_rdesc + 2 * nrs;
   uint16_t* s_rell = reinterpret_cast<uint16_t*>(s_cdesc + 2 * ncs); uint16_t* s_cell = s_rell + ((nru + 1) & ~1u);
-  for (u32 i = tid; i < nT; i += nthr) {
-    double al = alpha[t0 + i], av = a[t0 + i];
-    if (clamp && al < 1e-7 / 10.0) { al = 0.0; av = 0.0; }
-    s_al0[i] = al; s_a0[i] = av; s_single[i] = P.single[t0 + i]; s_eff[i] = P.eff[t0 + i];
-  }
-  for (u32 i = tid; i < nR; i += nthr) s_cw[i] = P.cw[r0 + i];
-  for (u32 i = tid; i < 2 * nrs; i += nthr) s_rdesc[i] = P.rdesc[2 * (u64)rs0 + i];
-  for (u32 i = tid; i < 2 * ncs; i += nthr) s_cdesc[i] = P.cdesc[2 * (u64)cs0 + i];
-  for (u32 i = tid; i < nru; i += nthr) { const uint16_t v = P.rell[re0 + i]; s_rell[i] = v == (uint16_t)L::SELL_PAD ? (uint16_t)nT : v; }
-  for (u32 i = tid; i < ncu; i += nthr) { const uint16_t v = P.cell[ce0 + i]; s_cell[i] = v == (uint16_t)L::SELL_PAD ? (uint16_t)nR : v; }
+  const EmsLds lds{s_al0, s_a0, s_single, s_eff, s_cw, s_rdesc, s_cdesc, s_rell, s_cell};
+  ems_stage_store(B, lds, clamp, tid, nthr, 0, S0);
+  ems_stage_rest<TR>(P, B, lds, alpha, a, clamp, tid, nthr);
   if (tid == 0) { s_al0[nT] = s_a0[nT] = s_al1[nT] = s_a1[nT] = 0.0; s_g[nR] = 0.0; }
   team_sync();
   double* al = s_al0; double* av = s_a0; double* aln = s_al1; double* avn = s_a1;
+  if (clk && lane == 0) { clk[17] = clk[18] = clock64(); clk[19] = wall_clock64(); }
   for (int r = 0; r < n_rounds; r++) {
     const bool tick = clk && r == EMS_CLK_ROUND && lane == 0;
     long long w0 = 0;
@@ -1154,17 +1238,14 @@
   }
   return S;
 }
-template <int W, int NS>
-__device__ __forceinline__ void ems_group_rounds_reg(const EmSellDev& P, u32 g, unsigned char* smem, u32 tid, u32 nthr, const double* alpha, const double* a,
+template <int W, int NS, int TR>
+__device__ __forceinline__ void ems_group_rounds_reg(const EmSellDev& P, const EmsBases& B, const EmsStage<TR>& S0, unsigned char* smem, u32 tid, u32 nthr, const double* alpha, const double* a,
                                                      double* alpha_out, double* a_out, int n_rounds, int clamp, int* s_hist, long long* clk = nullptr) {
   namespace L = kamd_em_sell;
   constexpr bool TREE = W >= 8 || (W == 4 && NS == 2);
   const int lane = lane_id();
   const u32 wv = (u32)__builtin_amdgcn_readfirstlane((int)(tid >> 6)), NW = nthr >> 6;
-  const u32 r0 = P.row_base[g], nR = P.row_base[g + 1] - r0, t0 = P.tr_base[g], nT = P.tr_base[g + 1] - t0;
-  const u32 rs0 = P.rslice_base[g], nrs = P.rslice_base[g + 1] - rs0, cs0 = P.cslice_base[g], ncs = P.cslice_base[g + 1] - cs0;
-  const u64 re0 = P.rell_base[g], ce0 = P.cell_base[g];
-  const u32 nru = (u32)(P.rell_base[g + 1] - re0), ncu = (u32)(P.cell_base[g + 1] - ce0);
+  const u32 nR = B.nR, t0 = B.t0, nT = B.nT, nrs = B.nrs, ncs = B.ncs, nru = B.nru, ncu = B.ncu;
   double* s_a0 = reinterpret_cast<double*>(smem);
   double* s_g = s_a0 + (nT + 1);
   double* s_al0 = s_g + (nR + 1);
@@ -1174,18 +1255,12 @@
   uint16_t* s_rell = reinterpret_cast<uint16_t*>(s_cdesc + 2 * ncs); uint16_t* s_cell = s_rell + ((nru + 1) & ~1u);
   const u32 a_off = 0u, g_off = (nT + 1) * 8u;
   const bool near = g_off + (nR + 1) * 8u <= 0x10000u;
-  for (u32 i = tid; i < nT; i += nthr) {
-    double al = alpha[t0 + i], av = a[t0 + i];
-    if (clamp && al < 1e-7 / 10.0) { al = 0.0; av = 0.0; }
-    s_al0[i] = al; s_a0[i] = av; s_single[i] = P.single[t0 + i]; s_eff[i] = P.eff[t0 + i];
-  }
-  for (u32 i = tid; i < nR; i += nthr) s_cw[i] = P.cw[r0 + i];
-  for (u32 i = tid; i < 2 * nrs; i += nthr) s_rdesc[i] = P.rdesc[2 * (u64)rs0 + i];
-  for (u32 i = tid; i < 2 * ncs; i += nthr) s_cdesc[i] = P.cdesc[2 * (u64)cs0 + i];
-  for (u32 i = tid; i < nru; i += nthr) { const uint16_t v = P.rell[re0 + i]; s_rell[i] = v == (uint16_t)L::SELL_PAD ? (uint16_t)nT : v; }
-  for (u32 i = tid; i < ncu; i += nthr) { const uint16_t v = P.cell[ce0 + i]; s_cell[i] = v == (uint16_t)L::SELL_PAD ? (uint16_t)nR : v; }
+  const EmsLds lds{s_al0, s_a0, s_single, s_eff, s_cw, s_rdesc, s_cdesc, s_rell, s_cell};
+  ems_stage_store(B, lds, clamp, tid, nthr, 0, S0);
+  ems_stage_rest<TR>(P, B, lds, alpha, a, clamp, tid, nthr);
   if (tid == 0) { s_al0[nT] = s_a0[nT] = 0.0; s_g[nR] = 0.0; }
   __syncthreads();
+  if (clk && lane == 0) clk[17] = clock64();
   struct Own { u64 w[W]; u32 nq, seg, steps; int reach; bool has, meta, fin; };
   auto take = [&](const u32* desc, const uint16_t* ell, u32 s, u32 n_slices, u32 n_segs, u32 zero, u32 base_off) {
     Own o;
@@ -1231,6 +1306,7 @@
   }
   double* const al = s_al0; double* const av = s_a0;
   const unsigned char* const lds0 = smem;
+  if (clk && lane == 0) { clk[18] = clock64(); clk[19] = wall_clock64(); }
   for (int r = 0; r < n_rounds; r++) {
     const bool tick = clk && r == EMS_CLK_ROUND && lane == 0;
     long long w0 = 0;
@@ -1337,12 +1413,19 @@
   extern __shared__ __attribute__((aligned(16))) unsigned char ems_smem[];
   __shared__ int s_hist[EML_MAX_ROUNDS];
   __shared__ int s_stop;
+  long long t_in = 0, w_in = 0;
+  if constexpr (CLK) { t_in = clock64(); w_in = wall_clock64(); }
+  constexpr int TR = (W >= 8 || (W == 4 && NS == 2)) ? 2 : 1;
+  const EmsBases B = ems_bases(P, g_first + blockIdx.x);
+  EmsStage<TR> S0;
+  ems_stage_issue(P, B, alpha, a, threadIdx.x, blockDim.x, 0, S0);
   if (ems_prev_stopped(prev, &s_stop)) return;
   if (threadIdx.x < EML_MAX_ROUNDS) s_hist[threadIdx.x] = 0;
   __syncthreads();
   long long* my_clk = CLK ? clk + ((size_t)blockIdx.x * (EMS_MAX_BLOCK / 64) + (threadIdx.x >> 6)) * EMS_CLK_WORDS : nullptr;
-  if constexpr (W > 0) ems_group_rounds_reg<W, NS>(P, g_first + blockIdx.x, ems_smem, threadIdx.x, blockDim.x, alpha, a, alpha_out, a_out, n_rounds, clamp, s_hist, my_clk);
-  else ems_group_rounds<false, EXP>(P, g_first + blockIdx.x, ems_smem, threadIdx.x, blockDim.x, alpha, a, alpha_out, a_out, n_rounds, clamp, s_hist, my_clk);
+  if constexpr (W > 0) ems_group_rounds_reg<W, NS, TR>(P, B, S0, ems_smem, threadIdx.x, blockDim.x, alpha, a, alpha_out, a_out, n_rounds, clamp, s_hist, my_clk);
+  else ems_group_rounds<false, EXP, TR>(P, B, S0, ems_smem, threadIdx.x, blockDim.x, alpha, a, alpha_out, a_out, n_rounds, clamp, s_hist, my_clk);
+  if constexpr (CLK) { if (lane_id() == 0) { my_clk[16] = t_in; my_clk[19] -= w_in; } }
   __syncthreads();
   if (hist && (int)threadIdx.x < n_rounds && s_hist[threadIdx.x]) atomicAdd(&hist[threadIdx.x], s_hist[threadIdx.x]);
 }
@@ -1352,12 +1435,15 @@
   extern __shared__ __attribute__((aligned(16))) unsigned char ems_smem[];
   __shared__ int s_hist[EML_MAX_ROUNDS];
   __shared__ int s_stop;
+  const u32 team = (u32)__builtin_amdgcn_readfirstlane((int)(threadIdx.x >> 6));
+  const u32 g = blockIdx.x * EMS_WAVE_TEAMS + team;
+  const EmsBases B = ems_bases(P, g < n_small ? g : 0u);
+  EmsStage<2> S0;
+  ems_stage_issue(P, B, alpha, a, (u32)lane_id(), 64u, 0, S0);
   if (ems_prev_stopped(prev, &s_stop)) return;
   if (threadIdx.x < EML_MAX_ROUNDS) s_hist[threadIdx.x] = 0;
   __syncthreads();
-  const u32 team = (u32)__builtin_amdgcn_readfirstlane((int)(threadIdx.x >> 6));
-  const u32 g = blockIdx.x * EMS_WAVE_TEAMS + team;
-  if (g < n_small) ems_group_rounds<true>(P, g, ems_smem + (size_t)team * team_bytes, (u32)lane_id(), 64u, alpha, a, alpha_out, a_out, n_rounds, clamp, s_hist);
+  if (g < n_small) ems_group_rounds<true, 0, 2>(P, B, S0, ems_smem + (size_t)team * team_bytes, (u32)lane_id(), 64u, alpha, a, alpha_out, a_out, n_rounds, clamp, s_hist);
   __syncthreads();
   if (hist && (int)threadIdx.x < n_rounds && s_hist[threadIdx.x]) atomicAdd(&hist[threadIdx.x], s_hist[threadIdx.x]);
 }
@@ -1770,6 +1856,14 @@
   HIPC(hipGetLastError());
   return 0;
 }
+int plan_pin_ensure(kamd_ctx* c, size_t bytes) {
+  if (c->plan_pin_bytes >= bytes) return 0;
+  if (c->plan_pin) { HIPC(hipStreamSynchronize(c->stream)); HIPC(hipHostFree(c->plan_pin)); c->plan_pin = nullptr; c->plan_pin_bytes = 0; }
+  const size_t want = std::max<size_t>(bytes * 2, 64 * 1024);
+  HIPC(hipHostMalloc(&c->plan_pin, want, hipHostMallocDefault));
+  c->plan_pin_bytes = want;
+  return 0;
+}
 int em_local_setup_device(kamd_ctx* c, const u64* d_ec_off, const u32* d_ec_ids, const u32* d_counts, const u32* d_wcounts, u64 n_ecs, u64 nnz,
                           const double* eff_lens, u64 T, u64 budget, u64 target, kamd_em_local::Plan* P, EmLocalDev* dev,
                           kamd_em_local::BuildArgs* args_out = nullptr, u32 small_limit = 0, u64 target_small = 0, bool host_maps = true,
@@ -1797,10 +1891,13 @@
   A.c_tr = (u32*)(tb + o_ct); A.cum_nnz = (const uint64_t*)(tb + o_cum); A.local_of = (u32*)(tb + o_loc); A.row_new = (u32*)(tb + o_rnew);
   hipLaunchKernelGGL(k_eml_step<0>, dim3(grid_for(n_ecs, BLOCK)), dim3(BLOCK), 0, c->stream, A, n_ecs);
   hipLaunchKernelGGL(k_eml_step<1>, dim3(grid_for(T, BLOCK)), dim3(BLOCK), 0, c->stream, A, T);
+  if (int rc = plan_pin_ensure(c, 256)) return rc;
   CompStats cst{};
+  CompStats* const cst_pin = (CompStats*)c->plan_pin;
+  u64* const nz_pin = (u64*)((char*)c->plan_pin + 64);
   HIPC(hipMemsetAsync(c->pt_hist.p, 0, sizeof(CompStats), c->stream));
   hipLaunchKernelGGL(k_comp_stats, dim3(std::min<unsigned>(grid_for(T, BLOCK), COMP_STATS_BLOCKS)), dim3(BLOCK), 0, c->stream, A.c_nnz, A.c_rows, A.c_tr, T, (u32*)c->pt_hist.p);
-  HIPC(hipMemcpyAsync(&cst, c->pt_hist.p, sizeof(CompStats), hipMemcpyDeviceToHost, c->stream));
+  HIPC(hipMemcpyAsync(cst_pin, c->pt_hist.p, sizeof(CompStats), hipMemcpyDeviceToHost, c->stream));
   u64 NZ = 0;
   u32 ng = 0;
   P->n_small = 0;
@@ -1809,10 +1906,11 @@
     hipLaunchKernelGGL(k_eml_step<9>, dim3(grid_for(T, BLOCK)), dim3(BLOCK), 0, c->stream, A, T);
     if (int rc = exclusive_scan(c, A.c_small, T, (u64*)(tb + o_cum), (u64*)(tb + o_cum) + T)) return rc;
     if (int rc = exclusive_scan(c, A.c_big, T, (u64*)(tb + o_cumb), (u64*)(tb + o_cumb) + T)) return rc;
-    u64 nz2[2] = {0, 0};
-    HIPC(hipMemcpyAsync(&nz2[0], (u64*)(tb + o_cum) + T, 8, hipMemcpyDeviceToHost, c->stream));
-    HIPC(hipMemcpyAsync(&nz2[1], (u64*)(tb + o_cumb) + T, 8, hipMemcpyDeviceToHost, c->stream));
+    HIPC(hipMemcpyAsync(&nz_pin[0], (u64*)(tb + o_cum) + T, 8, hipMemcpyDeviceToHost, c->stream));
+    HIPC(hipMemcpyAsync(&nz_pin[1], (u64*)(tb + o_cumb) + T, 8, hipMemcpyDeviceToHost, c->stream));
     HIPC(hipStreamSynchronize(c->stream));
+    const u64 nz2[2] = {nz_pin[0], nz_pin[1]};
+    cst = *cst_pin;
     NZ = nz2[0] + nz2[1];
     if (comp_out) *comp_out = cst;
     if (NZ == 0) return 1;
@@ -1822,8 +1920,10 @@
     P->n_small = A.ng_small;
   } else {
     if (int rc = exclusive_scan(c, A.c_nnz, T, (u64*)(tb + o_cum), (u64*)(tb + o_cum) + T)) return rc;
-    HIPC(hipMemcpyAsync(&NZ, (u64*)(tb + o_cum) + T, 8, hipMemcpyDeviceToHost, c->stream));
+    HIPC(hipMemcpyAsync(&nz_pin[0], (u64*)(tb + o_cum) + T, 8, hipMemcpyDeviceToHost, c->stream));
     HIPC(hipStreamSynchronize(c->stream));
+    NZ = nz_pin[0];
+    cst = *cst_pin;
     if (comp_out) *comp_out = cst;
     if (NZ == 0) return 1;
     ng = (u32)((NZ - 1) / A.target_nnz + 1);
@@ -1834,11 +1934,13 @@
   HIPC(hipMemsetAsync(tb + o_gr, 0, t1.off - o_gr, c->stream));
   A.g_rows = (u32*)(tb + o_gr); A.g_tr = (u32*)(tb + o_gt); A.g_nnz = (u32*)(tb + o_gn); A.row_fill = (u32*)(tb + o_rf); A.tr_fill = (u32*)(tb + o_tf);
   hipLaunchKernelGGL(k_eml_step<2>, dim3(grid_for(T, BLOCK)), dim3(BLOCK), 0, c->stream, A, T);
-  std::vector<u32> g_rows(ng), g_tr(ng), g_nnz(ng);
-  HIPC(hipMemcpyAsync(g_rows.data(), A.g_rows, ng * 4, hipMemcpyDeviceToHost, c->stream));
-  HIPC(hipMemcpyAsync(g_tr.data(), A.g_tr, ng * 4, hipMemcpyDeviceToHost, c->stream));
-  HIPC(hipMemcpyAsync(g_nnz.data(), A.g_nnz, ng * 4, hipMemcpyDeviceToHost, c->stream));
+  const size_t g_span = (o_gn - o_gr) + (size_t)ng * 4;
+  if (int rc = plan_pin_ensure(c, g_span)) return rc;
+  HIPC(hipMemcpyAsync(c->plan_pin, tb + o_gr, g_span, hipMemcpyDeviceToHost, c->stream));
   HIPC(hipStreamSynchronize(c->stream));
+  const u32* const g_rows = (const u32*)c->plan_pin;
+  const u32* const g_tr = (const u32*)((const char*)c->plan_pin + (o_gt - o_gr));
+  const u32* const g_nnz = (const u32*)((const char*)c->plan_pin + (o_gn - o_gr));
   P->n_groups = ng; P->T = T; P->max_group_bytes = 0;
   P->row_base.assign(ng + 1, 0); P->tr_base.assign(ng + 1, 0); P->nz_base.assign(ng + 1, 0);
   for (u32 g = 0; g < ng; g++) {
@@ -2898,8 +3000,9 @@
   const u64 nseg = std::max(R, M);
   hipLaunchKernelGGL(k_sell_lens, dim3(grid_for(nseg, BLOCK)), dim3(BLOCK), 0, c->stream, B);
   hipLaunchKernelGGL(k_sell_sizes, dim3(grid_for(2 * (u64)ng, SELL_BUILD_WAVES)), dim3(64 * SELL_BUILD_WAVES), 0, c->stream, B);
-  std::vector<u32> gsz((size_t)ng * 4);
-  HIPC(hipMemcpyAsync(gsz.data(), B.gsz, (size_t)ng * 16, hipMemcpyDeviceToHost, c->stream));
+  if (int rc = plan_pin_ensure(c, (size_t)ng * 16)) return rc;
+  const u32* const gsz = (const u32*)c->plan_pin;
+  HIPC(hipMemcpyAsync(c->plan_pin, B.gsz, (size_t)ng * 16, hipMemcpyDeviceToHost, c->stream));
   HIPC(hipStreamSynchronize(c->stream));
   P->n_groups = ng; P->n_small = C.n_small; P->T = T; P->row_base = C.row_base; P->tr_base = C.tr_base; P->single_all = C.single_all;
   P->rslice_base.assign(ng + 1, 0); P->cslice_base.assign(ng + 1, 0); P->rell_base.assign(ng + 1, 0); P->cell_base.assign(ng + 1, 0);
@@ -2919,7 +3022,7 @@
   const u64 nrs = P->rslice_base[ng], ncs = P->cslice_base[ng], nru = P->rell_base[ng], ncu = P->cell_base[ng];
   Carver pv;
   const size_t p_rsb = pv.take((ng + 1) * 4), p_csb = pv.take((ng + 1) * 4), p_reb = pv.take((ng + 1) * 8), p_ceb = pv.take((ng + 1) * 8);
-  const size_t p_rd = pv.take(nrs * 8 + 8), p_cdesc = pv.take(ncs * 8 + 8), p_re = pv.take(nru * 2 + 8), p_ce = pv.take(ncu * 2 + 8);
+  const size_t p_rd = pv.take(nrs * 8 + 8), p_cdesc = pv.take(ncs * 8 + 8), p_re = pv.take(nru * 2 + 16), p_ce = pv.take(ncu * 2 + 16);
   const size_t p_cw = pv.take(R * 8 + 8), p_sg = pv.take(M * 8 + 8), p_ef = pv.take(M * 8 + 8), p_id = pv.take(M * 4 + 8);
   if (int rc = c->ems_plan.ensure(pv.off, 0, c->stream)) return rc;
   char* pb = (char*)c->ems_plan.p;
@@ -2941,17 +3044,18 @@
   }
   Carver bv;
   const size_t b_rb = bv.take((ng + 1) * 4), b_tb = bv.take((ng + 1) * 4), b_rf = bv.take(n_ecs * 4 + 8), b_ms = bv.take(T * 4 + 8), b_sa = bv.take(T * 8 + 8),
-               b_ef = bv.take(T * 8 + 8);
+               b_ef = bv.take(T * 8 + 8), b_gr = bv.take((size_t)ng * EMS_GREC_WORDS * 4 + 16);
   if (int rc = c->ems_maps.ensure(bv.off, 0, c->stream)) return rc;
   char* mb = (char*)c->ems_maps.p;
   HIPC(hipMemcpyAsync(mb + b_rb, cd.row_base, (ng + 1) * 4, hipMemcpyDeviceToDevice, c->stream));
   HIPC(hipMemcpyAsync(mb + b_tb, cd.tr_base, (ng + 1) * 4, hipMemcpyDeviceToDevice, c->stream));
   hipLaunchKernelGGL(k_sell_maps, dim3(grid_for(std::max<u64>(n_ecs, T), BLOCK)), dim3(BLOCK), 0, c->stream, A, B, (u32*)(mb + b_rf), (u32*)(mb + b_ms));
   HIPC(hipMemcpyAsync(mb + b_sa, A.single_all, T * 8, hipMemcpyDeviceToDevice, c->stream));
+  *dev = EmSellDev{(const u32*)(mb + b_rb), (const u32*)(mb + b_tb), B.rslice_base, B.cslice_base, B.rell_base, B.cell_base, B.rdesc, B.cdesc, B.rell, B.cell,
+                   B.cw_new, B.single_new, B.eff_new, (const u32*)(mb + b_gr)};
+  hipLaunchKernelGGL(k_sell_group_rec, dim3(grid_for(ng, BLOCK)), dim3(BLOCK), 0, c->stream, *dev, ng, (u32*)(mb + b_gr));
   HIPC(hipGetLastError());
   HIPC(hipStreamSynchronize(c->stream));
-  *dev = EmSellDev{(const u32*)(mb + b_rb), (const u32*)(mb + b_tb), B.rslice_base, B.cslice_base, B.rell_base, B.cell_base, B.rdesc, B.cdesc, B.rell, B.cell,
-                   B.cw_new, B.single_new, B.eff_new};
   if (cache) { cache->row_final = (u32*)(mb + b_rf); cache->mslot = (u32*)(mb + b_ms); cache->single_all = (double*)(mb + b_sa); cache->d_eff = (double*)(mb + b_ef); }
   return 0;
 }
diff --git a/scratch/em_clk_report.py b/scratch/em_clk_report.py
--- a/scratch/em_clk_report.py
+++ b/scratch/em_clk_report.py
@@ -41,3 +41,9 @@
             if sel.any():
                 print(f"  width {lo:2d}-{hi:2d}: n {sel.sum():6d}  sums {t_sum[sel].mean():8.1f} clk ({(t_sum[sel] / np.maximum(width[sel], 1)).mean():6.1f} / trip)  scan+finish {t_fin[sel].mean():8.1f}"
                       f"  (split {t_fin[sel & (meta == 1)].mean() if (sel & (meta == 1)).any() else 0:8.1f}, plain {t_fin[sel & (meta == 0)].mean() if (sel & (meta == 0)).any() else 0:8.1f})")
+if words >= 20:
+    print("entry -> tables in LDS    ", q((c[:, :, 17] - c[:, :, 16]).max(1)))
+    print("tables in LDS -> round 0  ", q((c[:, :, 18] - c[:, :, 17]).max(1)))
+    print("entry -> round 0, clocks  ", q((c[:, :, 18] - c[:, :, 16]).max(1)))
+    print("entry -> round 0, wall ticks (10 ns)", q(c[:, :, 19].max(1)))
+    print("round / (entry -> round 0)", f"{(tot / np.maximum((c[:, :, 18] - c[:, :, 16]).max(1), 1)).mean():.3f}")
```

Result: faster. 1162 (median of 6 runs) (+2.1%).
